# simonsobs/pixell

Hardware: AMD Instinct MI355X
Metric: map2alm+alm2map round-trips/sec (higher is better)
Workload: dtype f64

## Files before the change

### pixell_amd/csrc/fft.hip

```cpp
#include "fft.hpp"
#include "fft_dev.hpp"
#include <cmath>
#include <algorithm>
#include <functional>

namespace pxs {

struct KArgs {
	int n, nfac, T, generic, mode, forward, n1, n2;
	int ns;
	long N;
	const PassDesc* pass;
	const int* perm; const double2* tw;
	FastDiv dn, dT;
	FftDims d; long i_base, i_count;
	long ntile;
	FftLoad ld; FftStore st;
	double2* temp; const double2* bigtw;
	int load_inner_fast, store_inner_fast, tile_i;
};

__device__ __forceinline__ double2 read_elem(const void* p, int dtype, long off) {
	switch (dtype) {
		case PX_F32:  return make_double2((double)((const float*)p)[off], 0.0);
// ... 15 lines not shown
	const FftLoad& ld = a.ld;
	const long base = i*a.d.is_i + o1*a.d.is_o1 + o2*a.d.is_o2;
	const long N = a.N;
	switch (LM) {
	case LD_PLAIN: {
		const long se = e - ld.shift;
		if (se < 0 || (ld.ne >= 0 && se >= ld.ne)) return make_double2(0, 0);
		double2 v = read_elem(ld.ptr, ld.dtype, base + se*a.d.is_e);
		if (ld.mul) v = cmul(v, ld.mul[e]);
		return v; }
	case LD_HERM: {
		if (!ld.herm_fold) {
			const long Nh = ld.herm_n > 0 ? ld.herm_n : N;
			if (e >= Nh) return make_double2(0, 0);
			double2 v;
			if (e < ld.ne) v = read_elem(ld.ptr, ld.dtype, base + e*a.d.is_e);
			else if (Nh - e < ld.ne) v = cconj(read_elem(ld.ptr, ld.dtype, base + (Nh-e)*a.d.is_e));
			else return make_double2(0, 0);
			if (ld.mul) v = cmul(v, ld.mul[e]);
			return v;
		}
		double2 acc = make_double2(0, 0);
		for (long m = e; m < ld.ne; m += N) {
			double2 v = read_elem(ld.ptr, ld.dtype, base + m*a.d.is_e);
			if (ld.mul) v = cmul(v, ld.mul[m]);
			if (m == 0) v.y = 0;
			acc = cadd(acc, v);
		}
		for (long m = N - e; m < ld.ne; m += N) {
			double2 v = read_elem(ld.ptr, ld.dtype, base + m*a.d.is_e);
			if (ld.mul) v = cmul(v, ld.mul[m]);
			acc = cadd(acc, cconj(v));
		}
		return acc; }
	case LD_MIRROR: {
		long src = e;
		const bool odd = ((ld.par_step*(i + a.i_base) + ld.par0) & 1) != 0;
		bool neg = false;
		if (e >= ld.ne) { src = N - e - ld.mir_c; if (src < 0) src += N; neg = odd; }
		if (odd && (2*e + ld.mir_c) % N == 0) return make_double2(0, 0);
		double2 v = read_elem(ld.ptr, ld.dtype, base + src*a.d.is_e);
		if (ld.mul) v = cmul(v, ld.mul[src]);
		return neg ? make_double2(-v.x, -v.y) : v; }
	case LD_MIRROR_PAIR: {
		const long la = 2*(i + a.i_base), lb = la + 1;
		const bool a_odd = (ld.par0 & 1) != 0;
		long src = e; bool mir = false;
		if (e >= ld.ne) { src = N - e - ld.mir_c; if (src < 0) src += N; mir = true; }
		const bool selfm = ((2*e + ld.mir_c) % N) == 0;
		const long ba = (2*i)*a.d.is_i + o1*a.d.is_o1 + o2*a.d.is_o2;
		double2 va = read_elem(ld.ptr, ld.dtype, ba + src*a.d.is_e);
		double2 vb = (lb < ld.pair_lines) ? read_elem(ld.ptr, ld.dtype, ba + a.d.is_i + src*a.d.is_e) : make_double2(0, 0);
		double2& vo = a_odd ? va : vb;
		if (selfm) vo = make_double2(0, 0);
		else if (mir) { vo.x = -vo.x; vo.y = -vo.y; }
		return cadd(va, vb); }
	case LD_REAL_PAIR: {
		const long ba = (2*i)*a.d.is_i + o1*a.d.is_o1 + o2*a.d.is_o2;
		const double va = read_elem(ld.ptr, ld.dtype, ba + e*a.d.is_e).x;
		const double vb = (2*(i + a.i_base) + 1 < ld.pair_lines) ? read_elem(ld.ptr, ld.dtype, ba + a.d.is_i + e*a.d.is_e).x : 0.0;
		return make_double2(va, vb); }
	case LD_HERM_PAIR: {
		long m; bool cj;
		if (e < ld.ne) { m = e; cj = false; }
		else if (N - e < ld.ne) { m = N - e; cj = true; }
		else return make_double2(0, 0);
		const long ba = (2*i)*a.d.is_i + o1*a.d.is_o1 + o2*a.d.is_o2;
		double2 ha = read_elem(ld.ptr, ld.dtype, ba + m*a.d.is_e);
		double2 hb = (2*(i + a.i_base) + 1 < ld.pair_lines) ? read_elem(ld.ptr, ld.dtype, ba + a.d.is_i + m*a.d.is_e) : make_double2(0, 0);
		if (m == 0) { ha.y = 0; hb.y = 0; }
		if (cj) { ha.y = -ha.y; hb.y = -hb.y; }
		return make_double2(ha.x - hb.y, ha.y + hb.x); }
	case LD_SPEC: {
		const long Ns = ld.ne;
		long k = (2*e <= N) ? e : e - N;
		long ak = k < 0 ? -k : k;
		if (ld.kmax >= 0 && ak > ld.kmax) return make_double2(0, 0);
		if (2*ak > Ns) return make_double2(0, 0);
		long si = k >= 0 ? k : Ns + k;
		double2 v = read_elem(ld.ptr, ld.dtype, base + si*a.d.is_e);
		if (2*ak == Ns && ld.nyq_half && N != Ns) { v.x *= 0.5; v.y *= 0.5; }
		if (ld.mul) { double2 ph = ld.mul[ak]; if (k < 0) ph.y = -ph.y; v = cmul(v, ph); }
		return v; }
	default: {
		const long Nb = ld.ne;
		long k = (2*e <= N) ? e : e - N;
		long ak = k < 0 ? -k : k;
		if (ld.kmax >= 0 && ak > ld.kmax) return make_double2(0, 0);
		double2 ph = ld.mul ? ld.mul[ak] : make_double2(1, 0);
		if (2*ak == N && ld.nyq_half && N != Nb) {
			double2 vp = read_elem(ld.ptr, ld.dtype, base + ak*a.d.is_e);
			double2 vm = read_elem(ld.ptr, ld.dtype, base + (Nb-ak)*a.d.is_e);
			double2 r = cadd(cmul(vp, cconj(ph)), cmul(vm, ph));
			return make_double2(0.5*r.x, 0.5*r.y);
		}
		long si = k >= 0 ? k : Nb + k;
		double2 v = read_elem(ld.ptr, ld.dtype, base + si*a.d.is_e);
		if (k >= 0) ph.y = -ph.y;
		return cmul(v, ph); }
	}
}

__device__ __forceinline__ void store_functor(const KArgs& a, long i, long o1, long o2, long e, double2 v) {
	const FftStore& st = a.st;
	if ((st.ne >= 0 && e >= st.ne) || e < st.shift) return;
	long eo = e - st.shift;
	if (st.two_sided_k >= 0) {
		if (e > st.two_sided_k && e < a.N - st.two_sided_k) return;
		if (st.compact_two_sided && e > st.two_sided_k) eo = st.two_sided_k + (a.N - e);
	}
	if (st.conj_out) v.y = -v.y;
	if (st.mul) v = cmul(v, st.mul[e]);
	v.x *= st.scale; v.y *= st.scale;
	if (st.real_pair) {
		const long off = (2*i)*a.d.os_i + o1*a.d.os_o1 + o2*a.d.os_o2 + eo*a.d.os_e;
		write_elem(st.ptr, st.dtype, off, make_double2(v.x, 0));
		if (2*(i + a.i_base) + 1 < st.pair_lines) write_elem(st.ptr, st.dtype, off + a.d.os_i, make_double2(v.y, 0));
		return;
	}
	const long off = i*a.d.os_i + o1*a.d.os_o1 + o2*a.d.os_o2 + eo*a.d.os_e;
	write_elem(st.ptr, st.dtype, off, v);
}

template<int R, int NT> __device__ __forceinline__ void radix_pass(double2* buf, const double2* tw, const KArgs& a, const PassDesc& ps) {
	const int nb = a.n / R;
	const int total = a.T*nb;
	for (int b = threadIdx.x; b < total; b += NT) {
		const uint32_t t = fdiv(b, ps.dnb);
		const uint32_t bb = b - t*nb;
		const uint32_t blk = fdiv(bb, ps.dL);
		const uint32_t q = bb - blk*ps.L;
		const uint32_t p0 = t*a.ns + blk*ps.L*R + q;
		double2 v[R];
#pragma unroll
		for (int i = 0; i < R; i++) v[i] = buf[LPAD(p0 + i*ps.L)];
		if (ps.L > 1) {
			const int step = q*ps.tws;
#pragma unroll
			for (int i = 1; i < R; i++) v[i] = cmul(v[i], tw[i*step]);
		}
		butterfly<R>(v);
#pragma unroll
		for (int i = 0; i < R; i++) buf[LPAD(p0 + i*ps.L)] = v[i];
	}
}

template<int NT> __device__ __forceinline__ void generic_pass(const double2* src, double2* dst, const double2* tw, const KArgs& a, const PassDesc& ps) {
	const int R = ps.R, n = a.n;
	const int total = a.T*n;
	const int wstep = n / R;
	for (int idx = threadIdx.x; idx < total; idx += NT) {
		const uint32_t t = fdiv(idx, a.dn);
		const uint32_t j = idx - t*n;
		const uint32_t LR = ps.L*R;
		const uint32_t blk = j / LR;
		const uint32_t r = j - blk*LR;
		const uint32_t ip = r / ps.L;
		const uint32_t q = r - ip*ps.L;
		const uint32_t p0 = t*a.ns + blk*LR + q;
		double2 acc = make_double2(0, 0);
		uint32_t widx = 0;
		for (int i = 0; i < R; i++) {
			double2 v = src[LPAD(p0 + i*ps.L)];
			if (ps.L > 1) v = cmul(v, tw[i*q*ps.tws]);
			acc = cadd(acc, cmul(v, tw[widx*wstep]));
			widx += ip; if (widx >= (uint32_t)R) widx -= R;
		}
		dst[LPAD(t*a.ns + j)] = acc;
	}
}

struct TileCtx { long s0, other, o1, o2, lo; int nl; };
__device__ __forceinline__ TileCtx tile_decode(const KArgs& a, long bx) {
	TileCtx c;
	const long tile = bx % a.ntile; bx /= a.ntile;
	const long slim = (a.mode == 1) ? a.n2 : a.n1;
	c.other = 0;
	if (a.mode != 0) { const long no = a.tile_i ? slim : a.i_count; c.other = bx % no; bx /= no; }
	c.o1 = bx % a.d.n_o1; c.o2 = bx / a.d.n_o1;
	c.s0 = tile*a.T;
	const long tlim = (a.mode == 0 || a.tile_i) ? a.i_count : slim;
	c.nl = (int)min((long)a.T, tlim - c.s0);
	c.lo = c.o2*a.d.n_o1 + c.o1;
	return c;
}
template<int LM> __device__ __forceinline__ void tile_load_one(const KArgs& a, const TileCtx& c, int idx, int total, double2& v, int& pos) {
	const int n = a.n, T = a.T;
	pos = -1; v = make_double2(0, 0);
	if (idx >= total) return;
	uint32_t t, j;
	if (a.load_inner_fast) { j = fdiv(idx, a.dT); t = idx - j*T; }
	else                   { t = fdiv(idx, a.dn); j = idx - t*n; }
	if ((int)t >= c.nl) return;
	const long il = (a.mode == 0 || a.tile_i) ? c.s0 + t : c.other;
	const long sv = (a.mode == 0) ? 0 : (a.tile_i ? c.other : c.s0 + t);
	if (a.mode == 0)      v = load_functor<LM>(a, il, c.o1, c.o2, j);
	else if (a.mode == 1) v = load_functor<LM>(a, il, c.o1, c.o2, (long)j*a.n2 + sv);
	else {
		const long p2 = sv*a.n2 + j;
		v = a.temp[a.tile_i ? (c.lo*a.N + p2)*a.i_count + il : (c.lo*a.i_count + il)*a.N + p2];
	}
	if (!a.forward && a.mode != 2) v.y = -v.y;
	pos = (int)(t*a.ns) + a.perm[j];
}
template<int NT, bool GEN> __device__ __forceinline__ double2* tile_passes(const KArgs& a, double2* cur, double2* oth, const double2* tw) {
	for (int p = 0; p < a.nfac; p++) {
		const PassDesc ps = a.pass[p];
		switch (ps.R) {
			case 2: radix_pass<2, NT>(cur, tw, a, ps); break;
			case 3: radix_pass<3, NT>(cur, tw, a, ps); break;
			case 4: radix_pass<4, NT>(cur, tw, a, ps); break;
			case 5: radix_pass<5, NT>(cur, tw, a, ps); break;
			default: if constexpr (GEN) { generic_pass<NT>(cur, oth, tw, a, ps); double2* x = cur; cur = oth; oth = x; } break;
		}
		PXS_LDS_BARRIER();
	}
	return cur;
}
template<int NT> __device__ __forceinline__ void tile_store(const KArgs& a, const TileCtx& c, const double2* cur) {
	const int n = a.n, T = a.T, total = T*n;
	for (int idx0 = threadIdx.x; idx0 < total; idx0 += 4*NT) {
#pragma unroll
		for (int u = 0; u < 4; u++) {
			const int idx = idx0 + u*NT;
			if (idx >= total) continue;
			uint32_t t, j;
			if (a.store_inner_fast) { j = fdiv(idx, a.dT); t = idx - j*T; }
			else                    { t = fdiv(idx, a.dn); j = idx - t*n; }
			if ((int)t >= c.nl) continue;
			const long il = (a.mode == 0 || a.tile_i) ? c.s0 + t : c.other;
			const long sv = (a.mode == 0) ? 0 : (a.tile_i ? c.other : c.s0 + t);
			double2 v = cur[LPAD(t*a.ns + j)];
			if (a.mode == 1) {
				v = cmul(v, a.bigtw[(long)j*sv]);
				const long p2 = (long)j*a.n2 + sv;
				a.temp[a.tile_i ? (c.lo*a.N + p2)*a.i_count + il : (c.lo*a.i_count + il)*a.N + p2] = v;
			} else {
				if (!a.forward) v.y = -v.y;
				if (a.mode == 0) store_functor(a, il, c.o1, c.o2, j, v);
				else             store_functor(a, il, c.o1, c.o2, sv + (long)a.n1*j, v);
			}
		}
	}
}

template<int LM, int NT, bool GEN> __global__ __launch_bounds__(NT) void fft_lds_kernel(const KArgs a)
{
	PXS_SHARED(double2, lds);
	const int n = a.n, T = a.T;
	double2* tw = lds;
	double2* bufA = lds + n;
	double2* bufB = bufA + (size_t)T*a.ns + 1;
	const TileCtx c = tile_decode(a, blockIdx.x);
	for (int k = threadIdx.x; k < n; k += NT) tw[k] = a.tw[k];
	const int total = T*n;
	constexpr int LU = 4;
	for (int idx0 = threadIdx.x; idx0 < total; idx0 += LU*NT) {
		double2 v[LU]; int pos[LU];
#pragma unroll
		for (int u = 0; u < LU; u++) tile_load_one<LM>(a, c, idx0 + u*NT, total, v[u], pos[u]);
#pragma unroll
		for (int u = 0; u < LU; u++) if (pos[u] >= 0) bufA[LPAD(pos[u])] = v[u];
	}
	PXS_LDS_BARRIER();
	const double2* cur = tile_passes<NT, GEN>(a, bufA, bufB, tw);
	tile_store<NT>(a, c, cur);
}

template<int LM> static void launch_tiles_m(const KArgs& k, long nblk, size_t sh, hipStream_t st, int nt_override) {
#ifdef PXS_HOST_SIM
	hipLaunchKernelGGL((fft_lds_kernel<LM, 1, true>), dim3((unsigned)nblk), dim3(1), sh, st, k);
#else
	static const int nt_env = [] { const char* e = lab_getenv("PXS_FFT_NT"); return e ? atoi(e) : 0; }();
	const int nt = nt_override ? nt_override : nt_env ? nt_env : ((long)k.T*k.n >= 2048 ? 512 : 256);
	static const bool once = [] {
		(void)hipFuncSetAttribute((const void*)fft_lds_kernel<LM, 256, false>, hipFuncAttributeMaxDynamicSharedMemorySize, 160*1024 - 256);
		(void)hipFuncSetAttribute((const void*)fft_lds_kernel<LM, 256, true>, hipFuncAttributeMaxDynamicSharedMemorySize, 160*1024 - 256);
		(void)hipFuncSetAttribute((const void*)fft_lds_kernel<LM, 512, false>, hipFuncAttributeMaxDynamicSharedMemorySize, 160*1024 - 256);
		(void)hipFuncSetAttribute((const void*)fft_lds_kernel<LM, 128, false>, hipFuncAttributeMaxDynamicSharedMemorySize, 160*1024 - 256);
		return true; }();
	(void)once;
	if (k.generic)      hipLaunchKernelGGL((fft_lds_kernel<LM, 256, true>), dim3((unsigned)nblk), dim3(256), sh, st, k);
	else if (nt == 512) hipLaunchKernelGGL((fft_lds_kernel<LM, 512, false>), dim3((unsigned)nblk), dim3(512), sh, st, k);
	else if (nt == 128) hipLaunchKernelGGL((fft_lds_kernel<LM, 128, false>), dim3((unsigned)nblk), dim3(128), sh, st, k);
	else                hipLaunchKernelGGL((fft_lds_kernel<LM, 256, false>), dim3((unsigned)nblk), dim3(256), sh, st, k);
#endif
}
static void launch_tiles(const KArgs& k, long nblk, size_t sh, hipStream_t st, int nt_override = 0) {
	const int lm = k.mode == 2 ? (int)LD_PLAIN : k.ld.mode;
	switch (lm) {
		case LD_PLAIN:       launch_tiles_m<LD_PLAIN>(k, nblk, sh, st, nt_override); break;
		case LD_HERM:        launch_tiles_m<LD_HERM>(k, nblk, sh, st, nt_override); break;
		case LD_MIRROR:      launch_tiles_m<LD_MIRROR>(k, nblk, sh, st, nt_override); break;
		case LD_SPEC:        launch_tiles_m<LD_SPEC>(k, nblk, sh, st, nt_override); break;
		case LD_SPEC_ADJ:    launch_tiles_m<LD_SPEC_ADJ>(k, nblk, sh, st, nt_override); break;
		case LD_MIRROR_PAIR: launch_tiles_m<LD_MIRROR_PAIR>(k, nblk, sh, st, nt_override); break;
		case LD_REAL_PAIR:   launch_tiles_m<LD_REAL_PAIR>(k, nblk, sh, st, nt_override); break;
		case LD_HERM_PAIR:   launch_tiles_m<LD_HERM_PAIR>(k, nblk, sh, st, nt_override); break;
		default: throw Error(PXS_ERR_ARG, "fft: unknown load mode");
	}
}

struct FftSub {
	int n; std::vector<int> fac; bool generic = false;
	DevBuf perm, tw, d_pass;
	PassDesc pass[FFT_MAXFAC]; int nfac = 0;
};

static std::vector<int> factorize(long n) {
	std::vector<int> f;
	static const int oddfirst = [] { const char* e = lab_getenv("PXS_FFT_ODDFIRST"); return e ? atoi(e) : 1; }();
	if (oddfirst) {
		while (n % 3 == 0) { f.push_back(3); n /= 3; }
		while (n % 5 == 0) { f.push_back(5); n /= 5; }
		int twos = 0; while (n % 2 == 0) { twos++; n /= 2; }
		if (twos & 1) { f.push_back(2); twos--; }
		while (twos >= 2) { f.push_back(4); twos -= 2; }
	}
	while (n % 4 == 0) { f.push_back(4); n /= 4; }
	while (n % 2 == 0) { f.push_back(2); n /= 2; }
	while (n % 3 == 0) { f.push_back(3); n /= 3; }
	while (n % 5 == 0) { f.push_back(5); n /= 5; }
	for (long p = 7; p*p <= n; p += 2) while (n % p == 0) { f.push_back((int)p); n /= p; }
	if (n > 1) f.push_back((int)n);
	return f;
}

static void twiddles(long n, std::vector<double2>& tw) {
	tw.resize(n);
	const long double tp = 6.283185307179586476925286766559L;
	for (long k = 0; k < n; k++) {
		long double ang = tp*(long double)k/(long double)n;
		tw[k] = make_double2((double)cosl(ang), (double)(-sinl(ang)));
	}
}

FftContext::FftContext(int device) : device_(device) {
	size_t fr = 0, tot = 0;
	if (hipMemGetInfo(&fr, &tot) == hipSuccess && fr > 0) temp_budget = std::min<size_t>(size_t(4) << 30, std::max<size_t>(fr/16, size_t(64) << 20));
}
FftContext::~FftContext() {}

static bool split_two(long n, long& n1, long& n2) {
	long best = -1, best8 = -1;
	for (long a = 1; a*a <= n; a++) if (n % a == 0) {
		long b = n/a; if (b > FFT_NLOC_MAX) continue;
		best = a;
		if (a % 8 == 0 && b % 8 == 0 && 4*a >= b) best8 = a;
	}
	if (best < 0) return false;
	static const int align8 = [] { const char* e = lab_getenv("PXS_FFT_ALIGN8"); return e ? atoi(e) : 1; }();
	if (best8 > 0 && align8) best = best8;
	n1 = best; n2 = n/best;
	return n1 <= FFT_NLOC_MAX && n2 <= FFT_NLOC_MAX;
}

bool FftContext::supported(long n, std::string* why) {
	if (n < 1) { if (why) *why = "length < 1"; return false; }
	if (n <= FFT_NLOC_MAX) {
		if ((int)factorize(n).size() > FFT_MAXFAC) { if (why) *why = "too many factors"; return false; }
		return true;
	}
	long n1, n2;
	if (!split_two(n, n1, n2)) {
		if (why) *why = "FFT length " + std::to_string(n) + " has no factorisation n1*n2 with both factors <= " +
			std::to_string(FFT_NLOC_MAX) + " (large prime factor; Bluestein not implemented)";
		return false;
	}
	return true;
}

long FftContext::good_size(long n) {
	for (long m = std::max<long>(n, 1);; m++) {
		long r = m;
		while (r % 2 == 0) r /= 2; while (r % 3 == 0) r /= 3; while (r % 5 == 0) r /= 5;
		if (r == 1 && supported(m)) return m;
	}
}

static std::vector<int> factorize_comp(long n, int maxr) {
	static const std::vector<int> allowed = [] {
		std::vector<int> a; const char* e = lab_getenv("PXS_FFT_RADICES");
		std::string s = e ? e : "16,15,12,10,9,8,7,6,5,4,3,2";
		size_t pos = 0;
		while (pos < s.size()) { size_t c = s.find(',', pos); if (c == std::string::npos) c = s.size(); int v = atoi(s.substr(pos, c-pos).c_str()); if (v >= 2 && (v <= 5 || v <= PXS_COMP_MAXR)) a.push_back(v); pos = c+1; }
		return a; }();
	std::vector<int> best, cur;
	std::function<void(long, size_t)> rec = [&](long m, size_t from) {
		if (m == 1) { if (best.empty() || cur.size() < best.size()) best = cur; return; }
		if (!best.empty() && cur.size()+1 >= best.size()) return;
		for (size_t i = from; i < allowed.size(); i++) if (m % allowed[i] == 0 && (allowed[i] == 7 ? maxr >= 9 : (allowed[i] <= 5 || allowed[i] <= maxr))) { cur.push_back(allowed[i]); rec(m/allowed[i], i); cur.pop_back(); }
	};
	rec(n, 0);
	if (best.empty()) return factorize(n);
	std::stable_sort(best.begin(), best.end(), [](int a, int b) { const bool oa = a & 1, ob = b & 1; if (oa != ob) return oa; return a > b; });
	return best;
}

std::shared_ptr<FftSub> FftContext::sub(long n, bool comp, int maxr) {
	std::lock_guard<std::mutex> g(mu_);
	static const bool comp_on = [] { const char* e = lab_getenv("PXS_FFT_COMP"); return e ? atoi(e) != 0 : true; }();
	comp = comp && comp_on;
	maxr = std::min(maxr, PXS_COMP_MAXR);
	const long key = comp ? -(n + ((long)maxr << 40)) : n;
	auto it = subs_.find(key);
	if (it != subs_.end()) return it->second;
	auto s = std::make_shared<FftSub>();
	s->n = (int)n; s->fac = comp ? factorize_comp(n, maxr) : factorize(n);
	PXS_REQUIRE((int)s->fac.size() <= FFT_MAXFAC, "FFT: too many factors");
	int L = 1; s->nfac = (int)s->fac.size();
	std::vector<int> Ls(s->nfac+1); Ls[0] = 1;
	for (int p = 0; p < s->nfac; p++) {
		int R = s->fac[p];
		const bool comp_r = comp && R <= maxr && (R == 6 || R == 8 || R == 9 || R == 10 || R == 12 || R == 15 || R == 16);
		const bool seven = comp && R == 7 && maxr >= 9;
		if (R != 2 && R != 3 && R != 4 && R != 5 && !comp_r && !seven) s->generic = true;
		PassDesc& ps = s->pass[p];
		ps.R = R; ps.L = L; ps.tws = (int)(n/((long)L*R));
		ps.dL = make_fastdiv(L); ps.dnb = make_fastdiv((uint32_t)(n/R));
		L *= R; Ls[p+1] = L;
	}
	std::vector<int> perm(n);
	for (long j = 0; j < n; j++) {
		long t = j, pos = 0;
		for (int p = s->nfac-1; p >= 0; p--) { long i = t % s->fac[p]; t /= s->fac[p]; pos += i*Ls[p]; }
		perm[j] = (int)pos;
	}
	std::vector<double2> tw; twiddles(n, tw);
	s->perm = upload(perm); s->tw = upload(tw);
	s->d_pass = upload(std::vector<PassDesc>(s->pass, s->pass + FFT_MAXFAC));
	subs_[key] = s;
	return s;
}

FftContext::SubView FftContext::view(long n, int maxr) {
	auto s = sub(n, true, maxr);
	SubView v; v.n = s->n; v.nfac = s->nfac; v.ns = s->n | 1; v.generic = s->generic ? 1 : 0;
	v.pass = s->d_pass.p; v.perm = s->perm.as<int>(); v.tw = s->tw.as<double2>();
	return v;
}

const double2* FftContext::bigtw(long n) {
	std::lock_guard<std::mutex> g(mu_);
	auto it = bigtw_.find(n);
	if (it != bigtw_.end()) return it->second.as<double2>();
	std::vector<double2> tw; twiddles(n, tw);
	bigtw_[n] = upload(tw);
	return bigtw_[n].as<double2>();
}

static void fill_sub(KArgs& k, const FftSub& s, long maxlines) {
	k.n = s.n; k.nfac = s.nfac; k.generic = s.generic;
#ifdef PXS_LAB
	{ static const int nopass = [] { const char* e = getenv("PXS_FFT_DEBUG_NOPASS"); return e ? atoi(e) : 0; }(); if (nopass) k.nfac = 0; }
#endif
	k.pass = s.d_pass.as<PassDesc>();
	k.perm = s.perm.as<int>(); k.tw = s.tw.as<double2>();
	int bufs = s.generic ? 2 : 1;
	static const long env_pts = [] { const char* e = lab_getenv("PXS_FFT_PTS"); return e ? atol(e) : 0L; }();
	long pts = s.n <= 1024 ? FFT_LDS_PTS/2 : FFT_LDS_PTS;
	if (env_pts > 0 && s.n <= env_pts/2) pts = env_pts;
	long T = (pts - s.n)/((long)bufs*s.n);
	if (T < 1) T = 1;
	if (T > 64) T = 64;
	static const int align8 = [] { const char* e = lab_getenv("PXS_FFT_ALIGN8"); return e ? atoi(e) : 1; }();
	if (align8) {
		if (T >= 8) T -= T % 8;
		else if (T >= 5 && (long)bufs*8*s.n + s.n <= FFT_LDS_PTS) T = 8;
	}
	if (T > maxlines) T = maxlines;
	k.T = (int)T;
	k.dn = make_fastdiv(s.n); k.dT = make_fastdiv((uint32_t)T);
	static const int lpad = [] { const char* e = lab_getenv("PXS_FFT_LINEPAD"); return e ? atoi(e) : 1; }();
	k.ns = lpad ? (s.n | 1) : s.n;
}

static size_t lds_bytes(const KArgs& k) { const size_t pts = (size_t)k.T*k.ns + 2; return sizeof(double2)*((size_t)k.n + pts*(k.generic ? 2 : 1)); }

void FftContext::exec(hipStream_t st, long n, bool forward, const FftDims& d, const FftLoad& ld, const FftStore& stf) {
	std::string why;
	if (!supported(n, &why)) throw Error(PXS_ERR_UNSUPPORTED, why);
	if (d.n_i <= 0 || d.n_o1 <= 0 || d.n_o2 <= 0) return;
	KArgs k; memset(&k, 0, sizeof(k));
	k.N = n; k.forward = forward ? 1 : 0; k.d = d; k.ld = ld; k.st = stf; k.i_base = 0; k.i_count = d.n_i;
	if (n <= FFT_NLOC_MAX) {
		auto s = sub(n);
		fill_sub(k, *s, d.n_i);
		k.mode = 0; k.n1 = (int)n; k.n2 = 1;
		k.ntile = (d.n_i + k.T - 1)/k.T;
		k.load_inner_fast  = (std::abs(d.is_i) < std::abs(d.is_e)) ? 1 : 0;
		k.store_inner_fast = (std::abs(d.os_i) < std::abs(d.os_e)) ? 1 : 0;
		long nblk = k.ntile*d.n_o1*d.n_o2;
		size_t sh = lds_bytes(k);
		launch_tiles(k, nblk, sh, st);
		PXS_HIP(hipGetLastError());
		return;
	}
	long n1, n2; split_two(n, n1, n2);
	auto s1 = sub(n1); auto s2 = sub(n2);
	const double2* btw = bigtw(n);
	long lines_budget = std::max<long>(1, (long)(temp_budget/(sizeof(double2)*n)));
	DevBuf* tbuf = nullptr;
	{
		std::lock_guard<std::mutex> g(mu_);
		size_t want = sizeof(double2)*n*std::min<long>(lines_budget, d.n_i*d.n_o1*d.n_o2);
		tbuf = &temps_[st];
		tbuf->ensure(want);
	}
	long o1_per = 1, i_per = d.n_i;
	if (d.n_i <= lines_budget) { o1_per = std::min<long>(d.n_o1, std::max<long>(1, lines_budget/d.n_i)); }
	else i_per = lines_budget;
	for (long o2 = 0; o2 < d.n_o2; o2++)
	for (long o1 = 0; o1 < d.n_o1; o1 += o1_per)
	for (long i0 = 0; i0 < d.n_i; i0 += i_per) {
		long no1 = std::min(o1_per, d.n_o1 - o1), ni = std::min(i_per, d.n_i - i0);
		KArgs a = k;
		a.d.n_o1 = no1; a.d.n_o2 = 1; a.i_base = i0; a.i_count = ni;
		auto esz = [](int dt) { return dt == PX_F32 ? 4 : dt == PX_F64 ? 8 : dt == PX_C64 ? 8 : 16; };
		const long lmul = (ld.mode == LD_MIRROR_PAIR || ld.mode == LD_REAL_PAIR || ld.mode == LD_HERM_PAIR) ? 2 : 1;
		const long smul = stf.real_pair ? 2 : 1;
		a.ld.ptr = (const char*)ld.ptr + esz(ld.dtype)*(o2*d.is_o2 + o1*d.is_o1 + lmul*i0*d.is_i);
		a.st.ptr = (char*)stf.ptr + esz(stf.dtype)*(o2*d.os_o2 + o1*d.os_o1 + smul*i0*d.os_i);
		a.temp = tbuf->as<double2>(); a.bigtw = btw; a.n1 = (int)n1; a.n2 = (int)n2;
		const int tile_i = (std::abs(d.is_i) < std::abs(d.is_e)) ? 1 : 0;
		KArgs pa = a; fill_sub(pa, *s1, tile_i ? ni : n2); pa.mode = 1; pa.tile_i = tile_i;
		pa.ntile = ((tile_i ? ni : n2) + pa.T - 1)/pa.T;
		pa.load_inner_fast = 1; pa.store_inner_fast = 1;
		long nblkA = pa.ntile*(tile_i ? n2 : ni)*no1;
		launch_tiles(pa, nblkA, lds_bytes(pa), st);
		KArgs pb = a; fill_sub(pb, *s2, tile_i ? ni : n1); pb.mode = 2; pb.tile_i = tile_i;
		pb.ntile = ((tile_i ? ni : n1) + pb.T - 1)/pb.T;
		pb.load_inner_fast = tile_i ? 1 : 0; pb.store_inner_fast = 1;
		long nblkB = pb.ntile*(tile_i ? n1 : ni)*no1;
		launch_tiles(pb, nblkB, lds_bytes(pb), st);
		PXS_HIP(hipGetLastError());
	}
}

}
```

### pixell_amd/csrc/fft.hpp

```cpp
#pragma once
#include "common.hpp"
#include <map>
#include <memory>
#include <mutex>

namespace pxs {

enum LoadMode : int { LD_PLAIN = 0, LD_HERM = 1, LD_MIRROR = 2, LD_SPEC = 3, LD_SPEC_ADJ = 4, LD_MIRROR_PAIR = 5, LD_REAL_PAIR = 6, LD_HERM_PAIR = 7 };

struct FftDims {
	long n_i = 1, n_o1 = 1, n_o2 = 1;
	long is_i = 0, is_o1 = 0, is_o2 = 0, is_e = 1;
	long os_i = 0, os_o1 = 0, os_o2 = 0, os_e = 1;
};

struct FftLoad {
	const void* ptr = nullptr; int dtype = PX_C128; int mode = LD_PLAIN;
	long ne = -1;
	const double2* mul = nullptr;
	long shift = 0;
	int mir_c = 0, par0 = 0;
	int par_step = 1;
	long kmax = -1;
	int nyq_half = 0;
	long pair_lines = 0;
	int herm_fold = 0;
	long herm_n = 0;
};

struct FftStore {
	void* ptr = nullptr; int dtype = PX_C128;
	long ne = -1;
	long two_sided_k = -1;
	const double2* mul = nullptr;
	double scale = 1.0;
	long shift = 0;
	int conj_out = 0;
	int compact_two_sided = 0;
	int real_pair = 0;
	long pair_lines = 0;
};

struct FftSub;

class FftContext {
public:
	explicit FftContext(int device);
	~FftContext();
	void exec(hipStream_t st, long n, bool forward, const FftDims& d, const FftLoad& ld, const FftStore& stf);
	static long good_size(long n);
	static bool supported(long n, std::string* why = nullptr);
	struct SubView { int n, nfac, ns, generic; const void* pass; const int* perm; const double2* tw; };
	SubView view(long n, int maxr = 1000);
	const double2* twiddle_table(long n) { return bigtw(n); }
	void release_stream(hipStream_t st) { std::lock_guard<std::mutex> g(mu_); temps_.erase(st); }
	size_t temp_budget = size_t(4) << 30;
private:
	int device_;
	std::mutex mu_;
	std::map<long, std::shared_ptr<FftSub>> subs_;
	std::map<long, DevBuf> bigtw_;
	std::map<hipStream_t, DevBuf> temps_;
	std::shared_ptr<FftSub> sub(long n, bool comp = false, int maxr = 1000);
	const double2* bigtw(long n);
};

}
```

### pixell_amd/csrc/fftchain.hip

```cpp
#include "fftchain.hpp"
#include "fft_dev.hpp"
#include "chain_dev.hpp"
#include <algorithm>
#include <set>
#include <type_traits>
#include <cmath>

namespace pxs {

#ifndef PXS_CH_PTS
#define PXS_CH_PTS 2560
#endif
#ifdef PXS_HOST_SIM
static constexpr int CH_NT = 1, CH_MAXE = PXS_CH_PTS;
#else
#ifndef PXS_CH_NT
#define PXS_CH_NT 512
#endif
static constexpr int CH_NT = PXS_CH_NT, CH_MAXE = (PXS_CH_PTS + PXS_CH_NT - 1)/PXS_CH_NT;
#endif
static constexpr int CH_TILE_PTS = PXS_CH_PTS;
static constexpr int CH_NMAX = 512;

struct TileC { int outer, t0, nl, comp, q0; };

struct BlkIn {
	int Tw, nBf, wL; FastDiv dTTw, dTw, dwL;
	__device__ __forceinline__ long off(int line, int e, int nrows) const {
		const uint32_t B = fdiv((uint32_t)e, dTw);
		const int w = (int)B < nBf ? Tw : wL;
		return (long)B*Tw*nrows + (long)line*w + (e - (int)B*Tw);
	}
	__device__ __forceinline__ void split(int idx, int T, uint32_t& li, uint32_t& e) const {
		uint32_t B = fdiv((uint32_t)idx, dTTw);
		if ((int)B < nBf) { const uint32_t rem = idx - B*T*Tw; li = fdiv(rem, dTw); e = B*Tw + (rem - li*Tw); }
		else { const uint32_t rem = idx - (uint32_t)nBf*T*Tw; li = fdiv(rem, dwL); e = (uint32_t)nBf*Tw + (rem - li*wL); }
	}
};

struct StageBase {
	static constexpr bool R7 = true;
	static constexpr int NT = CH_NT;
	static constexpr int PTS = CH_TILE_PTS;
	LdsFft fa, fb;
	BlkIn bin; int bout;
	int T; int ntile;
	FastDiv dT, dna, dnb, dnt;
	const double2* btw; const double2* tws;
	int pf;
	static constexpr int PF = 256;
	static constexpr int PFI = 0;
	__device__ __forceinline__ const void* pfaddr(const TileC&, int) const { return nullptr; }
};

#ifndef PXS_HOST_SIM
#define PXS_CH_BOUNDS __launch_bounds__(NT, S::MINW)
#else
#define PXS_CH_BOUNDS
#endif
template<class S, int NT, int MAXE> __global__ PXS_CH_BOUNDS void chain_kernel(const S s)
{
	PXS_SHARED(double2, lds);
	const int na = s.fa.n, nb = s.fb.n;
	const int nlast = S::TWO ? nb : na, nslast = S::TWO ? s.fb.ns : s.fa.ns;
	const bool same_tw = S::TWO && nb == na;
	double2* twa = lds; double2* twb = same_tw ? lds : lds + na; double2* twx = lds + na + (same_tw ? 0 : nb); double2* buf = twx + (S::HAS_TW ? nlast : 0);
	TileC c;
	if (!s.decode((int)blockIdx.x, c)) return;
	const bool have_tw = S::HAS_TW && s.btw != nullptr;
	const int T = s.T;
	int pf_val = 0;
	{
		const int total = T*na;
		double2 v[MAXE]; int pos[MAXE];
#pragma unroll
		for (int u = 0; u < MAXE; u++) {
			const int idx = threadIdx.x + u*NT; pos[u] = -1;
			if (idx < total) {
				uint32_t li, e;
				if (S::LOAD_LINE_FAST) { e = fdiv(idx, s.dT); li = idx - e*T; }
				else if (s.bin.Tw > 0) s.bin.split(idx, T, li, e);
				else { li = fdiv(idx, s.dna); e = idx - li*na; }
				v[u] = s.load(c, (int)li, (int)e);
				if (S::INV_A) v[u].y = -v[u].y;
				pos[u] = (int)li*s.fa.ns + s.fa.perm[e];
			}
		}
		if ((S::LOADK == 0 || S::PFI > 0) && s.pf > 0 && (long)blockIdx.x + s.pf < (long)gridDim.x) {
			TileC c2;
			if (s.decode((int)blockIdx.x + s.pf, c2)) {
				if (S::LOADK == 0) {
					const int per = (na*16 + 127) >> 7, i = threadIdx.x;
					if (i < T*per) {
						const int li = i/per, seg = i - li*per;
						const double2* r = s.row(c2, li);
						if (r) pf_val = *reinterpret_cast<const int*>(reinterpret_cast<const char*>(r) + seg*128);
					}
				} else {
#pragma unroll
					for (int it = 0; it < S::PFI; it++) {
						const void* q = s.pfaddr(c2, (int)threadIdx.x + it*NT);
						if (q) pf_val += *reinterpret_cast<const int*>(q);
					}
				}
			}
		}
		for (int k = threadIdx.x; k < na; k += NT) twa[k] = s.fa.tw[k];
		if (!same_tw) for (int k = threadIdx.x; k < nb; k += NT) twb[k] = s.fb.tw[k];
		if (have_tw) for (int k = threadIdx.x; k < nlast; k += NT) twx[k] = s.btw[(long)c.t0*k];
#pragma unroll
		for (int u = 0; u < MAXE; u++) if (pos[u] >= 0) buf[pos[u]] = v[u];
	}
	PXS_LDS_BARRIER();
	lds_fft<NT, S::MAXR, S::R7>(buf, twa, s.fa, T);
	if (S::TWO) {
		const int total = T*nb;
		double2 v[MAXE]; int pos[MAXE];
#pragma unroll
		for (int u = 0; u < MAXE; u++) {
			const int idx = threadIdx.x + u*NT; pos[u] = -1;
			if (idx < total) {
				const uint32_t e = fdiv(idx, s.dT), li = idx - e*T;
				{ const double2* Al = buf + li*s.fa.ns; v[u] = s.mid(c, (int)li, (int)e, [&](int k) { return Al[k]; }); }
				if (S::INV_B) v[u].y = -v[u].y;
				pos[u] = (int)li*s.fb.ns + s.fb.perm[e];
			}
		}
		PXS_LDS_BARRIER();
#pragma unroll
		for (int u = 0; u < MAXE; u++) if (pos[u] >= 0) buf[pos[u]] = v[u];
		PXS_LDS_BARRIER();
		lds_fft<NT, S::MAXR, S::R7>(buf, twb, s.fb, T);
	}
	{
		const int total = T*nlast;
		const FastDiv dl = S::TWO ? s.dnb : s.dna;
		for (int idx = threadIdx.x; idx < total; idx += NT) {
			uint32_t li, e;
			if (S::STORE_LINE_FAST) { e = fdiv(idx, s.dT); li = idx - e*T; } else { li = fdiv(idx, dl); e = idx - li*nlast; }
			double2 w = make_double2(1, 0);
			if (have_tw) w = cmul(twx[e], s.tws[e*T + li]);
			s.store(c, (int)li, (int)e, [&](int l2, int e2) { return buf[l2*nslast + e2]; }, w);
		}
	}
#ifndef PXS_HOST_SIM
	if (S::LOADK == 0 || S::PFI > 0) asm volatile("" :: "v"(pf_val));
#endif
}

struct StFirst : StageBase {
	static constexpr int SID = 0;
	static constexpr bool TWO = false, INV_A = false, INV_B = false, LOAD_LINE_FAST = true, STORE_LINE_FAST = true, HAS_TW = true;
	static constexpr int MAXR = 9, MINW = 1;
	PairSrc src; int b; double2* Y; long ldY; int npair; FastDiv dnp;
	static constexpr int LOADK = 1, STOREK = 0;
	__device__ __forceinline__ const double2* row(const TileC&, int) const { return nullptr; }
	__device__ __forceinline__ bool decode(int bx, TileC& c) const {
		c.outer = fdiv(bx, dnt); c.t0 = (bx - c.outer*ntile)*T; c.nl = min(T, b - c.t0);
		c.comp = fdiv(c.outer, dnp); c.q0 = c.outer - c.comp*npair; return true; }
	__device__ __forceinline__ double2 load(const TileC& c, int li, int e) const {
		if (li >= c.nl) return make_double2(0, 0);
		return src.get(c.comp, c.q0, b*e + c.t0 + li); }
	template<class AF> __device__ __forceinline__ double2 mid(const TileC&, int, int, AF&&) const { return make_double2(0, 0); }
	template<class VF> __device__ __forceinline__ void store(const TileC& c, int li, int e, VF&& val, double2 w) const {
		if (li >= c.nl) return;
		const long o = bout ? ((long)c.outer*b + c.t0)*fa.n + (long)e*c.nl + li : ((long)c.outer*fa.n + e)*ldY + c.t0 + li;
		Y[o] = cmul(val(li, e), w); }
};

struct StFirst2D : StFirst {
	static constexpr bool R7 = false;
	static constexpr int PFI = 2;
	__device__ __forceinline__ const void* pfaddr(const TileC& c, int i) const {
		const int segs = (c.nl + 7) >> 3;
		const int e = i/segs; if (e >= fa.n) return nullptr;
		return src.leg + (long)c.comp*src.cstride + (long)c.q0*src.ld + (b*e + c.t0 + 8*(i - e*segs)); }
};

struct StResize : StageBase {
	static constexpr int SID = 1;
	static constexpr bool TWO = true, INV_A = false, INV_B = true, LOAD_LINE_FAST = false, STORE_LINE_FAST = true, HAS_TW = true;
	#ifndef PXS_RESIZE_MINW
#define PXS_RESIZE_MINW 1
#endif
	static constexpr int MAXR = 9, MINW = PXS_RESIZE_MINW;
#ifdef PXS_RESIZE_PTS
	static constexpr int PTS = PXS_RESIZE_PTS;
#endif
	const double2* Y; long ldY; double2* Z; long ldZ;
	int g, X1, X2, kmax, nyq; const double2* ph; FastDiv dg;
	int adj;
	static constexpr int LOADK = 0, STOREK = 0;
	__device__ __forceinline__ const double2* row(const TileC& c, int li) const { return li < c.nl ? Y + ((long)c.outer*g + c.t0 + li)*ldY : nullptr; }
	__device__ __forceinline__ bool decode(int bx, TileC& c) const {
		c.outer = fdiv(bx, dnt); c.t0 = (bx - c.outer*ntile)*T; c.nl = min(T, g - c.t0); return true; }
	__device__ __forceinline__ double2 load(const TileC& c, int li, int e) const {
		if (li >= c.nl) return make_double2(0, 0);
		return bin.Tw > 0 ? Y[(long)c.outer*g*fa.n + bin.off(c.t0 + li, e, g)] : Y[((long)c.outer*g + c.t0 + li)*ldY + e]; }
	template<class AF> __device__ __forceinline__ double2 mid(const TileC& c, int li, int e, AF&& A) const {
		if (li >= c.nl) return make_double2(0, 0);
		const int k1 = c.t0 + li;
		const int jp = g*e + k1;
		const int kap = (2*jp <= X2) ? jp : jp - X2;
		const int ak = kap < 0 ? -kap : kap;
		if ((kmax >= 0 && ak > kmax) || 2*ak > X1) return make_double2(0, 0);
		const int k = kap >= 0 ? kap : kap + X1;
		const uint32_t k2 = fdiv((uint32_t)(k - k1), dg);
		double2 v = A((int)k2);
		if (adj) {
			double2 t = ph ? ph[ak] : make_double2(1, 0);
			if (2*ak == X2 && X1 != X2) {
				const double2 vm = A((int)fdiv((uint32_t)(X1 - ak - k1), dg));
				const double2 r = cadd(cmul(v, cconj(t)), cmul(vm, t));
				return cscale(r, 0.5);
			}
			if (kap >= 0) t.y = -t.y;
			return cmul(v, t);
		}
		if (nyq && 2*ak == X1) v = cscale(v, 0.5);
		if (ph) { double2 t = ph[ak]; if (kap < 0) t.y = -t.y; v = cmul(v, t); }
		return v; }
	template<class VF> __device__ __forceinline__ void store(const TileC& c, int li, int e, VF&& val, double2 w) const {
		if (li >= c.nl) return;
		const long o = bout ? ((long)c.outer*g + c.t0)*fb.n + (long)e*c.nl + li : ((long)c.outer*fb.n + e)*ldZ + c.t0 + li;
		Z[o] = cmul(cconj(val(li, e)), cconj(w)); }
};

struct StSigma : StageBase {
	static constexpr int SID = 2;
	static constexpr bool TWO = true, INV_A = true, INV_B = false, LOAD_LINE_FAST = false, STORE_LINE_FAST = true, HAS_TW = true;
	static constexpr int MAXR = 9, MINW = 1;
	const double2* Z; long ldZ; double2* V; long ldV; int g, g2; const double2* sigma;
	static constexpr int LOADK = 0, STOREK = 0;
	__device__ __forceinline__ const double2* row(const TileC& c, int li) const { return li < c.nl ? Z + ((long)c.outer*g2 + c.t0 + li)*ldZ : nullptr; }
	__device__ __forceinline__ bool decode(int bx, TileC& c) const {
		c.outer = fdiv(bx, dnt); c.t0 = (bx - c.outer*ntile)*T; c.nl = min(T, g2 - c.t0); return true; }
	__device__ __forceinline__ double2 load(const TileC& c, int li, int e) const {
		if (li >= c.nl) return make_double2(0, 0);
		return bin.Tw > 0 ? Z[(long)c.outer*g2*fa.n + bin.off(c.t0 + li, e, g2)] : Z[((long)c.outer*g2 + c.t0 + li)*ldZ + e]; }
	template<class AF> __device__ __forceinline__ double2 mid(const TileC& c, int li, int e, AF&& A) const {
		if (li >= c.nl) return make_double2(0, 0);
		return cmul(cconj(A(e)), sigma[(c.t0 + li) + g2*e]); }
	template<class VF> __device__ __forceinline__ void store(const TileC& c, int li, int e, VF&& val, double2 w) const {
		if (li >= c.nl) return;
		const long o = bout ? ((long)c.outer*g2 + c.t0)*fb.n + (long)e*c.nl + li : ((long)c.outer*g + e)*ldV + c.t0 + li;
		V[o] = cmul(val(li, e), w); }
};

template<int MODE> struct StSplit : StageBase {
	static constexpr int SID = 3 + MODE;
#ifndef PXS_HOST_SIM
	static constexpr int NT = MODE == 1 ? 256 : CH_NT;
#endif
	static constexpr int PF = MODE == 1 ? 512 : 256;
	static constexpr bool TWO = false, INV_A = true, INV_B = false, LOAD_LINE_FAST = false, STORE_LINE_FAST = true, HAS_TW = false;
	static constexpr int MAXR = 9, MINW = 1;
	const double2* U; long ldU; int a, g, X, mir_c, nr_out, a_odd, ncol, npair;
	double2* out; long ld; const double2* w; const double2* tab; double scale; int TH; FastDiv da;
	long ocstride; int groups; FastDiv dnp, dgr;
	int self_half;
	static constexpr int LOADK = 0, STOREK = 1;
	__device__ __forceinline__ const double2* row(const TileC& c, int li) const {
		int line, pair; slot(c, li, line, pair);
		return line >= 0 ? U + (((long)c.comp*npair + pair)*a + line)*ldU : nullptr; }
	__device__ __forceinline__ int mirror_line(int k) const { int m = a - k - mir_c; if (m >= a) m -= a; if (m < 0) m += a; return m; }
	__device__ __forceinline__ bool decode(int bx, TileC& c) const {
		c.outer = fdiv(bx, dnt); c.t0 = (bx - c.outer*ntile)*(MODE == 0 ? TH : 1); c.nl = T;
		if (MODE == 0) { c.comp = fdiv(c.outer, dnp); c.q0 = c.outer - c.comp*npair; }
		else { c.comp = fdiv(c.outer, dgr); c.q0 = (c.outer - c.comp*groups)*(T/2); }
		if (MODE == 1) { if (mirror_line(c.t0) < c.t0) return false; }
		return true; }
	__device__ __forceinline__ void slot(const TileC& c, int li, int& line, int& pair) const {
		if (MODE == 0) {
			pair = c.q0;
			const int prim = c.t0 + (li < TH ? li : li - TH);
			line = -1;
			if (prim < a) {
				const int m = mirror_line(prim);
				if (li < TH) { if (prim <= m) line = prim; }
				else if (prim < m) line = m;
			}
		} else {
			pair = c.q0 + (li >> 1);
			const int m = mirror_line(c.t0);
			line = (li & 1) ? (m != c.t0 ? m : -1) : c.t0;
			if (pair >= npair) line = -1;
		}
	}
	__device__ __forceinline__ double2 load(const TileC& c, int li, int e) const {
		int line, pair; slot(c, li, line, pair);
		if (line < 0) return make_double2(0, 0);
		if (MODE == 0 && bin.Tw > 0) return U[((long)c.comp*npair + pair)*a*fa.n + bin.off(line, e, a)];
		return U[(((long)c.comp*npair + pair)*a + line)*ldU + e]; }
	template<class AF> __device__ __forceinline__ double2 mid(const TileC&, int, int, AF&&) const { return make_double2(0, 0); }
	template<class VF> __device__ __forceinline__ void store(const TileC& c, int li, int e, VF&& val, double2) const {
		int line, pair; slot(c, li, line, pair);
		if (line < 0) return;
		const int t = line + a*e;
		if (t >= nr_out) return;
		int tm = X - t - mir_c; if (tm >= X) tm -= X; if (tm < 0) tm += X;
		const double2 z = cconj(val(li, e));
		double2 ev, od;
		if (tm == t) { ev = self_half ? cscale(z, 0.5) : z; od = make_double2(0, 0); }
		else {
			const int ml = mirror_line(line);
			const int lp = (ml == line) ? li : (MODE == 0 ? (li < TH ? li + TH : li - TH) : (li ^ 1));
			const int e2 = (int)fdiv((uint32_t)(tm - ml), da);
			const double2 y = cconj(val(lp, e2));
			ev = make_double2(0.5*(z.x + y.x), 0.5*(z.y + y.y)); od = make_double2(0.5*(z.x - y.x), 0.5*(z.y - y.y));
		}
		const int ca = 2*pair;
		double2 va = a_odd ? od : ev, vb = a_odd ? ev : od;
		double2* oc = out + (long)c.comp*ocstride;
		if (MODE == 0) {
			const double f = scale*(w ? w[t].x : 1.0);
			oc[(long)ca*ld + t] = cscale(va, f);
			if (ca + 1 < ncol) oc[(long)(ca + 1)*ld + t] = cscale(vb, f);
		} else {
			const double f = scale*(w ? w[t].x : 1.0);
			oc[(long)t*ld + ca] = cscale(cmul(va, cconj(tab[ca])), f);
			if (ca + 1 < ncol) oc[(long)t*ld + ca + 1] = cscale(cmul(vb, cconj(tab[ca + 1])), f);
		}
	}
};


struct StRingA1 : StageBase {
	static constexpr int SID = 5;
	static constexpr int PTS = 2880;
	static constexpr bool TWO = false, INV_A = false, INV_B = false, LOAD_LINE_FAST = true, STORE_LINE_FAST = true, HAS_TW = true;
	static constexpr int MAXR = 8, MINW = 8;
	MapAddr m; int b, npair; double2* Y; long ldY; FastDiv dnp;
	static constexpr int LOADK = 1, STOREK = 0;
	__device__ __forceinline__ const double2* row(const TileC&, int) const { return nullptr; }
	__device__ __forceinline__ bool decode(int bx, TileC& c) const {
		c.outer = fdiv(bx, dnt); c.t0 = (bx - c.outer*ntile)*T; c.nl = min(T, b - c.t0);
		c.comp = fdiv(c.outer, dnp); c.q0 = c.outer - c.comp*npair; return true; }
	__device__ __forceinline__ double2 load(const TileC& c, int li, int e) const {
		if (li >= c.nl) return make_double2(0, 0);
		const int x = b*e + c.t0 + li;
		const int bi = (int)fdiv(c.comp, m.dncb);
		const long o = bi*m.bstride + (c.comp - bi*m.ncb)*m.cstride + m.off0 + (2L*c.q0)*m.rstride + x*m.pstride;
		const double re = rd_real(m.ptr, m.dtype, o).x;
		const double im = (2*c.q0 + 1 < m.nring) ? rd_real(m.ptr, m.dtype, o + m.rstride).x : 0.0;
		return make_double2(re, im); }
	template<class AF> __device__ __forceinline__ double2 mid(const TileC&, int, int, AF&&) const { return make_double2(0, 0); }
	template<class VF> __device__ __forceinline__ void store(const TileC& c, int li, int e, VF&& val, double2 w) const {
		if (li >= c.nl) return;
		Y[((long)c.outer*fa.n + e)*ldY + c.t0 + li] = cmul(val(li, e), w); }
};

struct StRingA2 : StageBase {
	static constexpr int SID = 6;
	static constexpr int PF = 512;
	static constexpr bool TWO = false, INV_A = false, INV_B = false, LOAD_LINE_FAST = false, STORE_LINE_FAST = true, HAS_TW = false;
	static constexpr int MAXR = 8, MINW = 8;
	const double2* Y; long ldY; int a, X, npair, groups, nring, mmax; double2* leg; long ldleg; int nm; const double2* tab; double scale; FastDiv da, dgr;
	static constexpr int LOADK = 0, STOREK = 1;
	__device__ __forceinline__ const double2* row(const TileC& c, int li) const {
		int line, q; slot(c, li, line, q);
		return line >= 0 ? Y + (((long)c.comp*npair + q)*a + line)*ldY : nullptr; }
	__device__ __forceinline__ int mirror_line(int k) const { return k == 0 ? 0 : a - k; }
	__device__ __forceinline__ bool decode(int bx, TileC& c) const {
		c.outer = fdiv(bx, dnt); c.t0 = bx - c.outer*ntile; c.nl = T;
		c.comp = fdiv(c.outer, dgr); c.q0 = (c.outer - c.comp*groups)*(T/2);
		return mirror_line(c.t0) >= c.t0; }
	__device__ __forceinline__ void slot(const TileC& c, int li, int& line, int& q) const {
		q = c.q0 + (li >> 1);
		const int ml = mirror_line(c.t0);
		line = (li & 1) ? (ml != c.t0 ? ml : -1) : c.t0;
		if (q >= npair) line = -1;
	}
	__device__ __forceinline__ double2 load(const TileC& c, int li, int e) const {
		int line, q; slot(c, li, line, q);
		if (line < 0) return make_double2(0, 0);
		return Y[(((long)c.comp*npair + q)*a + line)*ldY + e]; }
	template<class AF> __device__ __forceinline__ double2 mid(const TileC&, int, int, AF&&) const { return make_double2(0, 0); }
	template<class VF> __device__ __forceinline__ void store(const TileC& c, int li, int e, VF&& val, double2) const {
		int line, q; slot(c, li, line, q);
		if (line < 0) return;
		const int k = line + a*e;
		if (k > mmax) return;
		const double2 zp = val(li, e);
		double2 zm;
		if (k == 0) zm = zp;
		else {
			const int kp = X - k, ml = mirror_line(line);
			const int lp = (ml == line) ? li : (li ^ 1);
			zm = val(lp, (int)fdiv((uint32_t)(kp - ml), da));
		}
		double2 xa = make_double2(0.5*(zp.x + zm.x), 0.5*(zp.y - zm.y));
		const double2 d = make_double2(zp.x - zm.x, zp.y + zm.y);
		double2 xb = make_double2(0.5*d.y, -0.5*d.x);
		const double2 t = tab ? tab[k] : make_double2(1, 0);
		double2* o = leg + ((long)c.comp*nm + k)*ldleg + 2*q;
		o[0] = cscale(cmul(xa, t), scale);
		if (2*q + 1 < nring) o[1] = cscale(cmul(xb, t), scale);
	}
};

struct StRingS1 : StageBase {
	static constexpr int SID = 7;
	static constexpr bool TWO = false, INV_A = true, INV_B = false, LOAD_LINE_FAST = true, STORE_LINE_FAST = true, HAS_TW = true;
	static constexpr int MAXR = 8, MINW = 8;
	const double2* h; long ldh, hcomp; int b, X, npair, nring, mmax; double2* Y; long ldY; FastDiv dnp;
	static constexpr int LOADK = 1, STOREK = 0;
	__device__ __forceinline__ const double2* row(const TileC&, int) const { return nullptr; }
	__device__ __forceinline__ bool decode(int bx, TileC& c) const {
		c.outer = fdiv(bx, dnt); c.t0 = (bx - c.outer*ntile)*T; c.nl = min(T, b - c.t0);
		c.comp = fdiv(c.outer, dnp); c.q0 = c.outer - c.comp*npair; return true; }
	__device__ __forceinline__ double2 load(const TileC& c, int li, int e) const {
		if (li >= c.nl) return make_double2(0, 0);
		const int k = b*e + c.t0 + li;
		int m; bool cj;
		if (k <= mmax) { m = k; cj = false; }
		else if (X - k <= mmax) { m = X - k; cj = true; }
		else return make_double2(0, 0);
		const double2* r = h + ((long)c.comp*hcomp + 2*c.q0)*ldh + m;
		double2 ha = r[0];
		double2 hb = (2*c.q0 + 1 < nring) ? r[ldh] : make_double2(0, 0);
		if (m == 0) { ha.y = 0; hb.y = 0; }
		if (cj) { ha.y = -ha.y; hb.y = -hb.y; }
		return make_double2(ha.x - hb.y, ha.y + hb.x); }
	template<class AF> __device__ __forceinline__ double2 mid(const TileC&, int, int, AF&&) const { return make_double2(0, 0); }
	template<class VF> __device__ __forceinline__ void store(const TileC& c, int li, int e, VF&& val, double2 w) const {
		if (li >= c.nl) return;
		const long o = bout ? ((long)c.outer*b + c.t0)*fa.n + (long)e*c.nl + li : ((long)c.outer*fa.n + e)*ldY + c.t0 + li;
		Y[o] = cmul(cconj(val(li, e)), cconj(w)); }
};

struct StRingS2 : StageBase {
	static constexpr int SID = 8;
	static constexpr bool TWO = false, INV_A = true, INV_B = false, LOAD_LINE_FAST = false, STORE_LINE_FAST = true, HAS_TW = false;
	static constexpr int MAXR = 8, MINW = 8;
	const double2* Y; long ldY; int a, npair; MapAddr m; FastDiv dnp;
	static constexpr int LOADK = 0, STOREK = 0;
	__device__ __forceinline__ const double2* row(const TileC& c, int li) const { return li < c.nl ? Y + ((long)c.outer*a + c.t0 + li)*ldY : nullptr; }
	__device__ __forceinline__ bool decode(int bx, TileC& c) const {
		c.outer = fdiv(bx, dnt); c.t0 = (bx - c.outer*ntile)*T; c.nl = min(T, a - c.t0);
		c.comp = fdiv(c.outer, dnp); c.q0 = c.outer - c.comp*npair; return true; }
	__device__ __forceinline__ double2 load(const TileC& c, int li, int e) const {
		if (li >= c.nl) return make_double2(0, 0);
		return bin.Tw > 0 ? Y[(long)c.outer*a*fa.n + bin.off(c.t0 + li, e, a)] : Y[((long)c.outer*a + c.t0 + li)*ldY + e]; }
	template<class AF> __device__ __forceinline__ double2 mid(const TileC&, int, int, AF&&) const { return make_double2(0, 0); }
	template<class VF> __device__ __forceinline__ void store(const TileC& c, int li, int e, VF&& val, double2) const {
		if (li >= c.nl) return;
		const int x = c.t0 + li + a*e;
		const double2 v = val(li, e);
		const int bi = (int)fdiv(c.comp, m.dncb);
		const long o = bi*m.bstride + (c.comp - bi*m.ncb)*m.cstride + m.off0 + (2L*c.q0)*m.rstride + x*m.pstride;
		wr_real(m.ptr, m.dtype, o, v.x);
		if (2*c.q0 + 1 < m.nring) wr_real(m.ptr, m.dtype, o + m.rstride, -v.y);
	}
};

struct StColOut : StageBase {
	static constexpr int SID = 9;
	static constexpr bool R7 = false;
	static constexpr bool TWO = false, INV_A = false, INV_B = false, LOAD_LINE_FAST = false, STORE_LINE_FAST = true, HAS_TW = false;
	static constexpr int MAXR = 9, MINW = 1;
	const double2* Y; long ldY; int a, nm, ny, nx, groups, conj_out, herm; double2* out; long ldo, ocomp; double scale; FastDiv dgr;
	static constexpr int LOADK = 0, STOREK = 0;
	__device__ __forceinline__ const double2* row(const TileC& c, int li) const { return c.q0 + li < nm ? Y + (((long)c.comp*nm + c.q0 + li)*a + c.t0)*ldY : nullptr; }
	__device__ __forceinline__ bool decode(int bx, TileC& c) const {
		c.outer = fdiv(bx, dnt); c.t0 = bx - c.outer*ntile; c.nl = T;
		c.comp = fdiv(c.outer, dgr); c.q0 = (c.outer - c.comp*groups)*T; return true; }
	__device__ __forceinline__ double2 load(const TileC& c, int li, int e) const {
		const int kx = c.q0 + li;
		if (kx >= nm) return make_double2(0, 0);
		return Y[(((long)c.comp*nm + kx)*a + c.t0)*ldY + e]; }
	template<class AF> __device__ __forceinline__ double2 mid(const TileC&, int, int, AF&&) const { return make_double2(0, 0); }
	template<class VF> __device__ __forceinline__ void store(const TileC& c, int li, int e, VF&& val, double2) const {
		const int kx = c.q0 + li;
		if (kx >= nm) return;
		const int ky = c.t0 + a*e;
		double2 v = cscale(val(li, e), scale);
		double2* oc = out + (long)c.comp*ocomp;
		oc[(long)ky*ldo + kx] = conj_out ? cconj(v) : v;
		if (herm && kx > 0 && 2*kx < nx) oc[(long)(ky == 0 ? 0 : ny - ky)*ldo + (nx - kx)] = conj_out ? v : cconj(v);
	}
};

static bool smooth235(long n) { if (n < 1) return false; for (int p : {2, 3, 5}) while (n % p == 0) n /= p; return n == 1; }
bool FftChain::sub_ok(long n) { return n >= 2 && n <= CH_NMAX && smooth235(n); }

static LdsFft mk(FftContext* fc, long n, int maxr = 9) {
	LdsFft f; memset(&f, 0, sizeof(f));
	if (n <= 0) return f;
	auto v = fc->view(n, maxr);
#ifdef PXS_LAB
	static const int nofft = [] { const char* e = getenv("PXS_CH_NOFFT"); return e ? atoi(e) : 0; }();
#else
	constexpr int nofft = 0;
#endif
	static const int nspad = [] { const char* e = lab_getenv("PXS_CH_NS_PAD"); return e ? atoi(e) : 0; }();
	f.n = v.n; f.nfac = nofft ? 0 : v.nfac; f.ns = v.ns + nspad; f.generic = v.generic; f.pass = (const PassDesc*)v.pass; f.perm = v.perm; f.tw = v.tw; f.dn = make_fastdiv((uint32_t)n);
	return f;
}

const double2* FftChain::small_tw(long X, int n, int T) {
#ifdef PXS_LAB
	{ static const int notw = [] { const char* e = getenv("PXS_CH_NOTW"); return e ? atoi(e) : 0; }(); if (notw) return nullptr; }
#endif
	std::lock_guard<std::mutex> g(mu_);
	auto key = std::make_tuple(X, n, T);
	auto it = stw_.find(key);
	if (it != stw_.end()) return it->second.as<double2>();
	std::vector<double2> t((size_t)n*T);
	const long double tp = 6.283185307179586476925286766559L;
	for (int e = 0; e < n; e++) for (int li = 0; li < T; li++) {
		const long double ang = tp*(long double)(((long)li*e) % X)/(long double)X;
		t[(size_t)e*T + li] = make_double2((double)cosl(ang), (double)(-sinl(ang)));
	}
	stw_[key] = upload(t);
	return stw_[key].as<double2>();
}

static int tile_lines(long n_a, long n_b, long nlines, int mult, long tab_pts = -1) {
	const long n = std::max(n_a, n_b);
	long T = CH_TILE_PTS / n;
	if (T >= mult) T -= T % mult;
	if (T < 1) T = 1;
	const long cap = ((nlines + mult - 1)/mult)*mult;
	if (T > cap) T = cap;
	static const long limit = [] { const char* e = lab_getenv("PXS_RING_TILE_KB"); return e ? (long)(atof(e)*1024) : 0L; }();
	if (tab_pts >= 0 && limit > 0)
		while (T > mult && (long)sizeof(double2)*(tab_pts + T*(n | 1) + 2) > limit) T -= mult;
	return (int)T;
}
template<class S> void FftChain::set_tiles(S& s, int T, long nlines, long X) {
	s.T = T; s.ntile = (int)((nlines + T - 1)/T); s.dT = make_fastdiv((uint32_t)T); s.dnt = make_fastdiv((uint32_t)s.ntile);
	s.dna = make_fastdiv((uint32_t)s.fa.n); s.dnb = make_fastdiv((uint32_t)std::max(1, s.fb.n));
	s.btw = nullptr; s.tws = nullptr;
	if (X > 0) { s.tws = small_tw(X, S::TWO ? s.fb.n : s.fa.n, T); s.btw = s.tws ? fc_->twiddle_table(X) : nullptr; }
}
static bool blocked_on() { static const bool on = [] { const char* e = lab_getenv("PXS_CH_BLOCKED"); return e ? atoi(e) != 0 : false; }(); return on; }
static BlkIn mk_blk(int Tw, long na, int T) {
	BlkIn b; memset(&b, 0, sizeof(b));
	if (!blocked_on()) return b;
	b.Tw = Tw; b.nBf = (int)(na/Tw); b.wL = (int)(na - (long)b.nBf*Tw);
	b.dTTw = make_fastdiv((uint32_t)(T*Tw)); b.dTw = make_fastdiv((uint32_t)Tw); b.dwL = make_fastdiv((uint32_t)std::max(b.wL, 1));
	return b;
}

static const int F2_RADICES[] = {2, 3, 4, 5, 6, 8, 9};

template<class S> static void launch_stage(const S& s, long nblk, hipStream_t st) {
	if (nblk <= 0) return;
	PXS_REQUIRE((long)s.T*std::max(s.fa.n, s.fb.n) <= S::PTS, "internal: chain tile too large");
	PXS_REQUIRE(nblk < (1L << 31), "internal: chain grid too large");
	size_t sh = sizeof(double2)*((size_t)s.fa.n + (S::TWO && s.fb.n == s.fa.n ? 0 : s.fb.n) + (S::HAS_TW ? std::max(s.fa.n, s.fb.n) : 0) + (size_t)s.T*std::max(s.fa.ns, s.fb.ns) + 2);
	{ static const size_t pad = [] { const char* e = lab_getenv("PXS_CH_LDS_PAD"); return e ? (size_t)atol(e) : (size_t)0; }(); sh += pad; }
	{ static const int pf = [] {
		const std::string name = "PXS_CH_PF_SID" + std::to_string(S::SID);
		const char* e1 = lab_getenv(name.c_str()); const char* e = lab_getenv("PXS_CH_PF");
		return e1 ? atoi(e1) : (e ? atoi(e) : S::PF); }(); const_cast<S&>(s).pf = pf; }
	if (getenv("PXS_CHAIN_VERBOSE")) {
		static std::mutex mu; static std::set<std::tuple<int, int, int, int>> seen; std::lock_guard<std::mutex> g(mu);
		if (seen.insert(std::make_tuple(S::SID, s.fa.n, s.fb.n, s.T)).second)
			fprintf(stderr, "[pxsht] chain stage %d: na=%d nb=%d T=%d LDS %.1f KiB -> %d WG/CU by LDS, %ld workgroups\n", S::SID, s.fa.n, s.fb.n, s.T, sh/1024.0, (int)((160*1024)/sh), nblk);
	}
#ifndef PXS_HOST_SIM
#ifdef PXS_CH_NT2
	static const long mask2 = [] { const char* e = lab_getenv("PXS_CH_NT2_MASK"); return e ? strtol(e, nullptr, 0) : 0L; }();
	if ((mask2 >> S::SID) & 1) {
		constexpr int NT2 = PXS_CH_NT2, MAXE2 = (S::PTS + NT2 - 1)/NT2;
		static const bool once2 = [] { (void)hipFuncSetAttribute((const void*)chain_kernel<S, NT2, MAXE2>, hipFuncAttributeMaxDynamicSharedMemorySize, 160*1024 - 256); return true; }();
		(void)once2;
		hipLaunchKernelGGL((chain_kernel<S, NT2, MAXE2>), dim3((unsigned)nblk), dim3(NT2), sh, st, s);
		return;
	}
#endif
	static const bool once = [] { (void)hipFuncSetAttribute((const void*)chain_kernel<S, S::NT, (S::PTS + S::NT - 1)/S::NT>, hipFuncAttributeMaxDynamicSharedMemorySize, 160*1024 - 256); return true; }();
	(void)once;
#endif
	hipLaunchKernelGGL((chain_kernel<S, S::NT, (S::PTS + S::NT - 1)/S::NT>), dim3((unsigned)nblk), dim3(S::NT), sh, st, s);
}

template<class S> int FftChain::tile_lines_for(long n_a, long n_b, long nlines, int mult, long tab_pts) {
	int T = tile_lines(n_a, n_b, nlines, mult, tab_pts);
	if (S::PTS > CH_TILE_PTS && T < mult && (long)mult*std::max(n_a, n_b) <= S::PTS && nlines >= mult) T = mult;
	return T;
}
template<class S> void FftChain::launch_any(S& s, long nblk, hipStream_t st) { launch_stage(s, nblk, st); }

static bool split_balanced(long n, Split& s, long amax = 320) {
	long best = 0; double bestc = 1e300;
	for (long a = 2; a <= 1024 && a <= n/2; a++) if (n % a == 0) {
		const long b = n/a;
		if (!FftChain::sub_ok(a) || !FftChain::sub_ok(b)) continue;
		double c = std::fabs(std::log((double)a/(double)b));
		if (a > amax) c += 10;
		if (b % 8) c += 0.3;
		if (c < bestc) { bestc = c; best = a; }
	}
	if (!best) return false;
	s.a = best; s.b = n/best; return true;
}

bool FftChain::plan_rings(long nphi) {
	nphi_ = nphi; ra_ = Split(); rs_ = Split();
	Split s;
	if (!split_balanced(nphi, s)) return false;
	ra_.a = std::min(s.a, s.b); ra_.b = nphi/ra_.a;
	rs_.b = std::min(s.a, s.b); rs_.a = nphi/rs_.b;
	for (long a = 320; a >= 16; a -= 16) if (nphi % a == 0 && nphi/a <= 160 && nphi/a >= 2 && sub_ok(a) && sub_ok(nphi/a)) { rs_.a = a; rs_.b = nphi/a; break; }
	for (long b = 256; b >= 16; b -= 16) if (nphi % b == 0 && nphi/b >= 2 && nphi/b <= 320 && sub_ok(b) && sub_ok(nphi/b)) { ra_.b = b; ra_.a = nphi/b; break; }
	{
		const char* ea = lab_getenv("PXS_RING_A_ANA"); const char* es = lab_getenv("PXS_RING_A_SYN");
		if (ea && atol(ea) > 1 && nphi % atol(ea) == 0 && sub_ok(atol(ea)) && sub_ok(nphi/atol(ea))) { ra_.a = atol(ea); ra_.b = nphi/ra_.a; }
		if (es && atol(es) > 1 && nphi % atol(es) == 0 && sub_ok(atol(es)) && sub_ok(nphi/atol(es))) { rs_.a = atol(es); rs_.b = nphi/rs_.a; }
	}
	return true;
}

static long smooth_at_least(long n, bool even_product_with = false, long g = 1) {
	for (long m = std::max<long>(n, 2);; m++) if (smooth235(m) && (!even_product_with || ((m*g) % 2 == 0))) return m;
}

static bool smooth2357(long n) { if (n < 1) return false; for (int p : {2, 3, 5, 7}) while (n % p == 0) n /= p; return n == 1; }
static bool sub_ok7(long n) { return n >= 2 && n <= CH_NMAX && smooth2357(n); }
bool FftChain::sub_ok_theta(long n) { return sub_ok7(n); }
long FftChain::ducc_ncc(int lmax) {
	for (long n = std::max<long>(lmax + 1, 1);; n++) { long r = n; for (int p : {2, 3, 5, 7, 11}) while (r % p == 0) r /= p; if (r == 1) return 2*n; }
}

static double tile_fill(long n) {
	long T = CH_TILE_PTS / n; if (T >= 8) T -= T % 8; if (T < 1) T = 1;
	return (double)(T*n)/(double)CH_TILE_PTS*(T >= 8 ? 1.0 : 0.8);
}
static double modulus_pref(long g) { return 1.0 + 0.02*std::max(0.0, std::log2((double)g/160.0)) + 0.04*std::max(0.0, std::log2(64.0/(double)g)); }
ThetaPlan FftChain::plan_theta(long N, int lmax) {
	ThetaPlan best; double bestc = 1e300;
	static const long gforce = [] { const char* e = lab_getenv("PXS_THETA_G"); return e ? atol(e) : 0L; }();
	static const bool ducc_size = [] { const char* e = lab_getenv("PXS_THETA_DUCC_NCC"); return e ? atoi(e) != 0 : true; }();
	const long Nd = ducc_ncc(lmax);
	auto consider = [&](long g, long ac) {
		ThetaPlan t; t.N = N; t.g = g; t.bN = N/g; t.ac = ac; t.Ncc = g*ac;
		t.g2 = smooth_at_least((N + 2L*lmax + 2 + g - 1)/g); t.M = g*t.g2;
		if ((t.Ncc & 1) || !sub_ok(t.g2) || !sub_ok7(t.ac)) return;
		long gs_best = 0; double gsc = 1e300;
		static const long gsforce = [] { const char* e = lab_getenv("PXS_THETA_GS"); return e ? atol(e) : 0L; }();
		for (long gs = 2; gs <= 1024; gs++) if (t.Ncc % gs == 0 && N % gs == 0 && sub_ok7(gs) && sub_ok7(t.Ncc/gs) && sub_ok7(N/gs) && (!gsforce || gs == gsforce)) {
			const double c = ((2.0*t.Ncc + 1.5*N)/tile_fill(gs) + (double)(t.Ncc + N)/tile_fill(std::max(t.Ncc/gs, N/gs)))*modulus_pref(gs);
			if (c < gsc) { gsc = c; gs_best = gs; }
		}
		if (!gs_best) return;
		t.gs = gs_best; t.bs = t.Ncc/gs_best; t.aNs = N/gs_best;
		const double lmin = 2.0*lmax + 2, M2 = 2.0*t.Ncc;
		const double ana = (2.0*N + 2.0*M2 + 1.5*t.Ncc)/tile_fill(g) + (N + M2)/tile_fill(std::max(t.bN, 2*t.ac)) + (M2 + t.Ncc)/tile_fill(2*t.ac);
		double c = 60.0*(t.Ncc - lmin)/lmin + (ana*modulus_pref(g) + gsc)/(3.0*N + 4.0*M2 + 2.5*t.Ncc + 3.0*t.Ncc + 2.5*N);
		if (ducc_size && t.Ncc == Nd) c -= 1000.0;
		if (c < bestc) { bestc = c; best = t; best.ok = true; }
	};
	for (long g = 2; g <= 1024 && g <= N/2; g++) if (N % g == 0 && sub_ok7(g) && sub_ok7(N/g) && (!gforce || g == gforce)) {
		consider(g, smooth_at_least((2L*lmax + 2 + g - 1)/g, true, g));
		if (ducc_size && Nd % g == 0) consider(g, Nd/g);
	}
	return best;
}


static long ring_chunk(long npair, long bytes_per_pair, int mult) {
	static const long mb = [] { const char* e = getenv("PXS_RING_CHUNK_MB"); return e ? atol(e) : 0L; }();
	if (mb <= 0) return npair;
	long q = std::max<long>(mult, ((mb << 20)/std::max<long>(bytes_per_pair, 1))/mult*mult);
	return std::min(q, npair);
}

void FftChain::map2leg(hipStream_t st, const MapDesc& m, int nc, int mmax, double2* leg, long ldleg, const double2* tab, double scale) {
	PXS_REQUIRE(rings_ok() && m.nphi == nphi_, "internal: ring chain not planned");
	const long npair_all = (m.nring + 1)/2, a = ra_.a, b = ra_.b, ldY = pad8(b);
	int T2 = tile_lines_for<StRingA2>(b, 0, 2*npair_all, 8, b); if (T2 < 2) T2 = 2; T2 -= T2 % 2;
	const long qchunk = ring_chunk(npair_all, (long)sizeof(double2)*nc*a*ldY, T2/2);
	s1_.ensure(sizeof(double2)*(size_t)nc*qchunk*a*ldY);
	for (long q_lo = 0; q_lo < npair_all; q_lo += qchunk) {
		const long npair = std::min(qchunk, npair_all - q_lo);
		const int nring = m.nring - (int)(2*q_lo);
		{	StRingA1 s; memset(&s, 0, sizeof(s));
			s.fa = mk(fc_, a, 8); s.fb = mk(fc_, 0, 8);
			s.m = map_addr(m); s.m.off0 += 2*q_lo*m.ring_stride; s.m.nring = nring;
			s.b = (int)b; s.npair = (int)npair; s.Y = s1_.as<double2>(); s.ldY = ldY; s.dnp = make_fastdiv((uint32_t)npair);
			set_tiles(s, tile_lines_for<StRingA1>(a, 0, b, 16, 2*a), b, nphi_);
			launch_any(s, (long)nc*npair*s.ntile, st);
		}
		{	StRingA2 s; memset(&s, 0, sizeof(s));
			s.fa = mk(fc_, b, 8); s.fb = mk(fc_, 0, 8);
			const int T = T2;
			set_tiles(s, T, a*T, 0);
			s.Y = s1_.as<double2>(); s.ldY = ldY; s.a = (int)a; s.X = (int)nphi_; s.npair = (int)npair; s.nring = nring; s.mmax = mmax;
			s.groups = (int)((npair + T/2 - 1)/(T/2)); s.da = make_fastdiv((uint32_t)a); s.dgr = make_fastdiv((uint32_t)s.groups);
			s.leg = leg + 2*q_lo; s.ldleg = ldleg; s.nm = mmax + 1; s.tab = tab; s.scale = scale;
			launch_any(s, (long)nc*s.groups*a, st);
		}
	}
	PXS_HIP(hipGetLastError());
}

void FftChain::h2map(hipStream_t st, const double2* h, long ldh, const MapDesc& m, int nc, int mmax, long hcomp) {
	PXS_REQUIRE(rings_ok() && m.nphi == nphi_, "internal: ring chain not planned");
	if (line_h2map(st, h, ldh, m, nc, mmax, hcomp)) return;
	const long npair_all = (m.nring + 1)/2, a = rs_.a, b = rs_.b, ldY = pad8(b);
	const long qchunk = ring_chunk(npair_all, (long)sizeof(double2)*nc*a*ldY, 1);
	const int T1 = tile_lines_for<StRingS1>(a, 0, b, 8, 2*a), T2 = tile_lines_for<StRingS2>(b, 0, a, 16, b);
	s1_.ensure(sizeof(double2)*(size_t)nc*qchunk*a*ldY);
	for (long q_lo = 0; q_lo < npair_all; q_lo += qchunk) {
		const long npair = std::min(qchunk, npair_all - q_lo);
		const int nring = m.nring - (int)(2*q_lo);
		{	StRingS1 s; memset(&s, 0, sizeof(s));
			s.fa = mk(fc_, a, 8); s.fb = mk(fc_, 0, 8);
			s.h = h + 2*q_lo*ldh; s.ldh = ldh; s.hcomp = hcomp > 0 ? hcomp : m.nring; s.b = (int)b; s.X = (int)nphi_; s.npair = (int)npair; s.nring = nring; s.mmax = mmax;
			s.Y = s1_.as<double2>(); s.ldY = ldY; s.dnp = make_fastdiv((uint32_t)npair);
			set_tiles(s, T1, b, nphi_); s.bout = blocked_on();
			launch_any(s, (long)nc*npair*s.ntile, st);
		}
		{	StRingS2 s; memset(&s, 0, sizeof(s));
			s.fa = mk(fc_, b, 8); s.fb = mk(fc_, 0, 8);
			s.Y = s1_.as<double2>(); s.ldY = ldY; s.a = (int)a; s.npair = (int)npair; s.m = map_addr(m); s.m.off0 += 2*q_lo*m.ring_stride; s.m.nring = nring;
			s.dnp = make_fastdiv((uint32_t)npair);
			set_tiles(s, T2, a, 0); s.bin = mk_blk(T1, b, T2);
			launch_any(s, (long)nc*npair*s.ntile, st);
		}
	}
	PXS_HIP(hipGetLastError());
}

static int theta_comp_chunk(int nc, size_t need1_per_comp, size_t need2_per_comp) {
	static const size_t budget = [] { const char* e = getenv("PXS_CHAIN_SCRATCH_GB"); return (size_t)(e ? atol(e) : 12) << 30; }();
	const size_t per = sizeof(double2)*std::max(need1_per_comp, need2_per_comp);
	return (int)std::max<size_t>(1, std::min<size_t>((size_t)nc, budget/std::max<size_t>(per, 1)));
}
void FftChain::theta_scratch(const ThetaPlan& tp, int nm, int nc, int kind, size_t& b1, size_t& b2) {
	const size_t npair = (size_t)(nm + 1)/2;
	size_t n1, n2;
	if (kind == 0)      { n1 = npair*std::max(tp.g*pad8(tp.bN), tp.g*pad8(tp.g2)); n2 = npair*std::max(tp.g2*pad8(tp.g), tp.ac*pad8(tp.g)); }
	else if (kind == 1) { n1 = npair*tp.g*pad8(tp.bN); n2 = npair*tp.ac*pad8(tp.g); }
	else if (kind == 2) { n1 = npair*tp.gs*pad8(tp.bs); n2 = npair*tp.aNs*pad8(tp.gs); }
	else                { n1 = npair*std::max(tp.g*pad8(tp.ac), tp.g*pad8(tp.g2)); n2 = npair*std::max(tp.g2*pad8(tp.g), tp.bN*pad8(tp.g)); }
	const int cc = theta_comp_chunk(nc, n1, n2);
	b1 = sizeof(double2)*n1*cc; b2 = sizeof(double2)*n2*cc;
}
void FftChain::ring_scratch(long nring, int nc, bool analysis, size_t& b1, int mmax) const {
	if (!analysis && mmax >= 0 && line_h2map_takes(nphi_, mmax)) { b1 = 0; return; }
	const long npair = (nring + 1)/2, a = analysis ? ra_.a : rs_.a, b = analysis ? ra_.b : rs_.b;
	b1 = sizeof(double2)*(size_t)nc*npair*a*pad8(b);
}

void FftChain::to_cc(hipStream_t st, const ThetaPlan& tp, const double2* leg, long ldleg, int nr, int mir_c, double2* leg_cc, long ldcc, int ncc,
                     int nc, int nm, int spin, int lmax, const double2* ph_shift, const double2* sigma, const double2* wcc)
{
	if (line_analysis(st, tp, true, leg, ldleg, nr, mir_c, leg_cc, ldcc, ncc, nc, nm, spin, lmax, ph_shift, sigma, wcc, nullptr)) return;
	const long npair = (nm + 1)/2;
	const long g = tp.g, bN = tp.bN, g2 = tp.g2, ac = tp.ac;
	const long ldY1 = pad8(bN), ldZ2 = pad8(g), ldV3 = pad8(g2), ldU4 = pad8(g);
	const size_t need1 = (size_t)npair*std::max(g*ldY1, g*ldV3), need2 = (size_t)npair*std::max(g2*ldZ2, ac*ldU4);
	const int cchunk = theta_comp_chunk(nc, need1, need2);
	const int T1 = tile_lines_for<StFirst>(g, 0, bN, 8), T2 = tile_lines_for<StResize>(bN, g2, g, 8), T3 = tile_lines_for<StSigma>(g, g, g2, 8), T4 = tile_lines_for<StResize>(g2, ac, g, 8);
	s1_.ensure(sizeof(double2)*need1*cchunk); s2_.ensure(sizeof(double2)*need2*cchunk);
	for (int c0 = 0; c0 < nc; c0 += cchunk) {
		const long ncl = std::min(cchunk, nc - c0);
		{	StFirst s; memset(&s, 0, sizeof(s));
			s.fa = mk(fc_, g); s.fb = mk(fc_, 0);
			s.src.leg = leg + (size_t)c0*nm*ldleg; s.src.cstride = (long)nm*ldleg; s.src.ld = ldleg; s.src.nr = nr; s.src.N = (int)tp.N; s.src.mir_c = mir_c; s.src.a_odd = spin & 1; s.src.ncol = nm;
			s.b = (int)bN; s.Y = s1_.as<double2>(); s.ldY = ldY1; s.npair = (int)npair; s.dnp = make_fastdiv((uint32_t)npair);
			set_tiles(s, T1, bN, tp.N); s.bout = blocked_on();
			launch_any(s, ncl*npair*s.ntile, st);
		}
		{	StResize s; memset(&s, 0, sizeof(s));
			s.fa = mk(fc_, bN); s.fb = mk(fc_, g2);
			s.Y = s1_.as<double2>(); s.ldY = ldY1; s.Z = s2_.as<double2>(); s.ldZ = ldZ2; s.g = (int)g; s.X1 = (int)tp.N; s.X2 = (int)tp.M;
			s.kmax = tp.M > tp.N ? -1 : (int)(tp.M/2 - 1); s.nyq = tp.M > tp.N ? 1 : 0;
			s.ph = ph_shift; s.dg = make_fastdiv((uint32_t)g);
#ifdef PXS_LAB
			{ static const int noph = [] { const char* e = getenv("PXS_CH_NOPH"); return e ? atoi(e) : 0; }(); if (noph) s.ph = nullptr; }
#endif
			set_tiles(s, T2, g, tp.M); s.bin = mk_blk(T1, bN, T2); s.bout = blocked_on();
			launch_any(s, ncl*npair*s.ntile, st);
		}
		{	StSigma s; memset(&s, 0, sizeof(s));
			s.fa = mk(fc_, g); s.fb = mk(fc_, g);
			s.Z = s2_.as<double2>(); s.ldZ = ldZ2; s.V = s1_.as<double2>(); s.ldV = ldV3; s.g = (int)g; s.g2 = (int)g2; s.sigma = sigma;
			set_tiles(s, T3, g2, tp.M); s.bin = mk_blk(T2, g, T3); s.bout = blocked_on();
			launch_any(s, ncl*npair*s.ntile, st);
		}
		{	StResize s; memset(&s, 0, sizeof(s));
			s.fa = mk(fc_, g2); s.fb = mk(fc_, ac);
			s.Y = s1_.as<double2>(); s.ldY = ldV3; s.Z = s2_.as<double2>(); s.ldZ = ldU4; s.g = (int)g; s.X1 = (int)tp.M; s.X2 = (int)tp.Ncc; s.kmax = lmax; s.nyq = 0;
			s.ph = nullptr; s.dg = make_fastdiv((uint32_t)g);
			set_tiles(s, T4, g, tp.Ncc); s.bin = mk_blk(T3, g2, T4); s.bout = blocked_on();
			launch_any(s, ncl*npair*s.ntile, st);
		}
		{	StSplit<0> s; memset(&s, 0, sizeof(s));
			s.fa = mk(fc_, g); s.fb = mk(fc_, 0);
			int T = tile_lines_for<StSplit<0>>(g, 0, 2*ac, 8); if (T < 2) T = 2; T -= T % 2;
			const int TH = T/2;
			set_tiles(s, T, (long)((ac/2 + 1 + TH - 1)/TH)*T, 0);
			s.TH = TH;
			s.U = s2_.as<double2>(); s.ldU = ldU4; s.a = (int)ac; s.g = (int)g; s.X = (int)tp.Ncc; s.mir_c = 0; s.nr_out = ncc; s.a_odd = spin & 1; s.ncol = nm; s.npair = (int)npair;
			s.out = leg_cc + (size_t)c0*nm*ldcc; s.ocstride = (long)nm*ldcc; s.dnp = make_fastdiv((uint32_t)npair); s.groups = 1; s.dgr = make_fastdiv(1);
			s.ld = ldcc; s.w = wcc; s.tab = nullptr; s.scale = 1.0; s.da = make_fastdiv((uint32_t)ac);
			s.bin = mk_blk(T4, g, T);
			launch_any(s, ncl*npair*s.ntile, st);
		}
	}
	PXS_HIP(hipGetLastError());
}

void FftChain::from_cc_adjoint(hipStream_t st, const ThetaPlan& tp, const double2* leg, long ldleg, int nr, int mir_c, double2* leg_cc, long ldcc, int ncc,
                               int nc, int nm, int spin, int lmax, const double2* ph_shift, const double2* w, const double2* wring)
{
	if (line_analysis(st, tp, false, leg, ldleg, nr, mir_c, leg_cc, ldcc, ncc, nc, nm, spin, lmax, ph_shift, nullptr, w, wring)) return;
	const long npair = (nm + 1)/2;
	const long g = tp.g, bN = tp.bN, ac = tp.ac;
	const long ldY1 = pad8(bN), ldU = pad8(g);
	const size_t need1 = (size_t)npair*g*ldY1, need2 = (size_t)npair*ac*ldU;
	const int cchunk = theta_comp_chunk(nc, need1, need2);
	const int T1 = tile_lines_for<StFirst>(g, 0, bN, 8), T2 = tile_lines_for<StResize>(bN, ac, g, 8);
	s1_.ensure(sizeof(double2)*need1*cchunk); s2_.ensure(sizeof(double2)*need2*cchunk);
	for (int c0 = 0; c0 < nc; c0 += cchunk) {
		const long ncl = std::min(cchunk, nc - c0);
		{	StFirst s; memset(&s, 0, sizeof(s));
			s.fa = mk(fc_, g); s.fb = mk(fc_, 0);
			s.src.leg = leg + (size_t)c0*nm*ldleg; s.src.cstride = (long)nm*ldleg; s.src.ld = ldleg; s.src.nr = nr; s.src.N = (int)tp.N; s.src.mir_c = mir_c; s.src.a_odd = spin & 1; s.src.ncol = nm;
			s.src.w = wring;
			s.b = (int)bN; s.Y = s1_.as<double2>(); s.ldY = ldY1; s.npair = (int)npair; s.dnp = make_fastdiv((uint32_t)npair);
			set_tiles(s, T1, bN, tp.N); s.bout = blocked_on();
			launch_any(s, ncl*npair*s.ntile, st);
		}
		{	StResize s; memset(&s, 0, sizeof(s));
			s.fa = mk(fc_, bN); s.fb = mk(fc_, ac);
			s.Y = s1_.as<double2>(); s.ldY = ldY1; s.Z = s2_.as<double2>(); s.ldZ = ldU; s.g = (int)g; s.X1 = (int)tp.N; s.X2 = (int)tp.Ncc; s.kmax = lmax; s.nyq = 0;
			s.ph = ph_shift; s.dg = make_fastdiv((uint32_t)g);
			set_tiles(s, T2, g, tp.Ncc); s.bin = mk_blk(T1, bN, T2); s.bout = blocked_on();
			launch_any(s, ncl*npair*s.ntile, st);
		}
		{	StSplit<0> s; memset(&s, 0, sizeof(s));
			s.fa = mk(fc_, g); s.fb = mk(fc_, 0);
			int T = tile_lines_for<StSplit<0>>(g, 0, 2*ac, 8); if (T < 2) T = 2; T -= T % 2;
			const int TH = T/2;
			set_tiles(s, T, (long)((ac/2 + 1 + TH - 1)/TH)*T, 0);
			s.TH = TH;
			s.U = s2_.as<double2>(); s.ldU = ldU; s.a = (int)ac; s.g = (int)g; s.X = (int)tp.Ncc; s.mir_c = 0; s.nr_out = ncc; s.a_odd = spin & 1; s.ncol = nm; s.npair = (int)npair;
			s.out = leg_cc + (size_t)c0*nm*ldcc; s.ocstride = (long)nm*ldcc; s.dnp = make_fastdiv((uint32_t)npair); s.groups = 1; s.dgr = make_fastdiv(1);
			s.ld = ldcc; s.w = w; s.tab = nullptr; s.scale = 1.0; s.da = make_fastdiv((uint32_t)ac);
			s.bin = mk_blk(T2, g, T);
			launch_any(s, ncl*npair*s.ntile, st);
		}
	}
	PXS_HIP(hipGetLastError());
}

void FftChain::to_cc_adjoint(hipStream_t st, const ThetaPlan& tp, const double2* leg_cc, long ldcc, int ncc, double2* h, long ldh, int nr, int mir_c,
                             int nc, int nm, int spin, int lmax, const double2* ph_shift, const double2* sigma, const double2* whalf, const double2* tab, double scale)
{
	const long npair = (nm + 1)/2;
	const long g = tp.g, bN = tp.bN, g2 = tp.g2, ac = tp.ac;
	const long ldY = pad8(ac), ldZ = pad8(g), ldV = pad8(g2);
	const size_t need1 = (size_t)npair*std::max(g*ldY, g*ldV), need2 = (size_t)npair*std::max(g2*ldZ, bN*ldZ);
	const int cchunk = theta_comp_chunk(nc, need1, need2);
	const int T1 = tile_lines_for<StFirst>(g, 0, ac, 8), T2 = tile_lines_for<StResize>(ac, g2, g, 8), T3 = tile_lines_for<StSigma>(g, g, g2, 8), T4 = tile_lines_for<StResize>(g2, bN, g, 8);
	s1_.ensure(sizeof(double2)*need1*cchunk); s2_.ensure(sizeof(double2)*need2*cchunk);
	for (int c0 = 0; c0 < nc; c0 += cchunk) {
		const long ncl = std::min(cchunk, nc - c0);
		{	StFirst s; memset(&s, 0, sizeof(s));
			s.fa = mk(fc_, g); s.fb = mk(fc_, 0);
			s.src.leg = leg_cc + (size_t)c0*nm*ldcc; s.src.cstride = (long)nm*ldcc; s.src.ld = ldcc; s.src.nr = ncc; s.src.N = (int)tp.Ncc; s.src.mir_c = 0; s.src.a_odd = spin & 1; s.src.ncol = nm;
			s.src.w = whalf;
			s.b = (int)ac; s.Y = s1_.as<double2>(); s.ldY = ldY; s.npair = (int)npair; s.dnp = make_fastdiv((uint32_t)npair);
			set_tiles(s, T1, ac, tp.Ncc); s.bout = blocked_on();
			launch_any(s, ncl*npair*s.ntile, st);
		}
		{	StResize s; memset(&s, 0, sizeof(s));
			s.fa = mk(fc_, ac); s.fb = mk(fc_, g2);
			s.Y = s1_.as<double2>(); s.ldY = ldY; s.Z = s2_.as<double2>(); s.ldZ = ldZ; s.g = (int)g; s.X1 = (int)tp.Ncc; s.X2 = (int)tp.M; s.kmax = lmax; s.nyq = 0;
			s.ph = nullptr; s.dg = make_fastdiv((uint32_t)g);
			set_tiles(s, T2, g, tp.M); s.bin = mk_blk(T1, ac, T2); s.bout = blocked_on();
			launch_any(s, ncl*npair*s.ntile, st);
		}
		{	StSigma s; memset(&s, 0, sizeof(s));
			s.fa = mk(fc_, g); s.fb = mk(fc_, g);
			s.Z = s2_.as<double2>(); s.ldZ = ldZ; s.V = s1_.as<double2>(); s.ldV = ldV; s.g = (int)g; s.g2 = (int)g2; s.sigma = sigma;
			set_tiles(s, T3, g2, tp.M); s.bin = mk_blk(T2, g, T3); s.bout = blocked_on();
			launch_any(s, ncl*npair*s.ntile, st);
		}
		{	StResize s; memset(&s, 0, sizeof(s));
			s.fa = mk(fc_, g2); s.fb = mk(fc_, bN);
			s.Y = s1_.as<double2>(); s.ldY = ldV; s.Z = s2_.as<double2>(); s.ldZ = ldZ; s.g = (int)g; s.X1 = (int)tp.M; s.X2 = (int)tp.N; s.kmax = tp.M > tp.N ? -1 : (int)(tp.M/2 - 1); s.nyq = 0; s.adj = 1;
			s.ph = ph_shift; s.dg = make_fastdiv((uint32_t)g);
			set_tiles(s, T4, g, tp.N); s.bin = mk_blk(T3, g2, T4);
			launch_any(s, ncl*npair*s.ntile, st);
		}
		{	StSplit<1> s; memset(&s, 0, sizeof(s));
			s.fa = mk(fc_, g); s.fb = mk(fc_, 0);
			int T = tile_lines_for<StSplit<1>>(g, 0, 2*npair, 8); if (T < 2) T = 2; T -= T % 2;
			set_tiles(s, T, bN*T, 0);
			s.TH = 0;
			s.U = s2_.as<double2>(); s.ldU = ldZ; s.a = (int)bN; s.g = (int)g; s.X = (int)tp.N; s.mir_c = mir_c; s.nr_out = nr; s.a_odd = spin & 1; s.ncol = nm; s.npair = (int)npair;
			const long groups = (npair + T/2 - 1)/(T/2);
			s.out = h + (size_t)c0*nr*ldh; s.ocstride = (long)nr*ldh; s.dnp = make_fastdiv((uint32_t)npair); s.groups = (int)groups; s.dgr = make_fastdiv((uint32_t)groups);
			s.ld = ldh; s.w = nullptr; s.tab = tab; s.scale = scale; s.da = make_fastdiv((uint32_t)bN); s.self_half = 1;
			launch_any(s, ncl*groups*bN, st);
		}
	}
	PXS_HIP(hipGetLastError());
}

void FftChain::from_cc(hipStream_t st, const ThetaPlan& tp, const double2* leg_cc, long ldcc, int ncc, double2* h, long ldh, int nr, int mir_c,
                       int nc, int nm, int spin, int lmax, const double2* ph_up, const double2* tab, double scale, const double2* wring)
{
	const long npair = (nm + 1)/2;
	const long gs = tp.gs, bs = tp.bs, aN = tp.aNs;
	const long ldY = pad8(bs), ldZ = pad8(gs);
	const size_t need1 = (size_t)npair*gs*ldY, need2 = (size_t)npair*aN*ldZ;
	const int cchunk = theta_comp_chunk(nc, need1, need2);
	const int T1 = tile_lines_for<StFirst>(gs, 0, bs, 8), T2 = tile_lines_for<StResize>(bs, aN, gs, 8);
	s1_.ensure(sizeof(double2)*need1*cchunk); s2_.ensure(sizeof(double2)*need2*cchunk);
	for (int c0 = 0; c0 < nc; c0 += cchunk) {
		const long ncl = std::min(cchunk, nc - c0);
		{	StFirst s; memset(&s, 0, sizeof(s));
			s.fa = mk(fc_, gs); s.fb = mk(fc_, 0);
			s.src.leg = leg_cc + (size_t)c0*nm*ldcc; s.src.cstride = (long)nm*ldcc; s.src.ld = ldcc; s.src.nr = ncc; s.src.N = (int)tp.Ncc; s.src.mir_c = 0; s.src.a_odd = spin & 1; s.src.ncol = nm;
			s.b = (int)bs; s.Y = s1_.as<double2>(); s.ldY = ldY; s.npair = (int)npair; s.dnp = make_fastdiv((uint32_t)npair);
			set_tiles(s, T1, bs, tp.Ncc); s.bout = blocked_on();
			launch_any(s, ncl*npair*s.ntile, st);
		}
		{	StResize s; memset(&s, 0, sizeof(s));
			s.fa = mk(fc_, bs); s.fb = mk(fc_, aN);
			s.Y = s1_.as<double2>(); s.ldY = ldY; s.Z = s2_.as<double2>(); s.ldZ = ldZ; s.g = (int)gs; s.X1 = (int)tp.Ncc; s.X2 = (int)tp.N; s.kmax = lmax; s.nyq = 0;
			s.ph = ph_up; s.dg = make_fastdiv((uint32_t)gs);
			set_tiles(s, T2, gs, tp.N); s.bin = mk_blk(T1, bs, T2);
			launch_any(s, ncl*npair*s.ntile, st);
		}
		{	StSplit<1> s; memset(&s, 0, sizeof(s));
			s.fa = mk(fc_, gs); s.fb = mk(fc_, 0);
			int T = tile_lines_for<StSplit<1>>(gs, 0, 2*npair, 8); if (T < 2) T = 2; T -= T % 2;
			set_tiles(s, T, aN*T, 0);
			s.TH = 0;
			s.U = s2_.as<double2>(); s.ldU = ldZ; s.a = (int)aN; s.g = (int)gs; s.X = (int)tp.N; s.mir_c = mir_c; s.nr_out = nr; s.a_odd = spin & 1; s.ncol = nm; s.npair = (int)npair;
			const long groups = (npair + T/2 - 1)/(T/2);
			s.out = h + (size_t)c0*nr*ldh; s.ocstride = (long)nr*ldh; s.dnp = make_fastdiv((uint32_t)npair); s.groups = (int)groups; s.dgr = make_fastdiv((uint32_t)groups);
			s.ld = ldh; s.w = wring; s.tab = tab; s.scale = scale; s.da = make_fastdiv((uint32_t)aN);
			launch_any(s, ncl*groups*aN, st);
		}
	}
	PXS_HIP(hipGetLastError());
}

bool FftChain::fft2_real(hipStream_t st, const void* in, int in_dtype, double2* out, long npre, long ny, long nx, bool forward, double scale) {
	Split sy;
	if (nx < 4 || ny < 4 || !split_balanced(ny, sy) || ((nphi_ != nx || !rings_ok()) && !plan_rings(nx))) return false;
	const long nm = nx/2 + 1, ldF = pad8(ny), a = std::min(sy.a, sy.b), b = ny/a, ldY = pad8(b);
	if (getenv("PXS_CHAIN_VERBOSE")) fprintf(stderr, "[pxsht] fft2_real %ld x %ld x %ld: rows %s, columns %ld x %ld\n", npre, ny, nx, describe().c_str(), a, b);
	PXS_REQUIRE(npre*nm < (1L << 31)/std::max<long>(a, b), "fft2_real: too many lines");
	s2_.ensure(sizeof(double2)*(size_t)npre*nm*ldF);
	MapDesc m; m.ptr = in; m.dtype = in_dtype; m.cstride = ny*nx; m.ring_off0 = 0; m.ring_stride = nx; m.pix_stride = 1; m.nring = (int)ny; m.nphi = nx;
	map2leg(st, m, (int)npre, (int)(nm - 1), s2_.as<double2>(), ldF, nullptr, 1.0);
	s1_.ensure(sizeof(double2)*(size_t)npre*nm*a*ldY);
	{	StFirst2D s; memset(&s, 0, sizeof(s));
		s.fa = mk(fc_, a); s.fb = mk(fc_, 0);
		s.src.leg = s2_.as<double2>(); s.src.cstride = nm*ldF; s.src.ld = ldF; s.src.nr = (int)ny; s.src.N = (int)ny; s.src.ncol = (int)nm; s.src.plain = 1;
		s.b = (int)b; s.Y = s1_.as<double2>(); s.ldY = ldY; s.npair = (int)nm; s.dnp = make_fastdiv((uint32_t)nm);
		set_tiles(s, tile_lines_for<StFirst2D>(a, 0, b, 8), b, ny);
		launch_any(s, npre*nm*s.ntile, st);
	}
	{	StColOut s; memset(&s, 0, sizeof(s));
		s.fa = mk(fc_, b); s.fb = mk(fc_, 0);
		int T = tile_lines_for<StColOut>(b, 0, nm, 8);
		set_tiles(s, T, a*T, 0);
		s.Y = s1_.as<double2>(); s.ldY = ldY; s.a = (int)a; s.nm = (int)nm; s.ny = (int)ny; s.nx = (int)nx; s.conj_out = forward ? 0 : 1; s.out = out; s.scale = scale;
		s.herm = 1; s.ldo = nx; s.ocomp = ny*nx;
		s.groups = (int)((nm + T - 1)/T); s.dgr = make_fastdiv((uint32_t)s.groups);
		launch_any(s, npre*s.groups*a, st);
	}
	PXS_HIP(hipGetLastError());
	return true;
}

bool FftChain::fft2_c2c(hipStream_t st, const double2* in, double2* out, long npre, long ny, long nx, bool forward, double scale) {
	Split sx, sy;
	if (nx < 4 || ny < 4 || !split_balanced(nx, sx) || !split_balanced(ny, sy)) return false;
	const long ax = std::min(sx.a, sx.b), bx = nx/ax, ay = std::min(sy.a, sy.b), by = ny/ay, ldF = pad8(ny);
	if (npre*std::max(nx, ny) >= (1L << 31)/512) return false;
	if (getenv("PXS_CHAIN_VERBOSE")) fprintf(stderr, "[pxsht] fft2_c2c %ld x %ld x %ld: rows %ld x %ld, columns %ld x %ld\n", npre, ny, nx, ax, bx, ay, by);
	s1_.ensure(sizeof(double2)*(size_t)npre*std::max(ny*ax*pad8(bx), nx*ay*pad8(by)));
	s2_.ensure(sizeof(double2)*(size_t)npre*nx*ldF);
	auto first = [&](const double2* src, long nlines, long ld, long n, long a, long b, int conj) {
		StFirst2D s; memset(&s, 0, sizeof(s));
		s.fa = mk(fc_, a); s.fb = mk(fc_, 0);
		s.src.leg = src; s.src.cstride = nlines*ld; s.src.ld = ld; s.src.nr = (int)n; s.src.N = (int)n; s.src.ncol = (int)nlines; s.src.plain = 1; s.src.conj = conj;
		s.b = (int)b; s.Y = s1_.as<double2>(); s.ldY = pad8(b); s.npair = (int)nlines; s.dnp = make_fastdiv((uint32_t)nlines);
		set_tiles(s, tile_lines_for<StFirst2D>(a, 0, b, 8), b, n);
		launch_any(s, npre*nlines*s.ntile, st);
	};
	auto second = [&](double2* dst, long nlines, long ldo, long ocomp, long a, long b, int conj, double sc) {
		StColOut s; memset(&s, 0, sizeof(s));
		s.fa = mk(fc_, b); s.fb = mk(fc_, 0);
		int T = tile_lines_for<StColOut>(b, 0, nlines, 8);
		set_tiles(s, T, a*T, 0);
		s.Y = s1_.as<double2>(); s.ldY = pad8(b); s.a = (int)a; s.nm = (int)nlines; s.ny = 0; s.nx = 0; s.conj_out = conj; s.herm = 0; s.out = dst; s.ldo = ldo; s.ocomp = ocomp; s.scale = sc;
		s.groups = (int)((nlines + T - 1)/T); s.dgr = make_fastdiv((uint32_t)s.groups);
		launch_any(s, npre*s.groups*a, st);
	};
	first(in, ny, nx, nx, ax, bx, forward ? 0 : 1);
	second(s2_.as<double2>(), ny, ldF, nx*ldF, ax, bx, 0, 1.0);
	first(s2_.as<double2>(), nx, ldF, ny, ay, by, 0);
	second(out, nx, nx, ny*nx, ay, by, forward ? 0 : 1, scale);
	PXS_HIP(hipGetLastError());
	return true;
}

}
```

### pixell_amd/csrc/fftchain.hpp

```cpp
#pragma once
#include "fft.hpp"
#include <tuple>
#include <map>
#include <mutex>
#include <memory>

namespace pxs {

struct Lds2;

struct Split { long a = 0, b = 0; };

struct ThetaPlan {
	bool ok = false;
	long N = 0, M = 0, Ncc = 0;
	long g = 0, bN = 0, g2 = 0, ac = 0;
	long gs = 0, bs = 0, aNs = 0;
};

class FftChain {
public:
	explicit FftChain(FftContext* fc) : fc_(fc) {}
	static bool sub_ok(long n);
	static bool sub_ok_theta(long n);
	static long pad8(long n) { return (n + 7) & ~7L; }
	bool plan_rings(long nphi);
	static ThetaPlan plan_theta(long N, int lmax);
	static long ducc_ncc(int lmax);
	bool rings_ok() const { return ra_.a > 0; }
	std::string describe() const { return "analysis " + std::to_string(ra_.a) + "x" + std::to_string(ra_.b) + ", synthesis " + std::to_string(rs_.a) + "x" + std::to_string(rs_.b); }

	struct MapDesc { const void* ptr; int dtype; long cstride, ring_off0, ring_stride, pix_stride; int nring; long nphi;
	                 long bstride = 0; int ncb = 0; };
	void map2leg(hipStream_t st, const MapDesc& m, int nc, int mmax, double2* leg, long ldleg, const double2* tab, double scale);
	void h2map(hipStream_t st, const double2* h, long ldh, const MapDesc& m, int nc, int mmax, long hcomp = 0);
	void to_cc(hipStream_t st, const ThetaPlan& tp, const double2* leg, long ldleg, int nr, int mir_c, double2* leg_cc, long ldcc, int ncc,
	           int nc, int nm, int spin, int lmax, const double2* ph_shift, const double2* sigma, const double2* wcc);
	void from_cc(hipStream_t st, const ThetaPlan& tp, const double2* leg_cc, long ldcc, int ncc, double2* h, long ldh, int nr, int mir_c,
	             int nc, int nm, int spin, int lmax, const double2* ph_up, const double2* tab, double scale, const double2* wring = nullptr);
	void from_cc_adjoint(hipStream_t st, const ThetaPlan& tp, const double2* leg, long ldleg, int nr, int mir_c, double2* leg_cc, long ldcc, int ncc,
	                     int nc, int nm, int spin, int lmax, const double2* ph_shift, const double2* w, const double2* wring = nullptr);
	void to_cc_adjoint(hipStream_t st, const ThetaPlan& tp, const double2* leg_cc, long ldcc, int ncc, double2* h, long ldh, int nr, int mir_c,
	                   int nc, int nm, int spin, int lmax, const double2* ph_shift, const double2* sigma, const double2* whalf, const double2* tab, double scale);
	bool fft2_real(hipStream_t st, const void* in, int in_dtype, double2* out, long npre, long ny, long nx, bool forward, double scale);
	bool fft2_c2c(hipStream_t st, const double2* in, double2* out, long npre, long ny, long nx, bool forward, double scale);
	bool line_analysis(hipStream_t st, const ThetaPlan& tp, bool has_mid, const double2* leg, long ldleg, int nr, int mir_c, double2* leg_cc, long ldcc, int ncc,
	                   int nc, int nm, int spin, int lmax, const double2* ph_shift, const double2* sigma, const double2* w, const double2* wring);
	static bool line_takes(const ThetaPlan& tp, bool has_mid);
	bool line_h2map(hipStream_t st, const double2* h, long ldh, const MapDesc& m, int nc, int mmax, long hcomp);
	static bool line_h2map_takes(long nphi, int mmax);
	size_t scratch_bytes() const { return s1_.bytes + s2_.bytes; }
	static void theta_scratch(const ThetaPlan& tp, int nm, int nc, int kind, size_t& b1, size_t& b2);
	void ring_scratch(long nring, int nc, bool analysis, size_t& b1, int mmax = -1) const;
	void reserve(size_t b1, size_t b2) { s1_.ensure(b1); s2_.ensure(b2); }
private:
	const double2* small_tw(long X, int n, int T);
	template<class S> void set_tiles(S& s, int T, long nlines, long X);
	template<class S> int tile_lines_for(long n_a, long n_b, long nlines, int mult, long tab_pts = -1);
	template<class S> void launch_any(S& s, long nblk, hipStream_t st);
	std::mutex mu_;
	std::map<std::tuple<long, int, int>, DevBuf> stw_;
	FftContext* fc_;
	Split ra_, rs_;
	long nphi_ = 0;
	DevBuf s1_, s2_;
	std::shared_ptr<struct ThetaLine> tl_;
};

struct MapAddr { void* ptr; int dtype; long cstride, bstride, off0, rstride, pstride; int nring, ncb; FastDiv dncb; };
inline MapAddr map_addr(const FftChain::MapDesc& m) {
	MapAddr a; a.ptr = const_cast<void*>(m.ptr); a.dtype = m.dtype; a.cstride = m.cstride; a.bstride = m.bstride; a.off0 = m.ring_off0; a.rstride = m.ring_stride; a.pstride = m.pix_stride; a.nring = m.nring;
	a.ncb = m.ncb > 0 ? m.ncb : (1 << 30); a.dncb = make_fastdiv((uint32_t)a.ncb);
	return a;
}

}
```

### pixell_amd/csrc/sht.hip

```cpp
#include "../../include/pxsht.h"
#include "fft.hpp"
#include "legendre.hpp"
#include "fftchain.hpp"
#include <map>
#include <memory>
#include <cmath>
#include <mutex>
#include <algorithm>

namespace pxs {

FftContext& fft_context(int device);
void fft_dense_lines(int device, hipStream_t st, long n, bool forward, long nlines, const double2* in, double2* out);
void fft_release_stream(int device, hipStream_t st);
const char* get_last_error();
struct PointsState;
PointsState* points_create(int ntheta, int nphi, int lmax, int mmax, int device, long npts, const double* d_loc, double eps, hipStream_t st);
void points_free(PointsState* s);
void points_run(PointsState* s, pxs_plan* grid, int spin, int mode, int adjoint, int nb, const AlmArg& alm, const MapArg& map, hipStream_t st);
int64_t points_query(const PointsState* s, const std::string& name);
void points_profile(PointsState* s, bool on);

typedef long double LDb;
static const LDb PIl = 3.141592653589793238462643383279502884L;
// ... 645 lines not shown
		FftStore sf; sf.ptr = (char*)m.ptr + esz(m.dtype)*p->ring_off0; sf.dtype = m.dtype;
		p->fc->exec(st, p->nphi, false, d, ld, sf);
	}
	p->prof.end(st, PXS_STAGE_RING_FFT);
	PXS_HIP(hipGetLastError());
}

void resample_to_cc(pxs_plan* p, hipStream_t st, const double2* leg_in, double2* leg_cc, int nc, int spin, long M, const double2* sigma, const double2* wcc) {
	const int nm = p->mmax+1, nr = p->nring;
	const long npair_all = (nm + 1)/2;
	const long chunk = std::max<long>(32, std::min<long>(npair_all, (long)(p->resample_chunk_bytes/(sizeof(double2)*M))));
	p->b1.ensure(sizeof(double2)*(size_t)chunk*std::max(p->N, p->Ncc));
	p->b2.ensure(sizeof(double2)*(size_t)chunk*M);
	p->prof.begin(st, PXS_STAGE_RESAMPLE);
	for (int c = 0; c < nc; c++)
	for (long p0 = 0; p0 < npair_all; p0 += chunk) {
		const long np = std::min<long>(chunk, npair_all - p0);
		const long m0 = 2*p0, nlines = std::min<long>(2*np, nm - m0);
		{
			FftDims d; d.n_i = np; d.is_i = nr; d.os_i = p->N; d.is_e = 1; d.os_e = 1;
			FftLoad ld; ld.ptr = leg_in + ((size_t)c*nm + m0)*nr; ld.mode = LD_MIRROR_PAIR; ld.ne = nr; ld.mir_c = p->mir_c;
			ld.par0 = (spin + (int)m0) & 1; ld.pair_lines = nlines;
			FftStore sf; sf.ptr = p->b1.p;
			p->fc->exec(st, p->N, true, d, ld, sf);
		}
		{
			FftDims d; d.n_i = np; d.is_i = p->N; d.os_i = M; d.is_e = 1; d.os_e = 1;
			FftLoad ld; ld.ptr = p->b1.p; ld.mode = LD_SPEC; ld.ne = p->N; ld.nyq_half = M > p->N ? 1 : 0; ld.kmax = M > p->N ? -1 : M/2 - 1; ld.mul = p->ph_shift.as<double2>();
			FftStore sf; sf.ptr = p->b2.p; sf.mul = sigma;
			p->fc->exec(st, M, false, d, ld, sf);
		}
		{
			FftDims d; d.n_i = np; d.is_i = M; d.os_i = M; d.is_e = 1; d.os_e = 1;
			FftLoad ld; ld.ptr = p->b2.p;
			FftStore sf; sf.ptr = p->b2.p; sf.two_sided_k = p->lmax;
			p->fc->exec(st, M, true, d, ld, sf);
		}
		{
			FftDims d; d.n_i = np; d.is_i = M; d.os_i = p->Ncc; d.is_e = 1; d.os_e = 1;
			FftLoad ld; ld.ptr = p->b2.p; ld.mode = LD_SPEC; ld.ne = M; ld.kmax = p->lmax;
			FftStore sf; sf.ptr = p->b1.p;
			p->fc->exec(st, p->Ncc, false, d, ld, sf);
		}
		{
			const long tot = np*p->ncc;
			hipLaunchKernelGGL(split_pair, dim3((unsigned)((tot+255)/256)), dim3(256), 0, st, (const double2*)p->b1.p,
				leg_cc + ((size_t)c*nm + m0)*p->ncc, p->ncc, p->Ncc, 0, np, nlines, (spin + (int)m0) & 1, wcc, 1.0);
		}
	}
	p->prof.end(st, PXS_STAGE_RESAMPLE);
	PXS_HIP(hipGetLastError());
}

void resample_to_cc_adjoint(pxs_plan* p, hipStream_t st, const double2* leg_cc, double2* leg_out, int nc, int spin, long M, const double2* sigma, const double2* wcc) {
	const int nm = p->mmax+1, nr = p->nring;
	const long chunk = std::max<long>(32, std::min<long>(nm, (long)(p->resample_chunk_bytes/(sizeof(double2)*M))));
	p->b1.ensure(sizeof(double2)*(size_t)chunk*std::max(p->N, p->Ncc));
	p->b2.ensure(sizeof(double2)*(size_t)chunk*M);
	p->prof.begin(st, PXS_STAGE_RESAMPLE);
	for (int c = 0; c < nc; c++)
	for (long m0 = 0; m0 < nm; m0 += chunk) {
		const long nl = std::min<long>(chunk, nm - m0);
		{
			FftDims d; d.n_i = nl; d.is_i = p->ncc; d.os_i = p->Ncc; d.is_e = 1; d.os_e = 1;
			FftLoad ld; ld.ptr = leg_cc + ((size_t)c*nm + m0)*p->ncc; ld.ne = p->ncc; ld.mul = wcc;
			FftStore sf; sf.ptr = p->b1.p;
			p->fc->exec(st, p->Ncc, true, d, ld, sf);
		}
		{
			FftDims d; d.n_i = nl; d.is_i = p->Ncc; d.os_i = M; d.is_e = 1; d.os_e = 1;
			FftLoad ld; ld.ptr = p->b1.p; ld.mode = LD_SPEC; ld.ne = p->Ncc; ld.kmax = p->lmax;
			FftStore sf; sf.ptr = p->b2.p; sf.mul = sigma;
			p->fc->exec(st, M, false, d, ld, sf);
		}
		{
			FftDims d; d.n_i = nl; d.is_i = M; d.os_i = M; d.is_e = 1; d.os_e = 1;
			FftLoad ld; ld.ptr = p->b2.p;
			FftStore sf; sf.ptr = p->b2.p; sf.two_sided_k = M > p->N ? p->N/2 : -1;
			p->fc->exec(st, M, true, d, ld, sf);
		}
		{
			FftDims d; d.n_i = nl; d.is_i = M; d.os_i = p->N; d.is_e = 1; d.os_e = 1;
			FftLoad ld; ld.ptr = p->b2.p; ld.mode = LD_SPEC_ADJ; ld.ne = M; ld.nyq_half = M > p->N ? 1 : 0; ld.kmax = M > p->N ? -1 : M/2 - 1; ld.mul = p->ph_shift.as<double2>();
			FftStore sf; sf.ptr = p->b1.p;
			p->fc->exec(st, p->N, false, d, ld, sf);
		}
		{
			const long tot = nl*nr;
			hipLaunchKernelGGL(fold_mirror, dim3((unsigned)((tot+255)/256)), dim3(256), 0, st, (const double2*)p->b1.p,
				leg_out + ((size_t)c*nm + m0)*nr, nr, p->N, p->mir_c, nl, (spin + (int)m0) & 1);
		}
	}
	p->prof.end(st, PXS_STAGE_RESAMPLE);
	PXS_HIP(hipGetLastError());
}

void resample_from_cc(pxs_plan* p, hipStream_t st, const double2* leg_cc, double2* leg_out, int nc, int spin, double2* h_out = nullptr) {
	const int nm = p->mmax+1, nr = p->nring;
	const long npair_all = (nm + 1)/2;
	const long chunk = std::max<long>(32, std::min<long>(npair_all, (long)(p->resample_chunk_bytes/(sizeof(double2)*p->N))));
	p->b1.ensure(sizeof(double2)*(size_t)chunk*std::max(p->N, p->Ncc));
	p->b2.ensure(sizeof(double2)*(size_t)chunk*p->N);
	p->prof.begin(st, PXS_STAGE_RESAMPLE);
	for (int c = 0; c < nc; c++)
	for (long p0 = 0; p0 < npair_all; p0 += chunk) {
		const long np = std::min<long>(chunk, npair_all - p0);
		const long m0 = 2*p0, nlines = std::min<long>(2*np, nm - m0);
		{
			FftDims d; d.n_i = np; d.is_i = p->ncc; d.os_i = p->Ncc; d.is_e = 1; d.os_e = 1;
			FftLoad ld; ld.ptr = leg_cc + ((size_t)c*nm + m0)*p->ncc; ld.mode = LD_MIRROR_PAIR; ld.ne = p->ncc; ld.mir_c = 0;
			ld.par0 = (spin + (int)m0) & 1; ld.pair_lines = nlines;
			FftStore sf; sf.ptr = p->b1.p;
			p->fc->exec(st, p->Ncc, true, d, ld, sf);
		}
		{
			FftDims d; d.n_i = np; d.is_i = p->Ncc; d.os_i = p->N; d.is_e = 1; d.os_e = 1;
			FftLoad ld; ld.ptr = p->b1.p; ld.mode = LD_SPEC; ld.ne = p->Ncc; ld.kmax = p->lmax; ld.mul = p->ph_up.as<double2>();
			FftStore sf; sf.ptr = p->b2.p;
			p->fc->exec(st, p->N, false, d, ld, sf);
		}
		if (h_out && np == npair_all) {
			dim3 grid((nm+31)/32, (nr+31)/32);
			hipLaunchKernelGGL(split_pair_transposed, grid, dim3(256), sizeof(double2)*32*33, st, (const double2*)p->b2.p,
				h_out + (size_t)c*nr*nm, nr, nm, p->N, p->mir_c, spin & 1, (const double2*)p->phase.p, 1.0/(double)p->Ncc);
		} else {
			const long tot = np*nr;
			hipLaunchKernelGGL(split_pair, dim3((unsigned)((tot+255)/256)), dim3(256), 0, st, (const double2*)p->b2.p,
				leg_out + ((size_t)c*nm + m0)*nr, nr, p->N, p->mir_c, np, nlines, (spin + (int)m0) & 1, (const double2*)nullptr, 1.0/(double)p->Ncc);
		}
	}
	p->prof.end(st, PXS_STAGE_RESAMPLE);
	PXS_HIP(hipGetLastError());
}

}

#define PXS_TRY try {
#define PXS_CATCH } catch (const pxs::Error& e) { pxs::set_last_error(e.what()); return e.code; } \
	catch (const std::exception& e) { pxs::set_last_error(e.what()); return pxs::PXS_ERR_ARG; } return 0;

extern "C" {

int pxs_grid_maxlmax(const char* geometry, int ntheta) { return grid_maxlmax(geometry ? geometry : "", ntheta); }

int pxs_gridweights(const char* geometry, int ntheta, double* out) {
	PXS_TRY
	PXS_REQUIRE(geometry && out && ntheta > 0, "pxs_gridweights: bad arguments");
	GridInfo gi = grid_info(geometry, ntheta);
	if (!gi.ok) throw Error(PXS_ERR_UNSUPPORTED, std::string("gridweights: unsupported geometry '") + geometry + "' (CC, F1, MW, MWflip, DH, F2)");
	if (grid_weights_only(geometry)) {
		const bool dh = std::string(geometry) == "DH";
		const std::vector<LDb> w = fejer2_weights(dh ? ntheta-1 : ntheta);
		if (dh) out[0] = 0;
		for (size_t j = 0; j < w.size(); j++) out[j + (dh ? 1 : 0)] = (double)(w[j]*2*PIl);
		return 0;
	}
	const long N = gi.N; const int n = ntheta;
	const LDb th0 = (LDb)gi.c*PIl/N;
	std::vector<LDb> v(N);
	const long K = (N-1)/2;
	if (N <= 4096) {
		for (long j = 0; j < N; j++) {
			LDb th = th0 + 2*PIl*j/N, s = (LDb)abs_sin_coef(0);
			for (long k = 2; k <= K; k += 2) s += 2*(-(2/PIl)/((LDb)k*k-1))*cosl(k*th);
			if (N % 2 == 0 && ((N/2) % 2) == 0) s += (-(2/PIl)/((LDb)(N/2)*(N/2)-1))*cosl((N/2)*(th-th0))*cosl((N/2)*th0);
			v[j] = s*PIl/N;
		}
	} else {
		std::vector<double2> c(N, make_double2(0, 0));
		c[0].x = (double)abs_sin_coef(0);
		for (long k = 2; k <= K; k += 2) {
			const LDb sk = -(2/PIl)/((LDb)k*k-1), a = (LDb)k*th0;
			c[k] = make_double2((double)(sk*cosl(a)), (double)(sk*sinl(a)));
			c[N-k] = make_double2(c[k].x, -c[k].y);
		}
		if (N % 2 == 0 && ((N/2) % 2) == 0) c[N/2] = make_double2((double)((-(2/PIl)/((LDb)(N/2)*(N/2)-1))*cosl((N/2)*th0)), 0.0);
		int dev = 0; PXS_HIP(hipGetDevice(&dev));
		DevBuf dc = upload(c);
		fft_dense_lines(dev, nullptr, N, false, 1, dc.as<double2>(), dc.as<double2>());
		PXS_HIP(hipStreamSynchronize(nullptr));
		PXS_HIP(hipMemcpy(c.data(), dc.p, sizeof(double2)*N, hipMemcpyDeviceToHost));
		for (long j = 0; j < N; j++) v[j] = (LDb)c[j].x*PIl/N;
	}
	for (int j = 0; j < n; j++) out[j] = 0;
	for (long jp = 0; jp < N; jp++) { long r = jp < n ? jp : ((-jp - gi.c) % N + N) % N; out[r] += (double)(v[jp]*2*PIl); }
	PXS_CATCH
}

int pxs_plan_grid2d(pxs_plan** plan, const char* geometry, int ntheta, int nphi, double phi0,
                    int flip_y, int flip_x, int lmax, int mmax, const uint64_t* mstart, int64_t lstride, int device)
{
	PXS_TRY
	PXS_REQUIRE(plan && geometry && ntheta > 0 && nphi > 0, "pxs_plan_grid2d: bad arguments");
	GridInfo gi = grid_info(geometry, ntheta);
	if (!gi.ok) throw Error(PXS_ERR_UNSUPPORTED, std::string("unsupported 2d geometry '") + geometry + "' (supported: CC, F1, MW, MWflip, DH, F2)");
	std::unique_ptr<pxs_plan> p(new pxs_plan());
	p->is_grid = true; p->geometry = geometry; p->nring = ntheta; p->nphi = nphi; p->phi0 = phi0;
	p->ring_stride = flip_y ? -(long)nphi : (long)nphi;
	p->pix_stride = flip_x ? -1 : 1;
	p->ring_off0 = (flip_y ? (long)(ntheta-1)*nphi : 0) + (flip_x ? (long)nphi-1 : 0);
	plan_common(p.get(), lmax, mmax, mstart, lstride, device);
	p->rs_map.build(grid_theta(geometry, ntheta)); p->rs_map.upload_all();
	if (grid_weights_only(geometry)) {
		std::vector<double> w(ntheta);
		if (pxs_gridweights(geometry, ntheta, w.data()) != 0) throw Error(PXS_ERR_ARG, get_last_error());
		std::vector<double2> wd(ntheta);
		for (int j = 0; j < ntheta; j++) wd[j] = make_double2(w[j]/nphi, 0.0);
		p->wring = upload(wd);
	} else if (lmax <= grid_maxlmax(geometry, ntheta)) setup_resampling(p.get());
	*plan = p.release();
	PXS_CATCH
}

int pxs_plan_rings(pxs_plan** plan, int nring, const double* theta, const uint64_t* nphi,
                   const double* phi0, const uint64_t* ringstart, int64_t pixstride,
                   int lmax, int mmax, const uint64_t* mstart, int64_t lstride, int device)
{
	PXS_TRY
	PXS_REQUIRE(plan && nring > 0 && theta && nphi && phi0 && ringstart, "pxs_plan_rings: bad arguments");
	std::unique_ptr<pxs_plan> p(new pxs_plan());
	p->is_grid = false; p->nring = nring; p->nphi = (int)nphi[0]; p->phi0 = phi0[0];
	p->ring_off0 = (long)ringstart[0];
	p->ring_stride = nring > 1 ? (long)ringstart[1] - (long)ringstart[0] : (long)nphi[0];
	for (int r = 0; r < nring; r++)
		if ((long)nphi[r] != p->nphi || std::fabs(phi0[r] - phi0[0]) > 1e-13 || (long)ringstart[r] != p->ring_off0 + r*p->ring_stride) p->general = true;
	if (!FftContext::supported(p->nphi)) p->general = true;
	{ const char* e = getenv("PXS_GENERAL_RINGS"); if (e && atoi(e) != 0) p->general = true; }
	p->pix_stride = pixstride;
	plan_common(p.get(), lmax, mmax, mstart, lstride, device);
	if (p->general) setup_general(p.get(), nring, nphi, phi0, ringstart);
	std::vector<LDb> th(nring);
	for (int r = 0; r < nring; r++) th[r] = theta[r];
	p->rs_map.build(th); p->rs_map.upload_all();
	{	static const bool on = [] { const char* e = lab_getenv("PXS_BAND_VIA_CC"); return e ? atoi(e) != 0 : true; }();
		if (on && !p->general && p->chain_rings && nring >= 2) {
			const LDb d = th[1] - th[0];
			const long n = d > 0 ? (long)llroundl(PIl/d) : 0;
			const long k0 = n > 0 ? (long)llroundl(th[0]*n/PIl - 0.5L) : -1;
			bool ok = n > nring && k0 >= 0 && k0 + nring <= n && lmax <= n - 1 && n < (1L << 30) && FftContext::supported(2*n);
			for (int r = 0; ok && r < nring; r++) ok = fabsl(th[r] - ((LDb)(k0 + r) + 0.5L)*PIl/n) < 1e-11L;
			if (ok) {
				p->band = true; p->geometry = "F1"; p->nfull = (int)n; p->row0 = (int)k0;
				setup_resampling(p.get());
				if (!p->chain_theta()) { p->band = false; p->nfull = 0; p->row0 = 0; p->ncc = 0; }
			}
		}
	}
	*plan = p.release();
	PXS_CATCH
}

int pxs_plan_points(pxs_plan** plan, const pxs_plan* g, int64_t npts, const double* d_loc, double epsilon, int device, void* stream)
{
	PXS_TRY
	PXS_REQUIRE(plan && g && npts >= 0 && (d_loc || npts == 0), "pxs_plan_points: bad arguments");
	PXS_REQUIRE(g->is_grid && g->geometry == "CC" && !g->pts && g->phi0 == 0 && g->ring_stride == g->nphi && g->pix_stride == 1,
		"pxs_plan_points: needs an unflipped CC grid plan with phi0 = 0");
	PXS_REQUIRE(g->nring >= g->lmax + 2 && g->nphi % 2 == 0 && g->nphi >= 2*g->mmax + 2, "pxs_plan_points: the CC grid needs ntheta >= lmax + 2 and an even nphi >= 2 mmax + 2");
	PXS_REQUIRE(FftContext::supported(2L*g->nring - 2) && FftContext::supported(g->nphi), "pxs_plan_points: CC grid sizes the FFT engine cannot transform");
	PXS_REQUIRE(epsilon >= 1e-13 && epsilon <= 0.1, "pxs_plan_points: epsilon must lie in [1e-13, 0.1]");
	PXS_REQUIRE(device == g->device, "pxs_plan_points: the grid plan lives on another device");
	PXS_HIP(hipSetDevice(device));
	std::unique_ptr<pxs_plan> p(new pxs_plan());
	p->device = device; p->lmax = g->lmax; p->mmax = g->mmax; p->lstride = g->lstride; p->pgrid = const_cast<pxs_plan*>(g);
	p->pts = points_create(g->nring, g->nphi, g->lmax, g->mmax, device, (long)npts, d_loc, epsilon, (hipStream_t)stream);
	*plan = p.release();
	PXS_CATCH
}

void pxs_plan_destroy(pxs_plan* plan) { delete plan; }

int pxs_plan_option(pxs_plan* p, const char* name, int64_t value) {
	PXS_TRY
	PXS_REQUIRE(p && name, "pxs_plan_option: null argument");
	std::lock_guard<std::mutex> plan_lock(p->call_mu);
	if (p->pts) {
		const std::string n(name);
		PXS_REQUIRE((n == "deterministic" || n == "profile") && (value == 0 || value == 1), "pxs_plan_option: a points plan takes 'deterministic' or 'profile' (0 or 1)");
		if (n == "deterministic") p->wk.deterministic = value != 0;
		else points_profile(p->pts, value != 0);
		return 0;
	}
	if (std::string(name) == "analysis") {
		PXS_REQUIRE(value >= 0 && value <= 2, "pxs_plan_option: analysis takes 0 (interpolant), 1 (weights) or 2 (ducc0)");
		p->ana_weights = (int)value;
	} else if (std::string(name) == "deterministic") {
		PXS_REQUIRE(value == 0 || value == 1, "pxs_plan_option: deterministic takes 0 or 1");
		p->wk.deterministic = value != 0;
	} else if (std::string(name) == "build_tables") {
		PXS_REQUIRE(value >= 0 && value <= p->lmax + 1, "pxs_plan_option: build_tables takes a spin");
		PXS_HIP(hipSetDevice(p->device));
		(void)p->table((int)value);
	} else throw Error(PXS_ERR_ARG, std::string("pxs_plan_option: unknown option '") + name + "'");
	PXS_CATCH
}

struct AnaSet { const ThetaPlan* tp; const double2* sigma; const double2* wcc; const double2* whalf; long M; bool fine; };
static AnaSet ana_set(const pxs_plan* p, bool allow_fine = true) {
	if (allow_fine && p->ana_weights != 0 && p->Mf > 0) return AnaSet{&p->tpf, p->sigma_f.as<double2>(), p->wcc_f.as<double2>(), p->whalf_f.as<double2>(), p->Mf, true};
	return AnaSet{&p->tp, p->sigma.as<double2>(), p->wcc.as<double2>(), p->whalf.as<double2>(), p->M, false};
}
static Route route_of(const pxs_plan* p, bool analysis, int spin, int mode, bool adjoint, const LegTables* tb);
static Route analysis_route_now(const pxs_plan* p) { return route_of(p, true, 0, PXS_MODE_STANDARD, false, nullptr); }
int pxs_plan_query(const pxs_plan* p, const char* name, int64_t* value) {
	PXS_TRY
	PXS_REQUIRE(p && name && value, "pxs_plan_query: null argument");
	const std::string n(name);
	if (p->pts) *value = points_query(p->pts, n);
	else if (n == "analysis_form") { const Route r = analysis_route_now(p); *value = (r.kind == R_RING_WEIGHTS || r.kind == R_CC_WEIGHTS) ? 1 : (r.fine ? 2 : 0); }
	else if (n == "ncc_circle") *value = p->ncc > 0 ? p->Ncc : 0;
	else if (n == "ducc_ncc_circle") *value = FftChain::ducc_ncc(p->lmax);
	else if (n == "theta_line") *value = analysis_route_now(p).line ? 1 : 0;
	else throw Error(PXS_ERR_ARG, std::string("pxs_plan_query: unknown name '") + name + "'");
	PXS_CATCH
}

int pxs_plan_info(const pxs_plan* p, int* nsyn, int* nana, int64_t* scratch) {
	if (!p) return PXS_ERR_ARG;
	if (nsyn) *nsyn = route_of(p, false, 2, PXS_MODE_STANDARD, false, nullptr).rs->nring;
	if (nana) *nana = p->ncc > 0 ? p->ncc : p->nring;
	if (scratch) *scratch = (int64_t)(p->leg.bytes + p->leg2.bytes + p->hbuf.bytes + p->b1.bytes + p->b2.bytes + p->wk.almt.bytes + p->wk.part.bytes + p->wk.mom.bytes);
	return 0;
}

int pxs_debug_theta_plan(int64_t N, int lmax, int64_t* out) {
	const ThetaPlan t = FftChain::plan_theta(N, lmax);
	const int64_t v[10] = {t.ok, t.g, t.bN, t.g2, t.M, t.ac, t.Ncc, t.gs, t.bs, t.aNs};
	for (int i = 0; i < 10; i++) out[i] = v[i];
	return 0;
}

int pxs_debug_chain(pxs_plan* p, int kind, int nc, int spin, int reps, double* ms) {
	PXS_TRY
	PXS_REQUIRE(p && ms && nc >= 1 && reps >= 1 && kind >= 0 && kind <= 4, "pxs_debug_chain: bad arguments");
	PXS_REQUIRE(p->chain_rings && (kind < 2 || p->chain_theta()), "pxs_debug_chain: the plan has no fused chain for this stage");
	PXS_HIP(hipSetDevice(p->device));
	std::lock_guard<std::mutex> plan_lock(p->call_mu);
	PlanUse use(p, nullptr);
	const size_t nm = (size_t)p->mmax + 1, nr = (size_t)p->nring, c16 = sizeof(double2);
	const long ldm = FftChain::pad8(p->nring), ldc = p->ld_cc(), ldh = p->ld_h();
	DevBuf dmap;
	if (kind < 2) { dmap.alloc(sizeof(double)*(size_t)nc*nr*p->nphi); PXS_HIP(hipMemset(dmap.p, 0, dmap.bytes)); }
	p->leg.ensure(c16*nc*nm*ldm); p->leg2.ensure(c16*nc*nm*std::max<long>(ldc, 8)); p->hbuf.ensure(c16*nc*nr*ldh);
	PXS_HIP(hipMemset(p->leg.p, 0, p->leg.bytes)); PXS_HIP(hipMemset(p->leg2.p, 0, p->leg2.bytes)); PXS_HIP(hipMemset(p->hbuf.p, 0, p->hbuf.bytes));
	hipStream_t st = nullptr;
	auto run = [&]() {
		const FftChain::MapDesc md = p->map_desc(MapArg{dmap.p, PX_F64, (long)nr*p->nphi, 0});
		switch (kind) {
		case 0: p->chain->map2leg(st, md, nc, p->mmax, p->leg.as<double2>(), ldm, p->phase.as<double2>(), 1.0); break;
		case 1: p->chain->h2map(st, p->hbuf.as<double2>(), ldh, md, nc, p->mmax); break;
		case 2: { AnaSet as = ana_set(p); if (!as.tp->ok) as = ana_set(p, false);
			p->chain->to_cc(st, *as.tp, p->leg.as<double2>(), ldm, p->nring, p->mir_c, p->leg2.as<double2>(), ldc, p->ncc, nc, (int)nm, spin, p->lmax,
				p->ph_shift.as<double2>(), as.sigma, as.wcc); } break;
		case 3: p->chain->from_cc(st, p->tp, p->leg2.as<double2>(), ldc, p->ncc, p->hbuf.as<double2>(), ldh, p->nring, p->mir_c, nc, (int)nm, spin, p->lmax,
				p->ph_up.as<double2>(), p->phase.as<double2>(), 1.0/(double)p->Ncc); break;
		default: p->chain->from_cc_adjoint(st, p->tp, p->leg.as<double2>(), ldm, p->nring, p->mir_c, p->leg2.as<double2>(), ldc, p->ncc, nc, (int)nm, spin, p->lmax,
				p->ph_shift.as<double2>(), p->wadj.as<double2>()); break;
		}
	};
	run(); PXS_HIP(hipStreamSynchronize(st));
	hipEvent_t e0, e1; PXS_HIP(hipEventCreate(&e0)); PXS_HIP(hipEventCreate(&e1));
	PXS_HIP(hipEventRecord(e0, st));
	for (int i = 0; i < reps; i++) run();
	PXS_HIP(hipEventRecord(e1, st)); PXS_HIP(hipEventSynchronize(e1));
	float t = 0; PXS_HIP(hipEventElapsedTime(&t, e0, e1));
	(void)hipEventDestroy(e0); (void)hipEventDestroy(e1);
	*ms = (double)t/reps;
	PXS_CATCH
}

int pxs_profile(pxs_plan* p, int enable) {
	PXS_TRY
	PXS_REQUIRE(p, "pxs_profile: null plan");
	p->prof.enabled = enable != 0;
	if (enable && !p->wk.count.p) { PXS_HIP(hipSetDevice(p->device)); p->wk.count.alloc(2*1024*sizeof(double)); PXS_HIP(hipMemset(p->wk.count.p, 0, p->wk.count.bytes)); }
	p->wk.count_on = enable != 0;
	PXS_CATCH
}

int pxs_profile_flops(pxs_plan* p, double* flops, int reset) {
	PXS_TRY
	PXS_REQUIRE(p && flops, "pxs_profile_flops: null argument");
	flops[0] = flops[1] = 0;
	if (!p->wk.count.p) return 0;
	PXS_HIP(hipSetDevice(p->device));
	PXS_HIP(hipDeviceSynchronize());
	std::vector<double> c(p->wk.count.bytes/sizeof(double)); PXS_HIP(hipMemcpy(c.data(), p->wk.count.p, p->wk.count.bytes, hipMemcpyDeviceToHost));
	for (size_t i = 0; i + 1 < c.size(); i += 2) { flops[0] += c[i]*128.0; flops[1] += c[i+1]*128.0; }
	if (reset) PXS_HIP(hipMemset(p->wk.count.p, 0, p->wk.count.bytes));
	PXS_CATCH
}

int pxs_profile_read(pxs_plan* p, double* ms, int* counts, int reset) {
	PXS_TRY
	PXS_REQUIRE(p && ms && counts, "pxs_profile_read: null argument");
	p->prof.read(ms, counts, PXS_NSTAGE, reset != 0);
	PXS_CATCH
}

static Route route_of(const pxs_plan* p, bool analysis, int spin, int mode, bool adjoint, const LegTables* tb) {
	Route r;
	const int nr = p->nring;
	const bool th = p->chain_theta();
	const long ldm = p->ld_map(), ldc = p->ld_cc(), ldh = p->ld_h();
	r.to_map = analysis ? adjoint : !adjoint; r.tb = tb;
	r.nc = analysis ? (spin == 0 ? 1 : 2) : ncomp_of(spin, mode, false); r.deriv1 = mode == PXS_MODE_DERIV1;
	r.rs = &p->rs_map; r.nr_th = nr; r.tp = &p->tp;
	auto use_h = [&](int rows) { r.nr_h = rows; r.ld_h = ldh; };
	auto form = [&](const AnaSet& as) { r.tp = as.tp; r.sigma = as.sigma; r.wcc = as.wcc; r.whalf = as.whalf; r.M = as.M; r.fine = as.fine; };
	if (!analysis) {
		const bool cc = (p->is_grid || (p->band && th)) && (spin == 0 ? p->syn_via_cc0 : p->syn_via_cc) && p->ncc > 0;
		static const bool adj_cc = [] { const char* e = lab_getenv("PXS_ADJ_VIA_CC"); return e ? atoi(e) != 0 : true; }();
		static const bool fuse = [] { const char* e = lab_getenv("PXS_FUSE_SPLIT"); return e ? atoi(e) != 0 : true; }();
		r.ld_leg = r.ld_leg_alloc = ldm;
		if (!cc || (adjoint && !(th && adj_cc))) { r.kind = R_DIRECT; if (!adjoint && !p->general) use_h(nr); }
		else {
			r.rs = &p->rs_cc; r.ld_leg2 = ldc; r.nr_th = p->band ? p->nfull : nr;
			if (adjoint) { r.kind = R_VIA_CC; r.theta = TH_FROM_CC_ADJ; r.ld_leg = r.ld_leg_alloc = p->band ? FftChain::pad8(p->nfull) : ldm; }
			else if (th) { r.kind = R_VIA_CC; r.theta = TH_FROM_CC; use_h(r.nr_th); r.ld_leg = 0; }
			else { r.kind = (fuse && !p->chain_rings) ? R_VIA_CC_UNFUSED_H : R_VIA_CC_UNFUSED; r.theta = TH_FROM_CC; use_h(nr); r.ld_leg = nr; }
		}
	} else if (p->wring.p) { r.kind = R_RING_WEIGHTS; }
	else if ((p->ana_weights == 1 || (p->ana_weights == 2 && p->geometry == "CC")) && (long)nr >= 2L*p->lmax + 2)
		r.kind = (th && p->ncc > 0) ? R_CC_WEIGHTS : R_RING_WEIGHTS;
	else {
		form(ana_set(p));
		auto adj_ana_fused = [] { const char* e = getenv("PXS_ADJ_ANA_FUSED"); return e ? atoi(e) != 0 : true; };
		r.kind = (th && (r.fine ? r.tp->ok : (!adjoint || adj_ana_fused()))) ? R_CHAIN : R_UNFUSED;
	}
	if (analysis) {
		if (r.kind == R_RING_WEIGHTS) { r.ld_leg = ldm; if (adjoint) use_h(nr); }
		else {
			r.rs = &p->rs_cc; r.ld_leg2 = r.kind == R_UNFUSED ? p->ncc : ldc;
			if (!adjoint || r.kind == R_UNFUSED) r.ld_leg = r.kind == R_UNFUSED ? nr : ldm;
			if (adjoint) use_h(nr);
			r.theta = r.kind == R_CC_WEIGHTS ? (adjoint ? TH_FROM_CC : TH_FROM_CC_ADJ) : (adjoint ? TH_TO_CC_ADJ : TH_TO_CC);
		}
		r.ld_leg_alloc = r.ld_leg;
	}
	const bool unfused = r.kind == R_VIA_CC_UNFUSED || r.kind == R_VIA_CC_UNFUSED_H || r.kind == R_UNFUSED;
	r.batched = !unfused;
	r.theta_fused = r.theta != TH_NONE && !unfused;
	r.line = r.theta_fused && r.theta <= TH_FROM_CC_ADJ && FftChain::line_takes(*r.tp, r.theta == TH_TO_CC);
	r.reserve_chain = p->chain_rings && r.kind != R_UNFUSED;
	return r;
}

static const double2* ring_weights(pxs_plan* p) {
	if (p->wring.p) return p->wring.as<double2>();
	if (!p->wgrid.p) {
		std::vector<double> w(p->nring);
		if (pxs_gridweights(p->geometry.c_str(), p->nring, w.data()) != 0) throw Error(PXS_ERR_ARG, get_last_error());
		std::vector<double2> wd(p->nring);
		for (int j = 0; j < p->nring; j++) wd[j] = make_double2(w[j]/p->nphi, 0.0);
		p->wgrid = upload(wd);
	}
	return p->wgrid.as<double2>();
}
static const double2* ring_weights_ext(pxs_plan* p) {
	const double2* w = ring_weights(p);
	if (p->geometry == "F1") return w;
	if (!p->wgrid_ext.p) {
		std::vector<double2> wd(p->nring);
		PXS_HIP(hipMemcpy(wd.data(), w, sizeof(double2)*p->nring, hipMemcpyDeviceToHost));
		for (int r = 0; r < p->nring; r++) { const long t = 2L*r + p->mir_c; if (t == 0 || t == p->N || t == 2*p->N) wd[r].x *= 2; }
		p->wgrid_ext = upload(wd);
	}
	return p->wgrid_ext.as<double2>();
}

static const double2* unit_weights_ext(pxs_plan* p) {
	if (p->geometry == "F1" || p->band) return nullptr;
	if (!p->wunit_ext.p) {
		std::vector<double2> wd(p->nring, make_double2(1, 0));
		for (int r = 0; r < p->nring; r++) { const long t = 2L*r + p->mir_c; if (t == 0 || t == p->N || t == 2*p->N) wd[r].x = 2; }
		p->wunit_ext = upload(wd);
	}
	return p->wunit_ext.as<double2>();
}

static void run_core(pxs_plan* p, const Route& r, int spin, int nb, const AlmArg& alm, const MapArg& map, hipStream_t st)
{
	const int nct = nb*r.nc, nr = p->nring, nm = p->mmax + 1;
	double2* leg = p->leg.as<double2>();
	switch (r.kind) {
	case R_VIA_CC_UNFUSED: case R_VIA_CC_UNFUSED_H: {
		PXS_REQUIRE(nb == 1, "internal: batched call on an unfused path");
		const bool to_h = r.kind == R_VIA_CC_UNFUSED_H;
		p->leg_syn(st, r, alm, 1);
		resample_from_cc(p, st, p->leg2.as<double2>(), leg, r.nc, spin, to_h ? p->hbuf.as<double2>() : nullptr);
		leg2map(p, st, r, to_h ? nullptr : leg, r.ld_leg, map, 1);
		return; }
	case R_UNFUSED:
		PXS_REQUIRE(nb == 1, "internal: batched call on an unfused path");
		if (r.to_map) {
			p->leg_syn(st, r, alm, 1);
			resample_to_cc_adjoint(p, st, p->leg2.as<double2>(), leg, r.nc, spin, r.M, r.sigma, r.wcc);
			leg2map(p, st, r, leg, r.ld_leg, map, 1);
		} else {
			map2leg(p, st, r, map, 1, leg);
			resample_to_cc(p, st, leg, p->leg2.as<double2>(), r.nc, spin, r.M, r.sigma, r.wcc);
			p->leg_ana(st, r, alm, 1);
		}
		return;
	default: break;
	}
	const double2* wleg = r.kind == R_RING_WEIGHTS ? ring_weights(p) : nullptr;
	const double2* wth = r.kind == R_CC_WEIGHTS ? (r.to_map ? ring_weights(p) : ring_weights_ext(p)) : (r.kind == R_VIA_CC && !r.to_map ? unit_weights_ext(p) : nullptr);
	auto weigh = [&] {
		if (!wleg) return;
		const long tot = (long)nct*nm*nr;
		hipLaunchKernelGGL(scale_rings, dim3((unsigned)((tot+255)/256)), dim3(256), 0, st, leg, (long)nct*nm, nr, r.ld_leg, wleg);
		PXS_HIP(hipGetLastError()); };
	if (r.to_map) {
		p->leg_syn(st, r, alm, nb);
		weigh();
		if (r.theta != TH_NONE) p->run_theta(st, r, nct, spin, wth);
		leg2map(p, st, r, r.theta != TH_NONE ? nullptr : leg, r.ld_leg, map, nb);
	} else {
		if (r.nr_th > nr) {
			PXS_HIP(hipMemsetAsync(p->leg.p, 0, sizeof(double2)*(size_t)nct*nm*r.ld_leg, st));
			leg += p->row0;
		}
		map2leg(p, st, r, map, nb, leg);
		weigh();
		if (r.theta != TH_NONE) p->run_theta(st, r, nct, spin, wth);
		p->leg_ana(st, r, alm, nb);
	}
}

static void reserve_call(pxs_plan* p, const Route& r, int nb) {
	const Route::Scratch s = r.scratch(p, nb);
	p->wk.almt.ensure(s.almt); p->wk.mom.ensure(s.mom);
	p->leg.ensure(s.leg); p->leg2.ensure(s.leg2); p->hbuf.ensure(s.h);
	if (r.reserve_chain) p->chain->reserve(std::max(s.c1, s.r1), s.c2);
}

static int batch_chunk(const pxs_plan* p, int nbatch, int ncm) {
	if (nbatch <= 1 || !p->chain_rings) return 1;
	const size_t per_map = sizeof(double2)*(size_t)ncm*((size_t)(p->mmax+1)*(p->nring + (p->ncc > 0 ? p->ncc : 0))*2 + (size_t)p->nring*p->nphi);
	static const size_t budget_env = [] { const char* e = getenv("PXS_BATCH_GB"); return (size_t)(e ? atol(e) : 0) << 30; }();
	size_t budget = budget_env ? budget_env : (size_t)64 << 30;
	if (!budget_env) {
		size_t fr = 0, tot = 0;
		const size_t held = p->leg.bytes + p->leg2.bytes + p->hbuf.bytes + (p->chain ? p->chain->scratch_bytes() : 0);
		if (hipMemGetInfo(&fr, &tot) == hipSuccess && fr > 0) budget = std::min(budget, std::max<size_t>((size_t)4 << 30, held + (size_t)(0.4*(double)fr)));
	}
	const int cap = (int)std::max<size_t>(1, std::min<size_t>((size_t)nbatch, budget/std::max<size_t>(per_map, 1)));
	if (ncm == 1 && cap >= 8 && nbatch > cap) {
		const int cap8 = cap & ~7, npass = (nbatch + cap8 - 1)/cap8;
		return std::min(cap8, (((nbatch + npass - 1)/npass + 7)/8)*8);
	}
	const int npass = (nbatch + cap - 1)/cap;
	return (nbatch + npass - 1)/npass;
}

static void run_call(pxs_plan* p, bool analysis, int spin, int mode, int adjoint, int nbatch, const AlmArg& alm, const MapArg& map, hipStream_t st) {
	const Route r = route_of(p, analysis, spin, mode, adjoint != 0, &p->table(spin));
	const int chunk = r.batched ? batch_chunk(p, nbatch, r.nc) : 1;
	if (getenv("PXS_CHAIN_VERBOSE")) fprintf(stderr, "[pxsht] %s route %s, adjoint %d, spin %d, analysis option %d, %d maps in passes of %d\n", analysis ? "analysis" : "synthesis", ROUTE_NAMES[r.kind], adjoint, spin, p->ana_weights, nbatch, chunk);
	reserve_call(p, r, std::min(chunk, nbatch));
	for (int b0 = 0; b0 < nbatch; b0 += chunk) run_core(p, r, spin, std::min(chunk, nbatch - b0), alm.from(b0), map.from(b0), st);
}

int pxs_synthesis(pxs_plan* p, int spin, int mode, int adjoint, int nbatch,
                  void* alm, int alm_dtype, int64_t alm_cstride, int64_t alm_bstride,
                  void* map, int map_dtype, int64_t map_cstride, int64_t map_bstride, void* stream)
{
	PXS_TRY
	PXS_REQUIRE(p && alm && map, "pxs_synthesis: null argument");
	std::lock_guard<std::mutex> plan_lock(p->call_mu);
	PXS_REQUIRE(spin >= 0 && spin <= p->lmax + 1, "pxs_synthesis: bad spin");
	PXS_REQUIRE(mode == PXS_MODE_STANDARD || (mode == PXS_MODE_DERIV1 && spin == 1), "DERIV1 needs spin 1");
	PXS_REQUIRE(map_dtype == PX_F32 || map_dtype == PX_F64, "map must be float32 or float64");
	PXS_REQUIRE(nbatch >= 1, "pxs_synthesis: nbatch must be >= 1");
	PXS_HIP(hipSetDevice(p->device));
	hipStream_t st = (hipStream_t)stream;
	PlanUse use(p, st);
	const AlmArg a{alm, alm_dtype, (long)alm_cstride, (long)alm_bstride}; const MapArg m{map, map_dtype, (long)map_cstride, (long)map_bstride};
	if (p->pts) points_run(p->pts, p->pgrid, spin, mode, adjoint, nbatch, a, m, st);
	else run_call(p, false, spin, mode, adjoint, nbatch, a, m, st);
	PXS_CATCH
}

int pxs_analysis(pxs_plan* p, int spin, int adjoint, int nbatch,
                 void* map, int map_dtype, int64_t map_cstride, int64_t map_bstride,
                 void* alm, int alm_dtype, int64_t alm_cstride, int64_t alm_bstride, void* stream)
{
	PXS_TRY
	PXS_REQUIRE(p && alm && map, "pxs_analysis: null argument");
	std::lock_guard<std::mutex> plan_lock(p->call_mu);
	PXS_REQUIRE(p->is_grid, "pxs_analysis needs a grid2d plan");
	PXS_REQUIRE(map_dtype == PX_F32 || map_dtype == PX_F64, "map must be float32 or float64");
	PXS_REQUIRE(nbatch >= 1, "pxs_analysis: nbatch must be >= 1");
	if (p->lmax > grid_maxlmax(p->geometry, p->nring)) throw Error(PXS_ERR_ARG, "too few rings for analysis up to requested lmax");
	PXS_HIP(hipSetDevice(p->device));
	hipStream_t st = (hipStream_t)stream;
	PlanUse use(p, st);
	run_call(p, true, spin, PXS_MODE_STANDARD, adjoint, nbatch, AlmArg{alm, alm_dtype, (long)alm_cstride, (long)alm_bstride}, MapArg{map, map_dtype, (long)map_cstride, (long)map_bstride}, st);
	PXS_CATCH
}

}
```

Baseline: 3.210.

## Add compile-time specialized chain FFT kernels for common sizes and tile shapes

```diff
diff --git a/pixell_amd/csrc/chain_static_table.hpp b/pixell_amd/csrc/chain_static_table.hpp
--- /dev/null
+++ b/pixell_amd/csrc/chain_static_table.hpp
@@ -0,0 +1,115 @@
+using F8 = StaticFft<8, 8>;
+using F10 = StaticFft<10, 5, 2>;
+using F15 = StaticFft<15, 5, 3>;
+using F16 = StaticFft<16, 8, 2>;
+using F21 = StaticFft<21, 7, 3>;
+using F25 = StaticFft<25, 5, 5>;
+using F32 = StaticFft<32, 8, 4>;
+using F42 = StaticFft<42, 7, 6>;
+using F48 = StaticFft<48, 8, 6>;
+using F64 = StaticFft<64, 8, 8>;
+using F72 = StaticFft<72, 9, 8>;
+using F90 = StaticFft<90, 9, 5, 2>;
+using F96 = StaticFft<96, 8, 6, 2>;
+using F112 = StaticFft<112, 7, 8, 2>;
+using F120 = StaticFft<120, 5, 3, 8>;
+using F126 = StaticFft<126, 9, 7, 2>;
+using F135 = StaticFft<135, 9, 5, 3>;
+using F144 = StaticFft<144, 9, 8, 2>;
+using F150 = StaticFft<150, 5, 5, 6>;
+using F160 = StaticFft<160, 5, 8, 4>;
+using F168 = StaticFft<168, 7, 3, 8>;
+using F200 = StaticFft<200, 5, 5, 8>;
+using F216 = StaticFft<216, 9, 3, 8>;
+using F225 = StaticFft<225, 9, 5, 5>;
+using F252 = StaticFft<252, 9, 7, 4>;
+using F256 = StaticFft<256, 8, 8, 4>;
+using F270 = StaticFft<270, 9, 5, 6>;
+using F300 = StaticFft<300, 5, 5, 6, 2>;
+using F336 = StaticFft<336, 7, 8, 6>;
+using G3 = StaticFft<3, 3>;
+using G8 = F8;
+using G40 = StaticFft<40, 5, 8>;
+using G45 = StaticFft<45, 5, 3, 3>;
+using G75 = StaticFft<75, 5, 5, 3>;
+using G80 = StaticFft<80, 5, 8, 2>;
+using G90 = StaticFft<90, 5, 3, 6>;
+using G135 = StaticFft<135, 5, 3, 3, 3>;
+using G180 = StaticFft<180, 5, 6, 6>;
+using G240 = StaticFft<240, 5, 8, 6>;
+using G256 = F256;
+using G288 = StaticFft<288, 8, 6, 6>;
+using G320 = StaticFft<320, 5, 8, 8>;
+static const std::vector<StaticEntry>& static_table() {
+	static const std::vector<StaticEntry> t = {
+		PXS_CS(StFirst, F8, NoFft, 136)
+		PXS_CS(StFirst, F8, NoFft, 256)
+		PXS_CS(StFirst, F64, NoFft, 16)
+		PXS_CS(StFirst, F64, NoFft, 32)
+		PXS_CS(StFirst, F72, NoFft, 32)
+		PXS_CS(StFirst, F96, NoFft, 24)
+		PXS_CS(StFirst, F160, NoFft, 16)
+		PXS_CS(StResize, F16, F32, 64)
+		PXS_CS(StResize, F25, F42, 56)
+		PXS_CS(StResize, F32, F16, 64)
+		PXS_CS(StResize, F32, F32, 64)
+		PXS_CS(StResize, F42, F21, 56)
+		PXS_CS(StResize, F112, F150, 16)
+		PXS_CS(StResize, F126, F270, 8)
+		PXS_CS(StResize, F135, F256, 8)
+		PXS_CS(StResize, F168, F300, 8)
+		PXS_CS(StResize, F225, F252, 8)
+		PXS_CS(StResize, F225, F336, 7)
+		PXS_CS(StResize, F252, F126, 8)
+		PXS_CS(StResize, F256, F270, 8)
+		PXS_CS(StResize, F270, F135, 8)
+		PXS_CS(StResize, F270, F252, 8)
+		PXS_CS(StResize, F336, F168, 7)
+		PXS_CS(StSigma, F8, F8, 272)
+		PXS_CS(StSigma, F48, F48, 48)
+		PXS_CS(StSigma, F64, F64, 32)
+		PXS_CS(StSigma, F72, F72, 32)
+		PXS_CS(StSigma, F96, F96, 24)
+		PXS_CS(StSigma, F160, F160, 16)
+		PXS_CS(StSplit<0>, F8, NoFft, 272)
+		PXS_CS(StSplit<0>, F48, NoFft, 48)
+		PXS_CS(StSplit<0>, F64, NoFft, 32)
+		PXS_CS(StSplit<0>, F72, NoFft, 32)
+		PXS_CS(StSplit<0>, F96, NoFft, 24)
+		PXS_CS(StSplit<0>, F160, NoFft, 16)
+		PXS_CS(StSplit<1>, F8, NoFft, 320)
+		PXS_CS(StSplit<1>, F64, NoFft, 40)
+		PXS_CS(StSplit<1>, F72, NoFft, 32)
+		PXS_CS(StRingA1, G3, NoFft, 80)
+		PXS_CS(StRingA1, G8, NoFft, 256)
+		PXS_CS(StRingA1, G40, NoFft, 48)
+		PXS_CS(StRingA1, G45, NoFft, 48)
+		PXS_CS(StRingA1, G90, NoFft, 16)
+		PXS_CS(StRingA1, G180, NoFft, 16)
+		PXS_CS(StRingA2, G45, NoFft, 56)
+		PXS_CS(StRingA2, G80, NoFft, 32)
+		PXS_CS(StRingA2, G240, NoFft, 8)
+		PXS_CS(StRingA2, G256, NoFft, 8)
+		PXS_CS(StRingS1, G45, NoFft, 40)
+		PXS_CS(StRingS1, G240, NoFft, 8)
+		PXS_CS(StRingS1, G256, NoFft, 8)
+		PXS_CS(StRingS1, G288, NoFft, 8)
+		PXS_CS(StRingS1, G320, NoFft, 8)
+		PXS_CS(StRingS2, G8, NoFft, 256)
+		PXS_CS(StRingS2, G40, NoFft, 48)
+		PXS_CS(StRingS2, G45, NoFft, 48)
+		PXS_CS(StRingS2, G75, NoFft, 32)
+		PXS_CS(StRingS2, G135, NoFft, 16)
+		PXS_CS(StColOut, F15, NoFft, 128)
+		PXS_CS(StColOut, F15, NoFft, 168)
+		PXS_CS(StColOut, F16, NoFft, 152)
+		PXS_CS(StColOut, F120, NoFft, 16)
+		PXS_CS(StColOut, F150, NoFft, 16)
+		PXS_CS(StColOut, F216, NoFft, 8)
+		PXS_CS(StFirst2D, F10, NoFft, 16)
+		PXS_CS(StFirst2D, F15, NoFft, 16)
+		PXS_CS(StFirst2D, F144, NoFft, 16)
+		PXS_CS(StFirst2D, F200, NoFft, 8)
+	};
+	return t;
+}
diff --git a/pixell_amd/csrc/fft.hip b/pixell_amd/csrc/fft.hip
--- a/pixell_amd/csrc/fft.hip
+++ b/pixell_amd/csrc/fft.hip
@@ -341,7 +341,7 @@
 }
 
 struct FftSub {
-	int n; std::vector<int> fac; bool generic = false;
+	int n; std::vector<int> fac, hperm; bool generic = false;
 	DevBuf perm, tw, d_pass;
 	PassDesc pass[FFT_MAXFAC]; int nfac = 0;
 };
@@ -466,7 +466,7 @@
 		perm[j] = (int)pos;
 	}
 	std::vector<double2> tw; twiddles(n, tw);
-	s->perm = upload(perm); s->tw = upload(tw);
+	s->perm = upload(perm); s->tw = upload(tw); s->hperm = perm;
 	s->d_pass = upload(std::vector<PassDesc>(s->pass, s->pass + FFT_MAXFAC));
 	subs_[key] = s;
 	return s;
@@ -475,7 +475,7 @@
 FftContext::SubView FftContext::view(long n, int maxr) {
 	auto s = sub(n, true, maxr);
 	SubView v; v.n = s->n; v.nfac = s->nfac; v.ns = s->n | 1; v.generic = s->generic ? 1 : 0;
-	v.pass = s->d_pass.p; v.perm = s->perm.as<int>(); v.tw = s->tw.as<double2>();
+	v.pass = s->d_pass.p; v.perm = s->perm.as<int>(); v.tw = s->tw.as<double2>(); v.hfac = s->fac.data(); v.hperm = s->hperm.data();
 	return v;
 }
 
diff --git a/pixell_amd/csrc/fft.hpp b/pixell_amd/csrc/fft.hpp
--- a/pixell_amd/csrc/fft.hpp
+++ b/pixell_amd/csrc/fft.hpp
@@ -50,7 +50,7 @@
 	void exec(hipStream_t st, long n, bool forward, const FftDims& d, const FftLoad& ld, const FftStore& stf);
 	static long good_size(long n);
 	static bool supported(long n, std::string* why = nullptr);
-	struct SubView { int n, nfac, ns, generic; const void* pass; const int* perm; const double2* tw; };
+	struct SubView { int n, nfac, ns, generic; const void* pass; const int* perm; const double2* tw; const int* hfac; const int* hperm; };
 	SubView view(long n, int maxr = 1000);
 	const double2* twiddle_table(long n) { return bigtw(n); }
 	void release_stream(hipStream_t st) { std::lock_guard<std::mutex> g(mu_); temps_.erase(st); }
diff --git a/pixell_amd/csrc/fft_static_dev.hpp b/pixell_amd/csrc/fft_static_dev.hpp
--- /dev/null
+++ b/pixell_amd/csrc/fft_static_dev.hpp
@@ -0,0 +1,82 @@
+#pragma once
+#include "fft_dev.hpp"
+
+namespace pxs {
+
+static constexpr int SDIV_MAX = 4096;
+constexpr int sdiv_shift(int D) { int s = 13; while ((1 << (s - 13)) < D) s++; return s; }
+template<int D> __device__ __forceinline__ uint32_t sdiv(uint32_t x) {
+	if constexpr (D <= 1) return x;
+	else if constexpr ((D & (D - 1)) == 0) return x / (uint32_t)D;
+	else {
+		constexpr int s = sdiv_shift(D);
+		constexpr uint32_t M = (1u << s)/D + 1;
+#ifdef PXS_HOST_SIM
+		return (x*M) >> s;
+#else
+		return __umul24(x, M) >> s;
+#endif
+	}
+}
+
+template<int N, int... Rs> struct StaticFft {
+	static constexpr int n = N, ns = N | 1, nfac = (int)sizeof...(Rs);
+	static_assert(N >= 2 && (Rs * ... * 1) == N, "StaticFft: the radices do not multiply to N");
+	static constexpr int radix(int p) { constexpr int r[] = {Rs...}; return r[p]; }
+	static constexpr int L(int p) { int l = 1; for (int i = 0; i < p; i++) l *= radix(i); return l; }
+	static constexpr int tws(int p) { return N/(L(p)*radix(p)); }
+	static constexpr int perm_host(int j) {
+		int t = j, pos = 0;
+		for (int p = nfac - 1; p >= 0; p--) { const int i = t % radix(p); t /= radix(p); pos += i*L(p); }
+		return pos;
+	}
+	template<int P = nfac - 1> static __device__ __forceinline__ uint32_t perm(uint32_t t) {
+		if constexpr (P == 0) return t;
+		else { const uint32_t q = sdiv<radix(P)>(t); return (t - q*radix(P))*L(P) + perm<P - 1>(q); }
+	}
+};
+struct NoFft {
+	static constexpr int n = 0, ns = 1, nfac = 0;
+	static constexpr int radix(int) { return 1; }
+	static constexpr int perm_host(int j) { return j; }
+	template<int P = 0> static __device__ __forceinline__ uint32_t perm(uint32_t t) { return t; }
+};
+
+template<class F, int P, int NT, int T> __device__ __forceinline__ void static_pass(double2* buf, const double2* tw) {
+	constexpr int R = F::radix(P), L = F::L(P), TWS = F::tws(P), nb = F::n/R, total = T*nb, iters = (total + NT - 1)/NT;
+	static_assert(iters*NT <= SDIV_MAX, "static_pass: index range of sdiv");
+	static_assert(R == 2 || R == 3 || R == 4 || R == 5 || R == 6 || R == 7 || R == 8 || R == 9, "static_pass: radix not compiled in");
+#pragma unroll
+	for (int it = 0; it < iters; it++) {
+		const uint32_t b = threadIdx.x + it*NT;
+		if (total % NT == 0 || b < (uint32_t)total) {
+			const uint32_t t = sdiv<nb>(b), bb = b - t*nb, blk = sdiv<L>(bb), q = bb - blk*L;
+			double2* p = buf + (t*F::ns + bb + blk*(L*(R - 1)));
+			double2 v[R];
+#pragma unroll
+			for (int i = 0; i < R; i++) v[i] = p[i*L];
+			if constexpr (L > 1) {
+				const uint32_t step = q*TWS;
+#pragma unroll
+				for (int i = 1; i < R; i++) v[i] = cmul(v[i], tw[i*step]);
+			}
+			if constexpr (R == 6 || R == 8 || R == 9) {
+				constexpr int A = R == 8 ? 4 : 3, B = R == 9 ? 3 : 2;
+				butterfly_comp<A, B>(v);
+#pragma unroll
+				for (int k = 0; k < R; k++) p[k*L] = v[B*(k % A) + k/A];
+			} else {
+				butterfly<R>(v);
+#pragma unroll
+				for (int i = 0; i < R; i++) p[i*L] = v[i];
+			}
+		}
+	}
+	PXS_LDS_BARRIER();
+}
+
+template<class F, int NT, int T, int P = 0> __device__ __forceinline__ void lds_fft_static(double2* buf, const double2* tw) {
+	if constexpr (P < F::nfac) { static_pass<F, P, NT, T>(buf, tw); lds_fft_static<F, NT, T, P + 1>(buf, tw); }
+}
+
+}
diff --git a/pixell_amd/csrc/fftchain.hip b/pixell_amd/csrc/fftchain.hip
--- a/pixell_amd/csrc/fftchain.hip
+++ b/pixell_amd/csrc/fftchain.hip
@@ -1,5 +1,6 @@
 #include "fftchain.hpp"
 #include "fft_dev.hpp"
+#include "fft_static_dev.hpp"
 #include "chain_dev.hpp"
 #include <algorithm>
 #include <set>
@@ -169,6 +170,7 @@
 };
 
 struct StFirst2D : StFirst {
+	static constexpr int SID = 10;
 	static constexpr bool R7 = false;
 	static constexpr int PFI = 2;
 	__device__ __forceinline__ const void* pfaddr(const TileC& c, int i) const {
@@ -481,6 +483,131 @@
 	}
 };
 
+template<class S, class FA, class FB, int T, int NT> __global__ PXS_CH_BOUNDS void chain_kernel_static(const S s)
+{
+	PXS_SHARED(double2, lds);
+	constexpr int na = FA::n, nb = FB::n;
+	static_assert(S::TWO == (nb > 0), "chain_kernel_static: second transform");
+	constexpr int nlast = S::TWO ? nb : na, nslast = S::TWO ? FB::ns : FA::ns;
+	constexpr bool same_tw = S::TWO && nb == na;
+	constexpr int LA = (T*na + NT - 1)/NT, LB = (T*nb + NT - 1)/NT, LS = (T*nlast + NT - 1)/NT;
+	static_assert(LA*NT <= SDIV_MAX && LB*NT <= SDIV_MAX && LS*NT <= SDIV_MAX, "chain_kernel_static: index range of sdiv");
+	double2* twa = lds; double2* twb = same_tw ? lds : lds + na; double2* twx = lds + na + (same_tw ? 0 : nb); double2* buf = twx + (S::HAS_TW ? nlast : 0);
+	TileC c;
+	if (!s.decode((int)blockIdx.x, c)) return;
+	const bool have_tw = S::HAS_TW && s.btw != nullptr;
+	int pf_val = 0;
+	{
+		double2 v[LA]; int pos[LA];
+#pragma unroll
+		for (int u = 0; u < LA; u++) {
+			const uint32_t idx = threadIdx.x + u*NT; pos[u] = -1;
+			if ((T*na) % NT == 0 || idx < (uint32_t)(T*na)) {
+				uint32_t li, e;
+				if (S::LOAD_LINE_FAST) { e = sdiv<T>(idx); li = idx - e*T; }
+				else { li = sdiv<na>(idx); e = idx - li*na; }
+				v[u] = s.load(c, (int)li, (int)e);
+				if (S::INV_A) v[u].y = -v[u].y;
+				pos[u] = (int)(li*FA::ns + FA::perm(e));
+			}
+		}
+		if ((S::LOADK == 0 || S::PFI > 0) && s.pf > 0 && (long)blockIdx.x + s.pf < (long)gridDim.x) {
+			TileC c2;
+			if (s.decode((int)blockIdx.x + s.pf, c2)) {
+				if (S::LOADK == 0) {
+					constexpr int per = (na*16 + 127) >> 7; const uint32_t i = threadIdx.x;
+					if (i < (uint32_t)(T*per)) {
+						const uint32_t li = sdiv<per>(i), seg = i - li*per;
+						const double2* r = s.row(c2, (int)li);
+						if (r) pf_val = *reinterpret_cast<const int*>(reinterpret_cast<const char*>(r) + seg*128);
+					}
+				} else {
+#pragma unroll
+					for (int it = 0; it < S::PFI; it++) {
+						const void* q = s.pfaddr(c2, (int)threadIdx.x + it*NT);
+						if (q) pf_val += *reinterpret_cast<const int*>(q);
+					}
+				}
+			}
+		}
+#pragma unroll
+		for (int k0 = 0; k0 < na; k0 += NT) { const int k = k0 + (int)threadIdx.x; if (k < na) twa[k] = s.fa.tw[k]; }
+		if constexpr (S::TWO && !same_tw) {
+#pragma unroll
+			for (int k0 = 0; k0 < nb; k0 += NT) { const int k = k0 + (int)threadIdx.x; if (k < nb) twb[k] = s.fb.tw[k]; }
+		}
+		if (have_tw) {
+#pragma unroll
+			for (int k0 = 0; k0 < nlast; k0 += NT) { const int k = k0 + (int)threadIdx.x; if (k < nlast) twx[k] = s.btw[(long)c.t0*k]; }
+		}
+#pragma unroll
+		for (int u = 0; u < LA; u++) if (pos[u] >= 0) buf[pos[u]] = v[u];
+	}
+	PXS_LDS_BARRIER();
+	lds_fft_static<FA, NT, T>(buf, twa);
+	if constexpr (S::TWO) {
+		double2 v[LB]; int pos[LB];
+#pragma unroll
+		for (int u = 0; u < LB; u++) {
+			const uint32_t idx = threadIdx.x + u*NT; pos[u] = -1;
+			if ((T*nb) % NT == 0 || idx < (uint32_t)(T*nb)) {
+				const uint32_t e = sdiv<T>(idx), li = idx - e*T;
+				{ const double2* Al = buf + li*FA::ns; v[u] = s.mid(c, (int)li, (int)e, [&](int k) { return Al[k]; }); }
+				if (S::INV_B) v[u].y = -v[u].y;
+				pos[u] = (int)(li*FB::ns + FB::perm(e));
+			}
+		}
+		PXS_LDS_BARRIER();
+#pragma unroll
+		for (int u = 0; u < LB; u++) if (pos[u] >= 0) buf[pos[u]] = v[u];
+		PXS_LDS_BARRIER();
+		lds_fft_static<FB, NT, T>(buf, twb);
+	}
+	{
+#pragma unroll
+		for (int u = 0; u < LS; u++) {
+			const uint32_t idx = threadIdx.x + u*NT;
+			if ((T*nlast) % NT == 0 || idx < (uint32_t)(T*nlast)) {
+				uint32_t li, e;
+				if (S::STORE_LINE_FAST) { e = sdiv<T>(idx); li = idx - e*T; } else { li = sdiv<nlast>(idx); e = idx - li*nlast; }
+				double2 w = make_double2(1, 0);
+				if (have_tw) w = cmul(twx[e], s.tws[S::STORE_LINE_FAST ? idx : e*T + li]);
+				s.store(c, (int)li, (int)e, [&](int l2, int e2) { return buf[l2*nslast + e2]; }, w);
+			}
+		}
+	}
+#ifndef PXS_HOST_SIM
+	if (S::LOADK == 0 || S::PFI > 0) asm volatile("" :: "v"(pf_val));
+#endif
+}
+
+struct StaticEntry {
+	int sid, na, nb, T, maxr; std::vector<int> ra, rb; std::vector<int> pa, pb;
+	void (*launch)(const void* s, long nblk, size_t sh, hipStream_t st);
+};
+template<class S, class FA, class FB, int T> static void launch_static(const void* sp, long nblk, size_t sh, hipStream_t st) {
+	const S& s = *static_cast<const S*>(sp);
+#ifndef PXS_HOST_SIM
+	static const bool once = [] { (void)hipFuncSetAttribute((const void*)chain_kernel_static<S, FA, FB, T, S::NT>, hipFuncAttributeMaxDynamicSharedMemorySize, 160*1024 - 256); return true; }();
+	(void)once;
+#endif
+	hipLaunchKernelGGL((chain_kernel_static<S, FA, FB, T, S::NT>), dim3((unsigned)nblk), dim3(S::NT), sh, st, s);
+}
+template<class F> static std::vector<int> radices_of() { std::vector<int> r; for (int p = 0; p < F::nfac; p++) r.push_back(F::radix(p)); return r; }
+template<class F> static std::vector<int> perm_of() { std::vector<int> r; for (int j = 0; j < F::n; j++) r.push_back(F::perm_host(j)); return r; }
+template<class S, class FA, class FB, int T> static StaticEntry static_entry() {
+	static_assert((long)T*(FA::n > FB::n ? FA::n : FB::n) <= S::PTS, "static chain stage: tile too large");
+	return StaticEntry{S::SID, FA::n, FB::n, T, S::MAXR, radices_of<FA>(), radices_of<FB>(), perm_of<FA>(), perm_of<FB>(), &launch_static<S, FA, FB, T>};
+}
+#define PXS_CS(S, FA, FB, T) static_entry<S, FA, FB, T>(),
+#include "chain_static_table.hpp"
+#undef PXS_CS
+static const StaticEntry* static_find(int sid, int na, int nb, int T) {
+	for (const StaticEntry& e : static_table()) if (e.sid == sid && e.na == na && e.nb == nb && e.T == T) return &e;
+	return nullptr;
+}
+static bool static_enabled() { const char* e = getenv("PXS_CHAIN_STATIC"); return e ? atoi(e) != 0 : true; }
+
 static bool smooth235(long n) { if (n < 1) return false; for (int p : {2, 3, 5}) while (n % p == 0) n /= p; return n == 1; }
 bool FftChain::sub_ok(long n) { return n >= 2 && n <= CH_NMAX && smooth235(n); }
 
@@ -494,6 +621,13 @@
 	constexpr int nofft = 0;
 #endif
 	static const int nspad = [] { const char* e = lab_getenv("PXS_CH_NS_PAD"); return e ? atoi(e) : 0; }();
+	if (getenv("PXS_CHAIN_VERBOSE")) {
+		static std::mutex mu; static std::set<std::pair<long, int>> seen; std::lock_guard<std::mutex> g(mu);
+		if (seen.insert(std::make_pair(n, maxr)).second) {
+			std::string r; for (int p = 0; p < v.nfac; p++) r += " " + std::to_string(v.hfac[p]);
+			fprintf(stderr, "[pxsht] chain fft n=%ld maxr=%d: radices%s\n", n, maxr, r.c_str());
+		}
+	}
 	f.n = v.n; f.nfac = nofft ? 0 : v.nfac; f.ns = v.ns + nspad; f.generic = v.generic; f.pass = (const PassDesc*)v.pass; f.perm = v.perm; f.tw = v.tw; f.dn = make_fastdiv((uint32_t)n);
 	return f;
 }
@@ -545,8 +679,17 @@
 
 static const int F2_RADICES[] = {2, 3, 4, 5, 6, 8, 9};
 
-template<class S> static void launch_stage(const S& s, long nblk, hipStream_t st) {
+template<class S> static const StaticEntry* static_for(const S& s) {
+	const StaticEntry* e = static_find(S::SID, s.fa.n, s.fb.n, s.T);
+	if (!e || s.bin.Tw > 0 || s.fa.ns != (s.fa.n | 1) || s.fa.nfac != (int)e->ra.size()) return nullptr;
+	if (S::TWO && (s.fb.ns != (s.fb.n | 1) || s.fb.nfac != (int)e->rb.size())) return nullptr;
+	return e;
+}
+template<class S> static void launch_stage(const S& s, long nblk, hipStream_t st, std::vector<ChainShape>* dry) {
 	if (nblk <= 0) return;
+	const StaticEntry* se = static_for(s);
+	if (dry) { dry->push_back(ChainShape{S::SID, s.fa.n, s.fb.n, s.T, se != nullptr}); return; }
+	if (!static_enabled()) se = nullptr;
 	PXS_REQUIRE((long)s.T*std::max(s.fa.n, s.fb.n) <= S::PTS, "internal: chain tile too large");
 	PXS_REQUIRE(nblk < (1L << 31), "internal: chain grid too large");
 	size_t sh = sizeof(double2)*((size_t)s.fa.n + (S::TWO && s.fb.n == s.fa.n ? 0 : s.fb.n) + (S::HAS_TW ? std::max(s.fa.n, s.fb.n) : 0) + (size_t)s.T*std::max(s.fa.ns, s.fb.ns) + 2);
@@ -558,8 +701,9 @@
 	if (getenv("PXS_CHAIN_VERBOSE")) {
 		static std::mutex mu; static std::set<std::tuple<int, int, int, int>> seen; std::lock_guard<std::mutex> g(mu);
 		if (seen.insert(std::make_tuple(S::SID, s.fa.n, s.fb.n, s.T)).second)
-			fprintf(stderr, "[pxsht] chain stage %d: na=%d nb=%d T=%d LDS %.1f KiB -> %d WG/CU by LDS, %ld workgroups\n", S::SID, s.fa.n, s.fb.n, s.T, sh/1024.0, (int)((160*1024)/sh), nblk);
-	}
+			fprintf(stderr, "[pxsht] chain stage %d: na=%d nb=%d T=%d LDS %.1f KiB -> %d WG/CU by LDS, %ld workgroups, static %d\n", S::SID, s.fa.n, s.fb.n, s.T, sh/1024.0, (int)((160*1024)/sh), nblk, se ? 1 : 0);
+	}
+	if (se) { se->launch(&s, nblk, sh, st); return; }
 #ifndef PXS_HOST_SIM
 #ifdef PXS_CH_NT2
 	static const long mask2 = [] { const char* e = lab_getenv("PXS_CH_NT2_MASK"); return e ? strtol(e, nullptr, 0) : 0L; }();
@@ -582,7 +726,31 @@
 	if (S::PTS > CH_TILE_PTS && T < mult && (long)mult*std::max(n_a, n_b) <= S::PTS && nlines >= mult) T = mult;
 	return T;
 }
-template<class S> void FftChain::launch_any(S& s, long nblk, hipStream_t st) { launch_stage(s, nblk, st); }
+template<class S> void FftChain::launch_any(S& s, long nblk, hipStream_t st) {
+	if (!dry_) static_check(S::MAXR);
+	launch_stage(s, nblk, st, dry_);
+}
+
+int FftChain::static_check(int maxr) {
+	std::lock_guard<std::mutex> g(mu_);
+	if (maxr > 0 && checked_.count(maxr)) return (int)static_table().size();
+	for (const StaticEntry& e : static_table()) {
+		if (maxr > 0 && e.maxr != maxr) continue;
+		for (int which = 0; which < 2; which++) {
+			const int n = which ? e.nb : e.na; if (n <= 0) continue;
+			const std::vector<int>& r = which ? e.rb : e.ra; const std::vector<int>& pm = which ? e.pb : e.pa;
+			const auto v = fc_->view(n, e.maxr);
+			bool ok = !v.generic && v.nfac == (int)r.size() && v.ns == (n | 1);
+			for (int p = 0; ok && p < v.nfac; p++) ok = v.hfac[p] == r[p];
+			for (int j = 0; ok && j < n; j++) ok = v.hperm[j] == pm[j];
+			PXS_REQUIRE(ok, "static chain table: the plan compiled for length " + std::to_string(n) + " (stage " + std::to_string(e.sid) + ") is not the one the FFT engine plans");
+		}
+	}
+	if (maxr > 0) checked_.insert(maxr);
+	return (int)static_table().size();
+}
+bool FftChain::static_has(int sid, int na, int nb, int T) { return static_find(sid, na, nb, T) != nullptr; }
+void FftChain::static_shapes(std::vector<ChainShape>& out) { for (const StaticEntry& e : static_table()) out.push_back(ChainShape{e.sid, e.na, e.nb, e.T, true}); }
 
 static bool split_balanced(long n, Split& s, long amax = 320) {
 	long best = 0; double bestc = 1e300;
@@ -673,7 +841,7 @@
 	const long npair_all = (m.nring + 1)/2, a = ra_.a, b = ra_.b, ldY = pad8(b);
 	int T2 = tile_lines_for<StRingA2>(b, 0, 2*npair_all, 8, b); if (T2 < 2) T2 = 2; T2 -= T2 % 2;
 	const long qchunk = ring_chunk(npair_all, (long)sizeof(double2)*nc*a*ldY, T2/2);
-	s1_.ensure(sizeof(double2)*(size_t)nc*qchunk*a*ldY);
+	ensure1(sizeof(double2)*(size_t)nc*qchunk*a*ldY);
 	for (long q_lo = 0; q_lo < npair_all; q_lo += qchunk) {
 		const long npair = std::min(qchunk, npair_all - q_lo);
 		const int nring = m.nring - (int)(2*q_lo);
@@ -694,16 +862,16 @@
 			launch_any(s, (long)nc*s.groups*a, st);
 		}
 	}
-	PXS_HIP(hipGetLastError());
+	if (!dry_) PXS_HIP(hipGetLastError());
 }
 
 void FftChain::h2map(hipStream_t st, const double2* h, long ldh, const MapDesc& m, int nc, int mmax, long hcomp) {
 	PXS_REQUIRE(rings_ok() && m.nphi == nphi_, "internal: ring chain not planned");
-	if (line_h2map(st, h, ldh, m, nc, mmax, hcomp)) return;
+	if (dry_ ? line_h2map_takes(nphi_, mmax) : line_h2map(st, h, ldh, m, nc, mmax, hcomp)) return;
 	const long npair_all = (m.nring + 1)/2, a = rs_.a, b = rs_.b, ldY = pad8(b);
 	const long qchunk = ring_chunk(npair_all, (long)sizeof(double2)*nc*a*ldY, 1);
 	const int T1 = tile_lines_for<StRingS1>(a, 0, b, 8, 2*a), T2 = tile_lines_for<StRingS2>(b, 0, a, 16, b);
-	s1_.ensure(sizeof(double2)*(size_t)nc*qchunk*a*ldY);
+	ensure1(sizeof(double2)*(size_t)nc*qchunk*a*ldY);
 	for (long q_lo = 0; q_lo < npair_all; q_lo += qchunk) {
 		const long npair = std::min(qchunk, npair_all - q_lo);
 		const int nring = m.nring - (int)(2*q_lo);
@@ -722,7 +890,7 @@
 			launch_any(s, (long)nc*npair*s.ntile, st);
 		}
 	}
-	PXS_HIP(hipGetLastError());
+	if (!dry_) PXS_HIP(hipGetLastError());
 }
 
 static int theta_comp_chunk(int nc, size_t need1_per_comp, size_t need2_per_comp) {
@@ -749,14 +917,14 @@
 void FftChain::to_cc(hipStream_t st, const ThetaPlan& tp, const double2* leg, long ldleg, int nr, int mir_c, double2* leg_cc, long ldcc, int ncc,
                      int nc, int nm, int spin, int lmax, const double2* ph_shift, const double2* sigma, const double2* wcc)
 {
-	if (line_analysis(st, tp, true, leg, ldleg, nr, mir_c, leg_cc, ldcc, ncc, nc, nm, spin, lmax, ph_shift, sigma, wcc, nullptr)) return;
+	if (dry_ ? line_takes(tp, true) : line_analysis(st, tp, true, leg, ldleg, nr, mir_c, leg_cc, ldcc, ncc, nc, nm, spin, lmax, ph_shift, sigma, wcc, nullptr)) return;
 	const long npair = (nm + 1)/2;
 	const long g = tp.g, bN = tp.bN, g2 = tp.g2, ac = tp.ac;
 	const long ldY1 = pad8(bN), ldZ2 = pad8(g), ldV3 = pad8(g2), ldU4 = pad8(g);
 	const size_t need1 = (size_t)npair*std::max(g*ldY1, g*ldV3), need2 = (size_t)npair*std::max(g2*ldZ2, ac*ldU4);
 	const int cchunk = theta_comp_chunk(nc, need1, need2);
 	const int T1 = tile_lines_for<StFirst>(g, 0, bN, 8), T2 = tile_lines_for<StResize>(bN, g2, g, 8), T3 = tile_lines_for<StSigma>(g, g, g2, 8), T4 = tile_lines_for<StResize>(g2, ac, g, 8);
-	s1_.ensure(sizeof(double2)*need1*cchunk); s2_.ensure(sizeof(double2)*need2*cchunk);
+	ensure1(sizeof(double2)*need1*cchunk); ensure2(sizeof(double2)*need2*cchunk);
 	for (int c0 = 0; c0 < nc; c0 += cchunk) {
 		const long ncl = std::min(cchunk, nc - c0);
 		{	StFirst s; memset(&s, 0, sizeof(s));
@@ -803,20 +971,20 @@
 			launch_any(s, ncl*npair*s.ntile, st);
 		}
 	}
-	PXS_HIP(hipGetLastError());
+	if (!dry_) PXS_HIP(hipGetLastError());
 }
 
 void FftChain::from_cc_adjoint(hipStream_t st, const ThetaPlan& tp, const double2* leg, long ldleg, int nr, int mir_c, double2* leg_cc, long ldcc, int ncc,
                                int nc, int nm, int spin, int lmax, const double2* ph_shift, const double2* w, const double2* wring)
 {
-	if (line_analysis(st, tp, false, leg, ldleg, nr, mir_c, leg_cc, ldcc, ncc, nc, nm, spin, lmax, ph_shift, nullptr, w, wring)) return;
+	if (dry_ ? line_takes(tp, false) : line_analysis(st, tp, false, leg, ldleg, nr, mir_c, leg_cc, ldcc, ncc, nc, nm, spin, lmax, ph_shift, nullptr, w, wring)) return;
 	const long npair = (nm + 1)/2;
 	const long g = tp.g, bN = tp.bN, ac = tp.ac;
 	const long ldY1 = pad8(bN), ldU = pad8(g);
 	const size_t need1 = (size_t)npair*g*ldY1, need2 = (size_t)npair*ac*ldU;
 	const int cchunk = theta_comp_chunk(nc, need1, need2);
 	const int T1 = tile_lines_for<StFirst>(g, 0, bN, 8), T2 = tile_lines_for<StResize>(bN, ac, g, 8);
-	s1_.ensure(sizeof(double2)*need1*cchunk); s2_.ensure(sizeof(double2)*need2*cchunk);
+	ensure1(sizeof(double2)*need1*cchunk); ensure2(sizeof(double2)*need2*cchunk);
 	for (int c0 = 0; c0 < nc; c0 += cchunk) {
 		const long ncl = std::min(cchunk, nc - c0);
 		{	StFirst s; memset(&s, 0, sizeof(s));
@@ -847,7 +1015,7 @@
 			launch_any(s, ncl*npair*s.ntile, st);
 		}
 	}
-	PXS_HIP(hipGetLastError());
+	if (!dry_) PXS_HIP(hipGetLastError());
 }
 
 void FftChain::to_cc_adjoint(hipStream_t st, const ThetaPlan& tp, const double2* leg_cc, long ldcc, int ncc, double2* h, long ldh, int nr, int mir_c,
@@ -859,7 +1027,7 @@
 	const size_t need1 = (size_t)npair*std::max(g*ldY, g*ldV), need2 = (size_t)npair*std::max(g2*ldZ, bN*ldZ);
 	const int cchunk = theta_comp_chunk(nc, need1, need2);
 	const int T1 = tile_lines_for<StFirst>(g, 0, ac, 8), T2 = tile_lines_for<StResize>(ac, g2, g, 8), T3 = tile_lines_for<StSigma>(g, g, g2, 8), T4 = tile_lines_for<StResize>(g2, bN, g, 8);
-	s1_.ensure(sizeof(double2)*need1*cchunk); s2_.ensure(sizeof(double2)*need2*cchunk);
+	ensure1(sizeof(double2)*need1*cchunk); ensure2(sizeof(double2)*need2*cchunk);
 	for (int c0 = 0; c0 < nc; c0 += cchunk) {
 		const long ncl = std::min(cchunk, nc - c0);
 		{	StFirst s; memset(&s, 0, sizeof(s));
@@ -902,7 +1070,7 @@
 			launch_any(s, ncl*groups*bN, st);
 		}
 	}
-	PXS_HIP(hipGetLastError());
+	if (!dry_) PXS_HIP(hipGetLastError());
 }
 
 void FftChain::from_cc(hipStream_t st, const ThetaPlan& tp, const double2* leg_cc, long ldcc, int ncc, double2* h, long ldh, int nr, int mir_c,
@@ -914,7 +1082,7 @@
 	const size_t need1 = (size_t)npair*gs*ldY, need2 = (size_t)npair*aN*ldZ;
 	const int cchunk = theta_comp_chunk(nc, need1, need2);
 	const int T1 = tile_lines_for<StFirst>(gs, 0, bs, 8), T2 = tile_lines_for<StResize>(bs, aN, gs, 8);
-	s1_.ensure(sizeof(double2)*need1*cchunk); s2_.ensure(sizeof(double2)*need2*cchunk);
+	ensure1(sizeof(double2)*need1*cchunk); ensure2(sizeof(double2)*need2*cchunk);
 	for (int c0 = 0; c0 < nc; c0 += cchunk) {
 		const long ncl = std::min(cchunk, nc - c0);
 		{	StFirst s; memset(&s, 0, sizeof(s));
@@ -943,7 +1111,7 @@
 			launch_any(s, ncl*groups*aN, st);
 		}
 	}
-	PXS_HIP(hipGetLastError());
+	if (!dry_) PXS_HIP(hipGetLastError());
 }
 
 bool FftChain::fft2_real(hipStream_t st, const void* in, int in_dtype, double2* out, long npre, long ny, long nx, bool forward, double scale) {
@@ -952,10 +1120,10 @@
 	const long nm = nx/2 + 1, ldF = pad8(ny), a = std::min(sy.a, sy.b), b = ny/a, ldY = pad8(b);
 	if (getenv("PXS_CHAIN_VERBOSE")) fprintf(stderr, "[pxsht] fft2_real %ld x %ld x %ld: rows %s, columns %ld x %ld\n", npre, ny, nx, describe().c_str(), a, b);
 	PXS_REQUIRE(npre*nm < (1L << 31)/std::max<long>(a, b), "fft2_real: too many lines");
-	s2_.ensure(sizeof(double2)*(size_t)npre*nm*ldF);
+	ensure2(sizeof(double2)*(size_t)npre*nm*ldF);
 	MapDesc m; m.ptr = in; m.dtype = in_dtype; m.cstride = ny*nx; m.ring_off0 = 0; m.ring_stride = nx; m.pix_stride = 1; m.nring = (int)ny; m.nphi = nx;
 	map2leg(st, m, (int)npre, (int)(nm - 1), s2_.as<double2>(), ldF, nullptr, 1.0);
-	s1_.ensure(sizeof(double2)*(size_t)npre*nm*a*ldY);
+	ensure1(sizeof(double2)*(size_t)npre*nm*a*ldY);
 	{	StFirst2D s; memset(&s, 0, sizeof(s));
 		s.fa = mk(fc_, a); s.fb = mk(fc_, 0);
 		s.src.leg = s2_.as<double2>(); s.src.cstride = nm*ldF; s.src.ld = ldF; s.src.nr = (int)ny; s.src.N = (int)ny; s.src.ncol = (int)nm; s.src.plain = 1;
@@ -972,7 +1140,7 @@
 		s.groups = (int)((nm + T - 1)/T); s.dgr = make_fastdiv((uint32_t)s.groups);
 		launch_any(s, npre*s.groups*a, st);
 	}
-	PXS_HIP(hipGetLastError());
+	if (!dry_) PXS_HIP(hipGetLastError());
 	return true;
 }
 
@@ -982,8 +1150,8 @@
 	const long ax = std::min(sx.a, sx.b), bx = nx/ax, ay = std::min(sy.a, sy.b), by = ny/ay, ldF = pad8(ny);
 	if (npre*std::max(nx, ny) >= (1L << 31)/512) return false;
 	if (getenv("PXS_CHAIN_VERBOSE")) fprintf(stderr, "[pxsht] fft2_c2c %ld x %ld x %ld: rows %ld x %ld, columns %ld x %ld\n", npre, ny, nx, ax, bx, ay, by);
-	s1_.ensure(sizeof(double2)*(size_t)npre*std::max(ny*ax*pad8(bx), nx*ay*pad8(by)));
-	s2_.ensure(sizeof(double2)*(size_t)npre*nx*ldF);
+	ensure1(sizeof(double2)*(size_t)npre*std::max(ny*ax*pad8(bx), nx*ay*pad8(by)));
+	ensure2(sizeof(double2)*(size_t)npre*nx*ldF);
 	auto first = [&](const double2* src, long nlines, long ld, long n, long a, long b, int conj) {
 		StFirst2D s; memset(&s, 0, sizeof(s));
 		s.fa = mk(fc_, a); s.fb = mk(fc_, 0);
@@ -1005,7 +1173,7 @@
 	second(s2_.as<double2>(), ny, ldF, nx*ldF, ax, bx, 0, 1.0);
 	first(s2_.as<double2>(), nx, ldF, ny, ay, by, 0);
 	second(out, nx, nx, ny*nx, ay, by, forward ? 0 : 1, scale);
-	PXS_HIP(hipGetLastError());
+	if (!dry_) PXS_HIP(hipGetLastError());
 	return true;
 }
 
diff --git a/pixell_amd/csrc/fftchain.hpp b/pixell_amd/csrc/fftchain.hpp
--- a/pixell_amd/csrc/fftchain.hpp
+++ b/pixell_amd/csrc/fftchain.hpp
@@ -2,6 +2,8 @@
 #include "fft.hpp"
 #include <tuple>
 #include <map>
+#include <set>
+#include <vector>
 #include <mutex>
 #include <memory>
 
@@ -10,6 +12,7 @@
 struct Lds2;
 
 struct Split { long a = 0, b = 0; };
+struct ChainShape { int sid, na, nb, T; bool is_static; };
 
 struct ThetaPlan {
 	bool ok = false;
@@ -53,7 +56,16 @@
 	static void theta_scratch(const ThetaPlan& tp, int nm, int nc, int kind, size_t& b1, size_t& b2);
 	void ring_scratch(long nring, int nc, bool analysis, size_t& b1, int mmax = -1) const;
 	void reserve(size_t b1, size_t b2) { s1_.ensure(b1); s2_.ensure(b2); }
+	void dry_begin(std::vector<ChainShape>* out) { dry_ = out; }
+	void dry_end() { dry_ = nullptr; }
+	int static_check(int maxr = 0);
+	static bool static_has(int sid, int na, int nb, int T);
+	static void static_shapes(std::vector<ChainShape>& out);
 private:
+	void ensure1(size_t b) { if (!dry_) s1_.ensure(b); }
+	void ensure2(size_t b) { if (!dry_) s2_.ensure(b); }
+	std::vector<ChainShape>* dry_ = nullptr;
+	std::set<int> checked_;
 	const double2* small_tw(long X, int n, int T);
 	template<class S> void set_tiles(S& s, int T, long nlines, long X);
 	template<class S> int tile_lines_for(long n_a, long n_b, long nlines, int mult, long tab_pts = -1);
diff --git a/pixell_amd/csrc/sht.hip b/pixell_amd/csrc/sht.hip
--- a/pixell_amd/csrc/sht.hip
+++ b/pixell_amd/csrc/sht.hip
@@ -971,6 +971,39 @@
 }
 static Route route_of(const pxs_plan* p, bool analysis, int spin, int mode, bool adjoint, const LegTables* tb);
 static Route analysis_route_now(const pxs_plan* p) { return route_of(p, true, 0, PXS_MODE_STANDARD, false, nullptr); }
+static std::vector<ChainShape> chain_shapes(const pxs_plan* cp) {
+	pxs_plan* p = const_cast<pxs_plan*>(cp);
+	std::vector<ChainShape> all, out;
+	if (!p->chain || !p->chain_rings) return out;
+	std::lock_guard<std::mutex> plan_lock(p->call_mu);
+	const int nm = p->mmax + 1;
+	FftChain::MapDesc md; memset(&md, 0, sizeof(md)); md.dtype = PX_F64; md.cstride = (long)p->nring*p->nphi; md.ring_stride = p->nphi; md.pix_stride = 1; md.nring = p->nring; md.nphi = p->nphi;
+	p->chain->dry_begin(&all);
+	try {
+		for (int which = 0; which < 3; which++) {
+			const bool ana = which == 0; const int spin = which == 2 ? 2 : 0;
+			const Route r = route_of(p, ana, spin, PXS_MODE_STANDARD, false, nullptr);
+			if (!r.reserve_chain) continue;
+			if (ana) p->chain->map2leg(nullptr, md, r.nc, p->mmax, nullptr, r.ld_leg, nullptr, 1.0);
+			else p->chain->h2map(nullptr, nullptr, r.ld_h, md, r.nc, p->mmax, 0);
+			if (!r.theta_fused || r.line) continue;
+			switch (r.theta) {
+			case TH_TO_CC:       p->chain->to_cc(nullptr, *r.tp, nullptr, r.ld_leg, r.nr_th, p->mir_c, nullptr, r.ld_leg2, p->ncc, r.nc, nm, spin, p->lmax, nullptr, nullptr, nullptr); break;
+			case TH_FROM_CC_ADJ: p->chain->from_cc_adjoint(nullptr, *r.tp, nullptr, r.ld_leg, r.nr_th, p->mir_c, nullptr, r.ld_leg2, p->ncc, r.nc, nm, spin, p->lmax, nullptr, nullptr, nullptr); break;
+			case TH_FROM_CC:     p->chain->from_cc(nullptr, *r.tp, nullptr, r.ld_leg2, p->ncc, nullptr, r.ld_h, r.nr_h, p->mir_c, r.nc, nm, spin, p->lmax, nullptr, nullptr, 1.0, nullptr); break;
+			case TH_TO_CC_ADJ:   p->chain->to_cc_adjoint(nullptr, *r.tp, nullptr, r.ld_leg2, p->ncc, nullptr, r.ld_h, r.nr_h, p->mir_c, r.nc, nm, spin, p->lmax, nullptr, nullptr, nullptr, nullptr, 2.0); break;
+			case TH_NONE: break;
+			}
+		}
+	} catch (...) { p->chain->dry_end(); throw; }
+	p->chain->dry_end();
+	for (const ChainShape& c : all) {
+		bool seen = false;
+		for (const ChainShape& o : out) seen = seen || (o.sid == c.sid && o.na == c.na && o.nb == c.nb && o.T == c.T);
+		if (!seen) out.push_back(c);
+	}
+	return out;
+}
 int pxs_plan_query(const pxs_plan* p, const char* name, int64_t* value) {
 	PXS_TRY
 	PXS_REQUIRE(p && name && value, "pxs_plan_query: null argument");
@@ -980,6 +1013,15 @@
 	else if (n == "ncc_circle") *value = p->ncc > 0 ? p->Ncc : 0;
 	else if (n == "ducc_ncc_circle") *value = FftChain::ducc_ncc(p->lmax);
 	else if (n == "theta_line") *value = analysis_route_now(p).line ? 1 : 0;
+	else if (n == "chain_stages" || n == "chain_static") {
+		int64_t k = 0;
+		for (const ChainShape& c : chain_shapes(p)) {
+			if (getenv("PXS_CHAIN_VERBOSE")) fprintf(stderr, "[pxsht] plan stage %d: na=%d nb=%d T=%d static %d\n", c.sid, c.na, c.nb, c.T, c.is_static ? 1 : 0);
+			k += (n == "chain_stages" || c.is_static) ? 1 : 0;
+		}
+		*value = k;
+	}
+	else if (n == "chain_static_table") *value = p->chain ? p->chain->static_check(0) : 0;
 	else throw Error(PXS_ERR_ARG, std::string("pxs_plan_query: unknown name '") + name + "'");
 	PXS_CATCH
 }
```

Measured after the change: 3.384, median of 6. 5.4% higher.
